# kerry-he/fsae-mpc

Measured on AMD Instinct MI355X. Metric: QP solves/sec (batched LTV-MPC, N=40 nx=5 nu=2 fp64), higher is better.
Workload: dtype f64

## Files before the change

### fsae-mpc_amd/_lib.py

```python
import ctypes as C
import os

_HERE = os.path.dirname(os.path.abspath(__file__))
LIB_PATH = os.environ.get("FSAEMPC_LIB") or os.path.join(_HERE, "lib", "libfsaempc.so")

EXPORTS = [
    "fsaempc_qp_default_opts", "fsaempc_qp_workspace_bytes", "fsaempc_qp_solve_batch_device", "fsaempc_qp_solve_batch",
    "fsaempc_ltv_nx", "fsaempc_ltv_nV", "fsaempc_ltv_nC", "fsaempc_ltv_build_qp_batch_device",
    "fsaempc_ltv_workspace_bytes", "fsaempc_ltv_step_batch_device", "fsaempc_ltv_step_batch_device_aux", "fsaempc_last_error", "fsaempc_selftest_mfma", "fsaempc_selftest_lane_reduce", "fsaempc_selftest_diag_factor",
    "fsaempc_debug_set_dump", "fsaempc_qp_solve_batch_device_aux", "fsaempc_qp_set_timing", "fsaempc_qp_get_timing", "fsaempc_ltv_get_timing",
    "fsaempc_seq_init", "fsaempc_seq_hotstart", "fsaempc_seq_hotstart_matrices", "fsaempc_seq_equality", "fsaempc_seq_cleanup",
    "fsaempc_obtain_reference_batch_device", "fsaempc_reference_live_batch_device",
    "fsaempc_cl_pre_batch_device", "fsaempc_cl_plant_batch_device", "fsaempc_cl_accept_batch_device",
    "fsaempc_track_from_csv", "fsaempc_track_from_points", "fsaempc_track_free", "fsaempc_track_save", "fsaempc_track_load", "fsaempc_track_last_error",
    "fsaempc_nlp_build_qp_batch_device", "fsaempc_sqp_default_opts", "fsaempc_sqp_workspace_bytes", "fsaempc_sqp_batch_device",
    "fsaempc_sqp_get_timing", "fsaempc_qp_vjp_workspace_bytes", "fsaempc_qp_vjp_batch_device",
    "fsaempc_ltv_affine_maps_batch_device", "fsaempc_ltv_step_batch_device_lambda", "fsaempc_ltv_step_vjp_workspace_bytes",
    "fsaempc_ltv_step_vjp_batch_device",
    "fsaempc_ltv_default_params", "fsaempc_ltv_build_qp_batch_device_p", "fsaempc_ltv_step_batch_device_p",
    "fsaempc_nlp_build_qp_batch_device_p", "fsaempc_sqp_batch_device_p", "fsaempc_cl_plant_batch_device_p",
    "fsaempc_ltv_blocked_nV", "fsaempc_ltv_build_qp_batch_device_b", "fsaempc_ltv_workspace_bytes_b", "fsaempc_ltv_step_batch_device_b",
    "fsaempc_qp_workspace_bytes_s", "fsaempc_qp_solve_batch_device_s", "fsaempc_qp_layout",
    "fsaempc_plan_profile_batch_device", "fsaempc_plan_reference_batch_device", "fsaempc_cl_pre_plan_batch_device",
    "fsaempc_raceline_build_qp_device", "fsaempc_plan_line_profile_batch_device", "fsaempc_plan_raceline_workspace_bytes",
    "fsaempc_plan_raceline_batch_device",
]

NPAR = 32
PARAM_INDEX = {name: i for i, name in enumerate(
    ["M", "IZ", "LF", "LR", "GRAV", "PB", "PC", "PD", "PE", "Q_S", "Q_N", "Q_MU", "Q_TERMINAL", "R_ACC", "R_STEER",
     "R_SOFT0", "R_SOFT1", "R_SOFT2", "R_SOFT3", "U_ACC_MAX", "U_STEER_MAX", "DELTA_MAX", "N_MAX", "V_MIN", "ALAT_MAX", "SLIP_MAX",
     "ELL_LONG", "ELL_LAT", "PID_KP_V", "PID_MAX_F", "PID_KP_D", "PID_MAX_DRATE"])}


class QpOpts(C.Structure):
    _fields_ = [("tol", C.c_double), ("tol_loose", C.c_double), ("tol_x", C.c_double), ("inf_bound", C.c_double),
                ("max_iter", C.c_int), ("polish", C.c_int)]


class QpAux(C.Structure):
    _fields_ = [("kkt", C.c_void_p), ("polished", C.c_void_p), ("x_init", C.c_void_p), ("difficulty", C.c_void_p)]


class QpDesc(C.Structure):
    _fields_ = [("nV", C.c_int), ("nC", C.c_int), ("batch", C.c_int), ("shared_HA", C.c_int)]


class QpVjpIO(C.Structure):
    _fields_ = [("xbar", C.c_void_p), ("fbar", C.c_void_p), ("gbar", C.c_void_p), ("lbbar", C.c_void_p), ("ubbar", C.c_void_p),
                ("lbAbar", C.c_void_p), ("ubAbar", C.c_void_p), ("Hbar", C.c_void_p), ("Abar", C.c_void_p)]


class LtvVjpIO(C.Structure):
    _fields_ = [("ubar", C.c_void_p), ("xbar", C.c_void_p), ("sbar", C.c_void_p), ("fbar", C.c_void_p), ("x0bar", C.c_void_p),
                ("xrefbar", C.c_void_p)]


class Spline(C.Structure):
    _fields_ = [("M", C.c_int), ("dl", C.c_double), ("xP", C.c_void_p), ("yP", C.c_void_p)]


class LtvDesc(C.Structure):
    _fields_ = [("model", C.c_int), ("N", C.c_int), ("batch", C.c_int), ("dt", C.c_double), ("integrator", C.c_int)]


class LtvParams(C.Structure):
    _fields_ = [("values", C.c_void_p), ("per_instance", C.c_int)]


class LtvBlocking(C.Structure):
    _fields_ = [("n_blocks", C.c_int), ("len", C.POINTER(C.c_int))]


PLAN_MAX_NS = 4096
LINE_MAX_NS = 2048
LINE_MIN_NC = 8
MAX_NV = 196


class PlanTable(C.Structure):
    _fields_ = [("table", C.c_void_p), ("t", C.c_void_p), ("N_s", C.c_int), ("ds", C.c_double), ("per_instance", C.c_int)]


def check_blocking(blocking, N):
    try:
        lens = [int(v) for v in blocking]
    except TypeError:
        raise ValueError("blocking must be a sequence of block lengths")
    if any(int(v) != v for v in blocking):
        raise ValueError("blocking: the block lengths must be integers")
    if len(lens) < 1:
        raise ValueError("blocking: at least one block")
    if min(lens) < 1:
        raise ValueError("blocking: every block length must be >= 1")
    if sum(lens) != N:
        raise ValueError("blocking: the block lengths sum to %d, the horizon has N = %d steps" % (sum(lens), N))
    return lens


class Blocking:

    def __init__(self, blocking, N):
        self.lens = check_blocking(blocking, N)
        self.n_blocks = len(self.lens)
        self.trivial = self.n_blocks == N
        self._arr = (C.c_int * self.n_blocks)(*self.lens)
        self.c = LtvBlocking(self.n_blocks, C.cast(self._arr, C.POINTER(C.c_int)))
        self.block_of_step = [j for j, l in enumerate(self.lens) for _ in range(l)]
        self.start = [sum(self.lens[:j]) for j in range(self.n_blocks)]

    def ref(self):
        return C.byref(self.c)


class SqpOpts(C.Structure):
    _fields_ = [("max_sweeps", C.c_int), ("trials", C.c_int), ("tol_step", C.c_double), ("tol_feas", C.c_double), ("armijo", C.c_double),
                ("rho0", C.c_double), ("warm_start", C.c_int)]


class SqpAux(C.Structure):
    _fields_ = [("lambda_", C.c_void_p), ("qp_iter", C.c_void_p), ("step_norm", C.c_void_p), ("hard_viol", C.c_void_p), ("merit", C.c_void_p)]


class TrackTable(C.Structure):
    _fields_ = [("M", C.c_int), ("dl", C.c_double), ("L", C.c_double), ("xP", C.POINTER(C.c_double)), ("yP", C.POINTER(C.c_double))]


class FsaempcError(RuntimeError):
    pass


_LIB = None


def lib():
    global _LIB
    if _LIB is None:
        if not os.path.exists(LIB_PATH):
            raise FsaempcError("libfsaempc.so not built (%s): run `make` or __graft_entry__.build(); "
                               "there is no CPU fallback" % LIB_PATH)
        try:
            import torch
        except ImportError:
            pass
        L = C.CDLL(LIB_PATH)
        L.fsaempc_last_error.restype = C.c_char_p
        L.fsaempc_qp_workspace_bytes.restype = C.c_longlong
        L.fsaempc_ltv_workspace_bytes.restype = C.c_longlong
        L.fsaempc_sqp_workspace_bytes.restype = C.c_longlong
        L.fsaempc_qp_vjp_workspace_bytes.restype = C.c_longlong
        L.fsaempc_ltv_step_vjp_workspace_bytes.restype = C.c_longlong
        vp, ll = C.c_void_p, C.c_longlong
        L.fsaempc_qp_solve_batch_device.argtypes = [C.POINTER(QpDesc)] + [vp] * 7 + [C.POINTER(QpOpts)] + [vp] * 5 + [vp, ll, vp]
        L.fsaempc_qp_solve_batch_device_aux.argtypes = [C.POINTER(QpDesc)] + [vp] * 7 + [C.POINTER(QpOpts)] + [vp] * 5 + [C.POINTER(QpAux), vp, ll, vp]
        L.fsaempc_qp_vjp_workspace_bytes.argtypes = [C.POINTER(QpDesc)]
        L.fsaempc_qp_vjp_batch_device.argtypes = [C.POINTER(QpDesc), C.c_int] + [vp] * 7 + [vp] * 4 + [C.POINTER(QpOpts), C.POINTER(QpVjpIO), vp, vp, ll, vp]
        L.fsaempc_ltv_affine_maps_batch_device.argtypes = [C.POINTER(LtvDesc), C.POINTER(Spline)] + [vp] * 5
        L.fsaempc_ltv_step_batch_device_lambda.argtypes = [C.POINTER(LtvDesc), C.POINTER(Spline)] + [vp] * 4 + [C.POINTER(QpOpts)] + [vp] * 7 + \
            [C.POINTER(QpAux), vp, ll, vp]
        L.fsaempc_ltv_step_vjp_workspace_bytes.argtypes = [C.POINTER(LtvDesc), C.c_int]
        L.fsaempc_ltv_step_vjp_batch_device.argtypes = [C.POINTER(LtvDesc), C.POINTER(Spline), C.c_int] + [vp] * 4 + [vp] * 5 + \
            [C.POINTER(QpOpts), C.POINTER(LtvVjpIO), vp, vp, ll, vp]
        L.fsaempc_qp_solve_batch.argtypes = [C.POINTER(QpDesc)] + [vp] * 7 + [C.POINTER(QpOpts)] + [vp] * 5
        L.fsaempc_ltv_build_qp_batch_device.argtypes = [C.POINTER(LtvDesc), C.POINTER(Spline)] + [vp] * 4 + [vp] * 7 + [vp] * 3 + [vp]
        L.fsaempc_ltv_step_batch_device.argtypes = [C.POINTER(LtvDesc), C.POINTER(Spline)] + [vp] * 4 + [C.POINTER(QpOpts)] + [vp] * 6 + [vp, ll, vp]
        L.fsaempc_ltv_step_batch_device_aux.argtypes = [C.POINTER(LtvDesc), C.POINTER(Spline)] + [vp] * 4 + [C.POINTER(QpOpts)] + [vp] * 6 + [C.POINTER(QpAux), vp, ll, vp]
        L.fsaempc_nlp_build_qp_batch_device.argtypes = [C.POINTER(LtvDesc), C.POINTER(Spline)] + [vp] * 3 + [vp] * 7 + [vp] * 3 + [vp]
        L.fsaempc_sqp_default_opts.argtypes = [C.POINTER(SqpOpts)]
        L.fsaempc_sqp_workspace_bytes.argtypes = [C.POINTER(LtvDesc)]
        L.fsaempc_sqp_batch_device.argtypes = [C.POINTER(LtvDesc), C.POINTER(Spline)] + [vp] * 3 + [C.POINTER(QpOpts), C.POINTER(SqpOpts)] + \
            [vp] * 6 + [C.POINTER(SqpAux), vp, ll, vp]
        L.fsaempc_sqp_get_timing.argtypes = [C.POINTER(C.c_double)] * 4
        L.fsaempc_obtain_reference_batch_device.argtypes = [vp, C.c_double, C.c_int, vp, vp, C.c_double, C.c_int, C.c_int, vp, vp]
        L.fsaempc_reference_live_batch_device.argtypes = [C.c_int, C.c_int, C.c_double, C.c_double, C.c_int, vp, vp, vp]
        L.fsaempc_cl_pre_batch_device.argtypes = [C.c_int, C.c_int, C.c_double, C.c_double, C.c_double, C.POINTER(Spline), vp, vp, C.c_int, vp, vp, vp, vp]
        L.fsaempc_cl_plant_batch_device.argtypes = [C.c_int, C.c_int, C.c_double, C.c_int, vp, vp, vp, vp, vp, vp, vp]
        L.fsaempc_cl_accept_batch_device.argtypes = [C.c_int, C.c_int, C.c_int, vp, vp, vp, vp, vp, vp]
        L.fsaempc_ltv_default_params.argtypes = [C.c_int, C.POINTER(C.c_double)]
        L.fsaempc_ltv_build_qp_batch_device_p.argtypes = [C.POINTER(LtvDesc), C.POINTER(Spline), C.POINTER(LtvParams)] + [vp] * 4 + [vp] * 7 + [vp] * 3 + [vp]
        L.fsaempc_ltv_step_batch_device_p.argtypes = [C.POINTER(LtvDesc), C.POINTER(Spline), C.POINTER(LtvParams)] + [vp] * 4 + [C.POINTER(QpOpts)] + \
            [vp] * 7 + [C.POINTER(QpAux), vp, ll, vp]
        L.fsaempc_nlp_build_qp_batch_device_p.argtypes = [C.POINTER(LtvDesc), C.POINTER(Spline), C.POINTER(LtvParams)] + [vp] * 3 + [vp] * 7 + [vp] * 3 + [vp]
        L.fsaempc_sqp_batch_device_p.argtypes = [C.POINTER(LtvDesc), C.POINTER(Spline), C.POINTER(LtvParams)] + [vp] * 3 + \
            [C.POINTER(QpOpts), C.POINTER(SqpOpts)] + [vp] * 6 + [C.POINTER(SqpAux), vp, ll, vp]
        L.fsaempc_cl_plant_batch_device_p.argtypes = [C.c_int, C.c_int, C.c_double, C.c_int, C.POINTER(LtvParams), vp, vp, vp, vp, vp, vp, vp]
        L.fsaempc_ltv_blocked_nV.argtypes = [C.c_int, C.POINTER(LtvBlocking)]
        L.fsaempc_ltv_build_qp_batch_device_b.argtypes = [C.POINTER(LtvDesc), C.POINTER(Spline), C.POINTER(LtvParams), C.POINTER(LtvBlocking)] + \
            [vp] * 4 + [vp] * 7 + [vp] * 3 + [vp]
        L.fsaempc_ltv_workspace_bytes_b.restype = C.c_longlong
        L.fsaempc_ltv_workspace_bytes_b.argtypes = [C.POINTER(LtvDesc), C.POINTER(LtvBlocking)]
        L.fsaempc_ltv_step_batch_device_b.argtypes = [C.POINTER(LtvDesc), C.POINTER(Spline), C.POINTER(LtvParams), C.POINTER(LtvBlocking)] + \
            [vp] * 4 + [C.POINTER(QpOpts)] + [vp] * 7 + [C.POINTER(QpAux), vp, ll, vp]
        L.fsaempc_qp_workspace_bytes_s.restype = C.c_longlong
        L.fsaempc_qp_workspace_bytes_s.argtypes = [C.POINTER(QpDesc), C.c_int]
        L.fsaempc_qp_solve_batch_device_s.argtypes = [C.POINTER(QpDesc), C.c_int] + [vp] * 7 + [C.POINTER(QpOpts)] + [vp] * 5 + \
            [C.POINTER(QpAux), vp, ll, vp]
        L.fsaempc_qp_layout.argtypes = [C.POINTER(QpDesc), C.c_int, C.POINTER(C.c_int)]
        L.fsaempc_plan_profile_batch_device.argtypes = [C.c_int, C.POINTER(Spline), C.c_double, C.POINTER(LtvParams), C.c_int, C.c_int,
                                                        C.c_double, C.c_double, vp, vp, vp]
        L.fsaempc_plan_reference_batch_device.argtypes = [C.c_int, C.POINTER(PlanTable), vp, C.c_double, C.c_int, C.c_int, vp, vp]
        L.fsaempc_cl_pre_plan_batch_device.argtypes = [C.c_int, C.c_int, C.c_double, C.c_double, C.POINTER(Spline), C.POINTER(PlanTable),
                                                       vp, vp, C.c_int, vp, vp, vp, vp]
        L.fsaempc_raceline_build_qp_device.argtypes = [C.POINTER(Spline), C.c_double, C.c_int, C.c_int, vp, vp, vp]
        L.fsaempc_plan_line_profile_batch_device.argtypes = [C.c_int, C.POINTER(Spline), C.c_double, C.POINTER(LtvParams), C.c_int, C.c_int, C.c_int,
                                                             vp, C.c_int, C.c_double, C.c_double, vp, vp, vp]
        L.fsaempc_plan_raceline_workspace_bytes.restype = C.c_longlong
        L.fsaempc_plan_raceline_workspace_bytes.argtypes = [C.c_int, C.c_int]
        L.fsaempc_plan_raceline_batch_device.argtypes = [C.c_int, C.POINTER(Spline), C.c_double, C.POINTER(LtvParams), C.c_int, C.c_int, C.c_int,
                                                         C.c_double, C.c_double, C.c_double, C.POINTER(QpOpts), vp, vp, vp, vp, vp, ll, vp]
        L.fsaempc_debug_set_dump.argtypes = [vp, C.c_int]
        L.fsaempc_track_last_error.restype = C.c_char_p
        L.fsaempc_track_from_csv.argtypes = [C.c_char_p, C.c_int, C.POINTER(TrackTable)]
        L.fsaempc_track_from_points.argtypes = [vp, vp, C.c_int, C.c_int, C.POINTER(TrackTable)]
        L.fsaempc_track_free.argtypes = [C.POINTER(TrackTable)]
        L.fsaempc_track_save.argtypes = [C.POINTER(TrackTable), C.c_char_p]
        L.fsaempc_track_load.argtypes = [C.c_char_p, C.POINTER(TrackTable)]
        _LIB = L
    return _LIB


def check(rc, what):
    if rc != 0:
        raise FsaempcError("%s failed (%d): %s" % (what, rc, lib().fsaempc_last_error().decode()))


def default_params(model):
    import numpy as np
    out = np.zeros(NPAR, dtype=np.float64)
    check(lib().fsaempc_ltv_default_params(int(model), out.ctypes.data_as(C.POINTER(C.c_double))), "fsaempc_ltv_default_params")
    return out


class ParamBlock:

    def __init__(self, params, batch, device):
        import numpy as np
        import torch
        t = params if isinstance(params, torch.Tensor) else torch.from_numpy(np.ascontiguousarray(np.asarray(params, dtype=np.float64)))
        if tuple(t.shape) not in ((NPAR,), (batch, NPAR)):
            raise ValueError("params must be (%d,) or (batch = %d, %d), got %s" % (NPAR, batch, NPAR, tuple(t.shape)))
        self.tensor = t.to(device=device, dtype=torch.float64).contiguous()
        self.per_instance = 1 if t.dim() == 2 else 0
        self.c = LtvParams(C.c_void_p(self.tensor.data_ptr()), self.per_instance)

    def ref(self):
        return C.byref(self.c)


def sqp_default_opts(**kw):
    o = SqpOpts()
    lib().fsaempc_sqp_default_opts(C.byref(o))
    for k, v in kw.items():
        if not hasattr(o, k):
            raise TypeError("unknown SQP option %r" % k)
        setattr(o, k, v)
    return o


def default_opts(**kw):
    o = QpOpts()
    lib().fsaempc_qp_default_opts(C.byref(o))
    for k, v in kw.items():
        setattr(o, k, v)
    return o
```

### fsae-mpc_amd/csrc/capi.hip

```cpp
#include <hip/hip_runtime.h>
#include <math.h>
#include <stdio.h>
#include <string.h>
#include <stdlib.h>
#include <dlfcn.h>
#include <atomic>
#include <mutex>
#include <vector>
#include "fsaempc.h"
#include "qp_solver.h"
#include "ltv_build.h"
#include "reference.h"
#include "plant.h"
#include "planner.h"
#include "raceline.h"
#include "sqp.h"
#include "qp_sens.h"

namespace {
thread_local char g_err[512] = "";
std::atomic<double*> g_dump{nullptr}; std::atomic<int> g_dump_stage{0};
std::atomic<bool> g_timing{false}; hipEvent_t g_ev[3] = {nullptr, nullptr, nullptr};
hipEvent_t g_evf[2] = {nullptr, nullptr};
hipEvent_t g_evs[5] = {nullptr, nullptr, nullptr, nullptr, nullptr};
// ... 767 lines not shown
  if (desc->batch == 0) return 0;
  SqpCarve c; sqp_carve(desc, &c);
  if ((long long)c.total > workspace_bytes) return fail(FSAEMPC_ERR_WORKSPACE, "workspace too small");
  char* w = (char*)workspace;
  auto D = [&](size_t off) { return (double*)(w + off); };
  auto Iw = [&](size_t off) { return (int*)(w + off); };
  hipStream_t st = (hipStream_t)stream;
  const int nx = fsaempc_ltv_nx(desc->model), N = desc->N, nV = fsaempc_ltv_nV(desc->model, N), nC = fsaempc_ltv_nC(desc->model, N);
  SqpParams P; memset(&P, 0, sizeof(P));
  P.nx = nx; P.N = N; P.integ = ltv_integ(desc); P.B = desc->batch; P.dt = desc->dt;
  P.spM = sp->M; P.spdl = sp->dl; P.xP = sp->xP; P.yP = sp->yP;
  P.x0 = x0; P.x_ref = x_ref; P.u = u_opt; P.x = x_opt; P.s = slack; P.fval = fval; P.status = status; P.sweeps = sweeps;
  P.rho = D(c.rho); P.J = D(c.J); P.viol = D(c.viol); P.vmax = D(c.vmax);
  if (aux) { P.lambda_out = aux->lambda; P.qp_iter = aux->qp_iter; P.step_norm = aux->step_norm; P.hard_viol = aux->hard_viol; P.merit = aux->merit; }
  P.max_sweeps = o.max_sweeps; P.trials = o.trials; P.tol_step = o.tol_step; P.tol_feas = o.tol_feas; P.armijo = o.armijo; P.rho0 = o.rho0;
  Range whole("fsaempc.sqp");
  const bool timing = g_timing.load();
  for (double& v : g_sqp_ms) v = 0;
  hipError_t e = sqp_init_launch(P, u_init, st, par_values(par), par_stride(par));
  if (e != hipSuccess) return hipfail(e, "sqp_init_launch");
  for (int sweep = 0; sweep < o.max_sweeps; ++sweep) {
    if (timing) { e = hipEventRecord(g_evs[0], st); if (e != hipSuccess) return hipfail(e, "hipEventRecord"); }
    int cnt = 0;
    { Range r("fsaempc.sqp.compact");
      e = sqp_compact_launch(status, desc->batch, Iw(c.idx), Iw(c.cnt), st);
      if (e == hipSuccess) e = hipMemcpyAsync(&cnt, Iw(c.cnt), sizeof(int), hipMemcpyDeviceToHost, st);
      if (e == hipSuccess) e = hipStreamSynchronize(st); }
    if (e != hipSuccess) return hipfail(e, "sqp compaction");
    if (cnt == 0) break;
    double* xinit = o.warm_start ? D(c.xinit) : nullptr;
    e = sqp_gather_launch(P, Iw(c.idx), cnt, D(c.gx0), D(c.gxr), D(c.gu), xinit, nV, st);
    if (e != hipSuccess) return hipfail(e, "sqp_gather_launch");
    if (timing) { e = hipEventRecord(g_evs[1], st); if (e != hipSuccess) return hipfail(e, "hipEventRecord"); }
    fsaempc_ltv_desc sub = *desc; sub.batch = cnt;
    { Range r("fsaempc.sqp.build");
      rc = build_qp(&sub, sp, D(c.gx0), D(c.gxr), nullptr, D(c.gu), D(c.H), D(c.g), D(c.A), D(c.lb), D(c.ub), D(c.lbA), D(c.ubA),
                    D(c.pred), D(c.Bt), D(c.qc), stream, true, par, Iw(c.idx)); }
    if (rc) return rc;
    if (timing) { e = hipEventRecord(g_evs[2], st); if (e != hipSuccess) return hipfail(e, "hipEventRecord"); }
    fsaempc_qp_desc q{nV, nC, cnt, 0};
    fsaempc_qp_aux qa{nullptr, nullptr, xinit, nullptr};
    rc = fsaempc_qp_solve_batch_device_aux(&q, D(c.H), D(c.g), D(c.A), D(c.lb), D(c.ub), D(c.lbA), D(c.ubA), qp_opts, D(c.z), D(c.qf),
                                           Iw(c.qflag), Iw(c.qit), D(c.lam), &qa, w + c.qpws, (long long)(c.total - c.qpws), stream);
    if (rc) return rc;
    if (timing) { e = hipEventRecord(g_evs[3], st); if (e != hipSuccess) return hipfail(e, "hipEventRecord"); }
    { Range r("fsaempc.sqp.linesearch");
      e = sqp_linesearch_launch(P, Iw(c.idx), cnt, sweep, D(c.z), D(c.qf), D(c.qc), Iw(c.qflag), Iw(c.qit), D(c.lam), st,
                                par_values(par), par_stride(par)); }
    if (e != hipSuccess) return hipfail(e, "sqp_linesearch_launch");
    if (timing) {
      e = hipEventRecord(g_evs[4], st); if (e == hipSuccess) e = hipEventSynchronize(g_evs[4]);
      if (e != hipSuccess) return hipfail(e, "hipEventRecord");
      for (int k = 0; k < 4; ++k) { float ms = 0; if (hipEventElapsedTime(&ms, g_evs[k], g_evs[k + 1]) == hipSuccess) g_sqp_ms[k] += ms; }
    }
  }
  return 0;
}

int fsaempc_sqp_get_timing(double* build_ms, double* solve_ms, double* linesearch_ms, double* compact_ms) {
  if (!build_ms || !solve_ms || !linesearch_ms || !compact_ms) return fail(FSAEMPC_ERR_ARG, "null argument");
  *compact_ms = g_sqp_ms[0]; *build_ms = g_sqp_ms[1]; *solve_ms = g_sqp_ms[2]; *linesearch_ms = g_sqp_ms[3];
  return 0;
}

int fsaempc_obtain_reference_batch_device(const double* plan, double ds, int N_s, const double* t, const double* s0, double dt,
                                          int N_t, int batch, double* x_ref, void* stream) {
  if (!plan || !t || !s0 || !x_ref) return fail(FSAEMPC_ERR_ARG, "null argument");
  if (N_s <= 0 || N_t <= 0 || batch < 0 || !(ds > 0) || !(dt > 0)) return fail(FSAEMPC_ERR_ARG, "bad dimensions");
  RefParams P; P.plan = plan; P.t = t; P.s0 = s0; P.x_ref = x_ref; P.ds = ds; P.dt = dt; P.N_s = N_s; P.N_t = N_t; P.batch = batch;
  hipError_t e = obtain_reference_launch(P, (hipStream_t)stream);
  if (e != hipSuccess) return hipfail(e, "obtain_reference_launch");
  return 0;
}

int fsaempc_reference_live_batch_device(int nx, int N, double dt, double target_vel, int batch, const double* x0, double* x_ref, void* stream) {
  if (!x0 || !x_ref) return fail(FSAEMPC_ERR_ARG, "null argument");
  if ((nx != 5 && nx != 7) || N <= 0 || batch < 0 || !(dt > 0)) return fail(FSAEMPC_ERR_ARG, "bad dimensions");
  hipError_t e = reference_live_launch(nx, N, dt, target_vel, batch, x0, x_ref, (hipStream_t)stream);
  if (e != hipSuccess) return hipfail(e, "reference_live_launch");
  return 0;
}

int fsaempc_cl_pre_batch_device(int model, int N, double dt, double target_vel, double L, const fsaempc_spline* sp, const double* cart,
                                const double* s_guess, int batch, double* x0, double* x_ref, int* finished, void* stream) {
  if (!sp || !sp->xP || !sp->yP || !cart || !s_guess || !x0 || !x_ref || !finished) return fail(FSAEMPC_ERR_ARG, "null argument");
  if (model != FSAEMPC_MODEL_KINEMATIC && model != FSAEMPC_MODEL_DYNAMIC) return fail(FSAEMPC_ERR_ARG, "unknown model");
  if (N <= 0 || batch < 0 || !(dt > 0) || sp->M <= 0 || !(sp->dl > 0) || !(L > 0)) return fail(FSAEMPC_ERR_ARG, "bad dimensions");
  ClPreParams P; P.nx = fsaempc_ltv_nx(model); P.N = N; P.batch = batch; P.dt = dt; P.target_vel = target_vel; P.L = L;
  P.spM = sp->M; P.spdl = sp->dl; P.xP = sp->xP; P.yP = sp->yP; P.cart = cart; P.s_guess = s_guess; P.x0 = x0; P.x_ref = x_ref; P.finished = finished;
  hipError_t e = cl_pre_launch(P, (hipStream_t)stream);
  if (e != hipSuccess) return hipfail(e, "cl_pre_launch");
  return 0;
}

int fsaempc_cl_plant_batch_device(int model, int N, double dt, int batch, double* cart, double* pid, const double* x_opt,
                                  const int* finished, const int* exitflag, double* u_last, void* stream) {
  return fsaempc_cl_plant_batch_device_p(model, N, dt, batch, nullptr, cart, pid, x_opt, finished, exitflag, u_last, stream);
}

int fsaempc_cl_plant_batch_device_p(int model, int N, double dt, int batch, const fsaempc_ltv_params* par, double* cart, double* pid,
                                    const double* x_opt, const int* finished, const int* exitflag, double* u_last, void* stream) {
  if (!cart || !pid || !x_opt) return fail(FSAEMPC_ERR_ARG, "null argument");
  if (model != FSAEMPC_MODEL_KINEMATIC && model != FSAEMPC_MODEL_DYNAMIC) return fail(FSAEMPC_ERR_ARG, "unknown model");
  if (N <= 0 || batch < 0 || !(dt > 0)) return fail(FSAEMPC_ERR_ARG, "bad dimensions");
  ClPlantParams P; P.nx = fsaempc_ltv_nx(model); P.N = N; P.batch = batch; P.dt = dt; P.cart = cart; P.pid = pid; P.x_opt = x_opt;
  P.finished = finished; P.exitflag = exitflag; P.u_last = u_last;
  hipError_t e = cl_plant_launch(P, (hipStream_t)stream, par_values(par), par_stride(par));
  if (e != hipSuccess) return hipfail(e, "cl_plant_launch");
  return 0;
}

int fsaempc_cl_accept_batch_device(int model, int N, int batch, const double* x_new, const double* u_new, const int* exitflag, double* x_keep, double* u_keep, void* stream) {
  if (!x_new || !u_new || !x_keep || !u_keep) return fail(FSAEMPC_ERR_ARG, "null argument");
  if (model != FSAEMPC_MODEL_KINEMATIC && model != FSAEMPC_MODEL_DYNAMIC) return fail(FSAEMPC_ERR_ARG, "unknown model");
  if (N <= 0 || batch < 0) return fail(FSAEMPC_ERR_ARG, "bad dimensions");
  hipError_t e = cl_accept_launch(fsaempc_ltv_nx(model) * N, 2 * N, batch, x_new, u_new, exitflag, x_keep, u_keep, (hipStream_t)stream);
  if (e != hipSuccess) return hipfail(e, "cl_accept_launch");
  return 0;
}

static bool pos_finite(double v) { return v > 0 && v < INFINITY; }
static int plan_check(const fsaempc_plan* plan, PlanTable* out) {
  if (!plan || !plan->table || !plan->t) return fail(FSAEMPC_ERR_ARG, "null argument");
  if (plan->N_s < 1 || !pos_finite(plan->ds)) return fail(FSAEMPC_ERR_ARG, "bad plan dimensions");
  out->table = plan->table; out->t = plan->t; out->N_s = plan->N_s; out->ds = plan->ds; out->per_instance = plan->per_instance ? 1 : 0;
  return 0;
}

int fsaempc_plan_profile_batch_device(int model, const fsaempc_spline* sp, double L, const fsaempc_ltv_params* par, int n_plans, int N_s,
                                      double v_cap, double grip, double* table, double* t, void* stream) {
  if (!sp || !sp->xP || !sp->yP || !table || !t) return fail(FSAEMPC_ERR_ARG, "null argument");
  if (model != FSAEMPC_MODEL_KINEMATIC && model != FSAEMPC_MODEL_DYNAMIC) return fail(FSAEMPC_ERR_ARG, "unknown model");
  if (sp->M <= 0 || !(sp->dl > 0)) return fail(FSAEMPC_ERR_ARG, "bad dimensions");
  if (N_s < 2 || N_s > FSAEMPC_PLAN_MAX_NS) return fail(FSAEMPC_ERR_ARG, "N_s must be 2 .. FSAEMPC_PLAN_MAX_NS");
  if (!pos_finite(v_cap) || !pos_finite(grip) || !pos_finite(L)) return fail(FSAEMPC_ERR_ARG, "v_cap, grip and L must be finite and > 0");
  if (grip > 1) return fail(FSAEMPC_ERR_ARG, "grip must be <= 1");
  if (n_plans < 1) return fail(FSAEMPC_ERR_ARG, "n_plans must be >= 1");
  if (par_values(par) && !par->per_instance && n_plans != 1) return fail(FSAEMPC_ERR_ARG, "a shared parameter block makes one plan");
  PlanProfileParams P; P.dynamic = model == FSAEMPC_MODEL_DYNAMIC; P.n_plans = n_plans; P.N_s = N_s; P.ds = L / N_s; P.v_cap = v_cap; P.grip = grip;
  P.spM = sp->M; P.spdl = sp->dl; P.xP = sp->xP; P.yP = sp->yP; P.table = table; P.t = t;
  hipError_t e = plan_profile_launch(P, par_values(par), par_stride(par), (hipStream_t)stream);
  if (e != hipSuccess) return hipfail(e, "plan_profile_launch");
  return 0;
}

int fsaempc_plan_reference_batch_device(int model, const fsaempc_plan* plan, const double* s0, double dt, int N, int batch, double* x_ref,
                                        void* stream) {
  PlanRefParams P;
  if (int rc = plan_check(plan, &P.plan)) return rc;
  if (!s0 || !x_ref) return fail(FSAEMPC_ERR_ARG, "null argument");
  if (model != FSAEMPC_MODEL_KINEMATIC && model != FSAEMPC_MODEL_DYNAMIC) return fail(FSAEMPC_ERR_ARG, "unknown model");
  if (N <= 0 || batch < 0 || !pos_finite(dt)) return fail(FSAEMPC_ERR_ARG, "bad dimensions");
  P.nx = fsaempc_ltv_nx(model); P.N = N; P.batch = batch; P.dt = dt; P.s0 = s0; P.x_ref = x_ref;
  hipError_t e = plan_reference_launch(P, (hipStream_t)stream);
  if (e != hipSuccess) return hipfail(e, "plan_reference_launch");
  return 0;
}

int fsaempc_cl_pre_plan_batch_device(int model, int N, double dt, double L, const fsaempc_spline* sp, const fsaempc_plan* plan,
                                     const double* cart, const double* s_guess, int batch, double* x0, double* x_ref, int* finished,
                                     void* stream) {
  ClPrePlanParams P;
  if (!sp || !sp->xP || !sp->yP || !cart || !s_guess || !x0 || !x_ref || !finished) return fail(FSAEMPC_ERR_ARG, "null argument");
  if (int rc = plan_check(plan, &P.plan)) return rc;
  if (model != FSAEMPC_MODEL_KINEMATIC && model != FSAEMPC_MODEL_DYNAMIC) return fail(FSAEMPC_ERR_ARG, "unknown model");
  if (N <= 0 || batch < 0 || !pos_finite(dt) || sp->M <= 0 || !(sp->dl > 0) || !(L > 0)) return fail(FSAEMPC_ERR_ARG, "bad dimensions");
  P.nx = fsaempc_ltv_nx(model); P.N = N; P.batch = batch; P.dt = dt; P.L = L;
  P.spM = sp->M; P.spdl = sp->dl; P.xP = sp->xP; P.yP = sp->yP; P.cart = cart; P.s_guess = s_guess; P.x0 = x0; P.x_ref = x_ref; P.finished = finished;
  hipError_t e = cl_pre_plan_launch(P, (hipStream_t)stream);
  if (e != hipSuccess) return hipfail(e, "cl_pre_plan_launch");
  return 0;
}

static int line_check(const fsaempc_spline* sp, double L, int N_s, int N_c) {
  if (!sp || !sp->xP || !sp->yP) return fail(FSAEMPC_ERR_ARG, "null argument");
  if (sp->M <= 0 || !(sp->dl > 0)) return fail(FSAEMPC_ERR_ARG, "bad dimensions");
  if (!pos_finite(L)) return fail(FSAEMPC_ERR_ARG, "L must be finite and > 0");
  if (N_c < FSAEMPC_LINE_MIN_NC || N_c > FSAEMPC_MAX_NV) return fail(FSAEMPC_ERR_ARG, "N_c must be FSAEMPC_LINE_MIN_NC .. FSAEMPC_MAX_NV");
  if (N_s < 2 * N_c || N_s > FSAEMPC_LINE_MAX_NS) return fail(FSAEMPC_ERR_ARG, "N_s must be 2 N_c .. FSAEMPC_LINE_MAX_NS");
  return 0;
}
static int line_profile_check(int model, const fsaempc_ltv_params* par, int n_plans, double v_cap, double grip) {
  if (model != FSAEMPC_MODEL_KINEMATIC && model != FSAEMPC_MODEL_DYNAMIC) return fail(FSAEMPC_ERR_ARG, "unknown model");
  if (!pos_finite(v_cap) || !pos_finite(grip)) return fail(FSAEMPC_ERR_ARG, "v_cap and grip must be finite and > 0");
  if (grip > 1) return fail(FSAEMPC_ERR_ARG, "grip must be <= 1");
  if (n_plans < 1) return fail(FSAEMPC_ERR_ARG, "n_plans must be >= 1");
  if (par_values(par) && !par->per_instance && n_plans != 1) return fail(FSAEMPC_ERR_ARG, "a shared parameter block makes one plan");
  return 0;
}
static RacelineQpParams line_qp_params(const fsaempc_spline* sp, double L, int N_s, int N_c, double* H, double* g) {
  RacelineQpParams Q; Q.N_s = N_s; Q.N_c = N_c; Q.ds = L / N_s; Q.spM = sp->M; Q.spdl = sp->dl; Q.xP = sp->xP; Q.yP = sp->yP; Q.H = H; Q.g = g;
  return Q;
}
static PlanLineParams line_profile_params(int model, const fsaempc_spline* sp, double L, int n_plans, int N_s, int N_c, double v_cap, double grip,
                                          double* table, double* t) {
  PlanLineParams P; memset(&P, 0, sizeof(P));
  P.dynamic = model == FSAEMPC_MODEL_DYNAMIC; P.n_plans = n_plans; P.N_s = N_s; P.N_c = N_c; P.ds = L / N_s; P.h = L / N_c; P.v_cap = v_cap; P.grip = grip;
  P.spM = sp->M; P.spdl = sp->dl; P.xP = sp->xP; P.yP = sp->yP; P.table = table; P.t = t;
  return P;
}

int fsaempc_raceline_build_qp_device(const fsaempc_spline* sp, double L, int N_s, int N_c, double* H, double* g, void* stream) {
  if (!H || !g) return fail(FSAEMPC_ERR_ARG, "null argument");
  if (int rc = line_check(sp, L, N_s, N_c)) return rc;
  hipError_t e = raceline_qp_launch(line_qp_params(sp, L, N_s, N_c, H, g), (hipStream_t)stream);
  if (e != hipSuccess) return hipfail(e, "raceline_qp_launch");
  return 0;
}

int fsaempc_plan_line_profile_batch_device(int model, const fsaempc_spline* sp, double L, const fsaempc_ltv_params* par, int n_plans, int N_s,
                                           int N_c, const double* line, int line_per_plan, double v_cap, double grip, double* table, double* t,
                                           void* stream) {
  if (!line || !table || !t) return fail(FSAEMPC_ERR_ARG, "null argument");
  if (int rc = line_check(sp, L, N_s, N_c)) return rc;
  if (int rc = line_profile_check(model, par, n_plans, v_cap, grip)) return rc;
  PlanLineParams P = line_profile_params(model, sp, L, n_plans, N_s, N_c, v_cap, grip, table, t);
  P.line = line; P.line_stride = line_per_plan ? N_c : 0;
  hipError_t e = plan_line_profile_launch(P, par_values(par), par_stride(par), (hipStream_t)stream);
  if (e != hipSuccess) return hipfail(e, "plan_line_profile_launch");
  return 0;
}

struct LineCarve { size_t H, g, lb, ub, fval, iter, qp, total; long long qp_bytes; };
static int line_carve(int n_plans, int N_c, LineCarve* c) {
  if (n_plans < 1 || N_c < FSAEMPC_LINE_MIN_NC || N_c > FSAEMPC_MAX_NV) return FSAEMPC_ERR_ARG;
  const fsaempc_qp_desc d = {N_c, 0, n_plans, 1};
  c->qp_bytes = fsaempc_qp_workspace_bytes_s(&d, 0);
  if (c->qp_bytes < 0) return (int)c->qp_bytes;
  const size_t vec = align64((size_t)n_plans * N_c * sizeof(double));
  size_t off = 0;
  c->H = off; off += align64((size_t)N_c * N_c * sizeof(double));
  c->g = off; off += vec;
  c->lb = off; off += vec;
  c->ub = off; off += vec;
  c->fval = off; off += align64((size_t)n_plans * sizeof(double));
  c->iter = off; off += align64((size_t)n_plans * sizeof(int));
  c->qp = off; off += (size_t)c->qp_bytes;
  c->total = off;
  return 0;
}
long long fsaempc_plan_raceline_workspace_bytes(int n_plans, int N_c) {
  LineCarve c;
  if (int rc = line_carve(n_plans, N_c, &c)) return rc;
  return (long long)c.total;
}

int fsaempc_plan_raceline_batch_device(int model, const fsaempc_spline* sp, double L, const fsaempc_ltv_params* par, int n_plans, int N_s,
                                       int N_c, double margin, double v_cap, double grip, const fsaempc_qp_opts* opts, double* line, int* flag,
                                       double* table, double* t, void* workspace, long long workspace_bytes, void* stream) {
  if (!line || !flag || !table || !t || !workspace) return fail(FSAEMPC_ERR_ARG, "null argument");
  if (int rc = line_check(sp, L, N_s, N_c)) return rc;
  if (int rc = line_profile_check(model, par, n_plans, v_cap, grip)) return rc;
  if (!(margin >= 0 && margin < INFINITY)) return fail(FSAEMPC_ERR_ARG, "margin must be finite and >= 0");
  LineCarve c;
  if (int rc = line_carve(n_plans, N_c, &c)) return fail(rc, "bad dimensions");
  if ((long long)c.total > workspace_bytes) return fail(FSAEMPC_ERR_WORKSPACE, "workspace too small");
  char* ws = (char*)workspace;
  double *H = (double*)(ws + c.H), *g = (double*)(ws + c.g), *lb = (double*)(ws + c.lb), *ub = (double*)(ws + c.ub);
  hipError_t e = raceline_qp_launch(line_qp_params(sp, L, N_s, N_c, H, g), (hipStream_t)stream);
  if (e != hipSuccess) return hipfail(e, "raceline_qp_launch");
  RacelineBoundsParams B; B.n_plans = n_plans; B.N_c = N_c; B.margin = margin; B.g = g; B.lb = lb; B.ub = ub;
  e = raceline_bounds_launch(B, par_values(par), par_stride(par), (hipStream_t)stream);
  if (e != hipSuccess) return hipfail(e, "raceline_bounds_launch");
  const fsaempc_qp_desc d = {N_c, 0, n_plans, 1};
  if (int rc = fsaempc_qp_solve_batch_device_s(&d, 0, H, g, nullptr, lb, ub, nullptr, nullptr, opts, line, (double*)(ws + c.fval), flag,
                                               (int*)(ws + c.iter), nullptr, nullptr, ws + c.qp, c.qp_bytes, stream)) return rc;
  PlanLineParams P = line_profile_params(model, sp, L, n_plans, N_s, N_c, v_cap, grip, table, t);
  P.line = line; P.line_stride = N_c; P.flag = flag; P.line_out = line; P.check_width = 1; P.margin = margin;
  e = plan_line_profile_launch(P, par_values(par), par_stride(par), (hipStream_t)stream);
  if (e != hipSuccess) return hipfail(e, "plan_line_profile_launch");
  return 0;
}

int fsaempc_selftest_mfma(void) {
  int cnt = 0;
  hipError_t e = hipGetDeviceCount(&cnt);
  if (e != hipSuccess || cnt == 0) return fail(FSAEMPC_ERR_NODEVICE, "no HIP device");
  char msg[256] = "";
  int bad = qp_selftest_mfma(msg, sizeof(msg));
  if (bad != 0) snprintf(g_err, sizeof(g_err), "%s", msg);
  return bad;
}

int fsaempc_selftest_lane_reduce(void) {
  int cnt = 0;
  hipError_t e = hipGetDeviceCount(&cnt);
  if (e != hipSuccess || cnt == 0) return fail(FSAEMPC_ERR_NODEVICE, "no HIP device");
  char msg[256] = "";
  int bad = qp_selftest_lane_reduce(msg, sizeof(msg));
  if (bad != 0) snprintf(g_err, sizeof(g_err), "%s", msg);
  return bad;
}

int fsaempc_selftest_diag_factor(void) {
  int cnt = 0;
  hipError_t e = hipGetDeviceCount(&cnt);
  if (e != hipSuccess || cnt == 0) return fail(FSAEMPC_ERR_NODEVICE, "no HIP device");
  char msg[256] = "";
  int bad = qp_selftest_diag_factor(msg, sizeof(msg));
  if (bad != 0) snprintf(g_err, sizeof(g_err), "%s", msg);
  return bad;
}

int fsaempc_debug_set_dump(double* out, int stage) { g_dump.store(out); g_dump_stage.store(stage); return 0; }

int fsaempc_qp_set_timing(int enable) {
  if (enable && !g_ev[0]) {
    for (int i = 0; i < 3; ++i) { hipError_t e = hipEventCreate(&g_ev[i]); if (e != hipSuccess) return hipfail(e, "hipEventCreate"); }
    for (int i = 0; i < 2; ++i) { hipError_t e = hipEventCreate(&g_evf[i]); if (e != hipSuccess) return hipfail(e, "hipEventCreate"); }
    for (int i = 0; i < 5; ++i) { hipError_t e = hipEventCreate(&g_evs[i]); if (e != hipSuccess) return hipfail(e, "hipEventCreate"); }
  }
  g_timing.store(enable != 0);
  return 0;
}

int fsaempc_ltv_get_timing(double* build_ms, double* prep_ms, double* solve_ms, double* post_ms) {
  if (!g_evf[0]) return fail(FSAEMPC_ERR_ARG, "timing was never enabled");
  hipError_t e = hipEventSynchronize(g_evf[1]);
  if (e != hipSuccess) return hipfail(e, "hipEventSynchronize (no fused step since timing was enabled?)");
  float t[4] = {0, 0, 0, 0};
  e = hipEventElapsedTime(&t[0], g_evf[0], g_ev[0]); if (e != hipSuccess) return hipfail(e, "hipEventElapsedTime");
  e = hipEventElapsedTime(&t[1], g_ev[0], g_ev[1]); if (e != hipSuccess) return hipfail(e, "hipEventElapsedTime");
  e = hipEventElapsedTime(&t[2], g_ev[1], g_ev[2]); if (e != hipSuccess) return hipfail(e, "hipEventElapsedTime");
  e = hipEventElapsedTime(&t[3], g_ev[2], g_evf[1]); if (e != hipSuccess) return hipfail(e, "hipEventElapsedTime");
  if (build_ms) *build_ms = t[0];
  if (prep_ms) *prep_ms = t[1];
  if (solve_ms) *solve_ms = t[2];
  if (post_ms) *post_ms = t[3];
  return 0;
}

int fsaempc_qp_get_timing(double* prep_ms, double* solve_ms) {
  if (!g_ev[0]) return fail(FSAEMPC_ERR_ARG, "timing was never enabled");
  hipError_t e = hipEventSynchronize(g_ev[2]);
  if (e != hipSuccess) return hipfail(e, "hipEventSynchronize");
  float a = 0, b = 0;
  e = hipEventElapsedTime(&a, g_ev[0], g_ev[1]); if (e != hipSuccess) return hipfail(e, "hipEventElapsedTime");
  e = hipEventElapsedTime(&b, g_ev[1], g_ev[2]); if (e != hipSuccess) return hipfail(e, "hipEventElapsedTime");
  if (prep_ms) *prep_ms = a;
  if (solve_ms) *solve_ms = b;
  return 0;
}

}
```

### fsae-mpc_amd/csrc/qp_selftest.h

```cpp
#pragma once
#include <stdlib.h>
#include <stdio.h>
#include "qp_solve_kernel.h"

namespace {

__global__ void mfma_selftest_kernel(const double* Am, const double* Bm, double* Cm) {
  const int lane = threadIdx.x;
  const double a = Am[(lane & 15) * 4 + (lane >> 4)];
  const double bb = Bm[(lane >> 4) * 16 + (lane & 15)];
  v4d c = {0, 0, 0, 0};
  c = __builtin_amdgcn_mfma_f64_16x16x4f64(a, bb, c, 0, 0, 0);
#pragma unroll
  for (int p = 0; p < 4; ++p) Cm[((lane >> 4) + 4 * p) * 16 + (lane & 15)] = c[p];
}

DEVINL bool same_bits(double a, double b) { return __double_as_longlong(a) == __double_as_longlong(b) || (a != a && b != b); }
template <class OP> DEVINL double lds_grp16(double* sh, int lane, double v) {
  const int src[4] = {lane ^ 1, lane ^ 2, (lane & ~7) | (7 - (lane & 7)), (lane & ~15) | (15 - (lane & 15))};
#pragma unroll
  for (int s = 0; s < 4; ++s) {
    sh[lane] = v; __syncthreads();
    const double o = sh[src[s]]; __syncthreads();
    v = OP::f(v, o);
  }
  return v;
}
template <class OP> DEVINL double lds_q(double* sh, int lane, double v) {
#pragma unroll
  for (int bit = 16; bit <= 32; bit <<= 1) {
    sh[lane] = v; __syncthreads();
    const double a = sh[lane & ~bit], b = sh[lane | bit]; __syncthreads();
    v = OP::f(a, b);
  }
  return v;
}
DEVINL double q_named(OpSum, double v) { return q_sum(v); }
DEVINL double q_named(OpMax, double v) { return q_max(v); }
DEVINL double q_named(OpMin, double v) { return q_min(v); }
DEVINL double wave_named(OpSum, double v) { return wave_sum(v); }
DEVINL double wave_named(OpMax, double v) { return wave_max(v); }
DEVINL double wave_named(OpMin, double v) { return wave_min(v); }
DEVINL double wave_named_zf(OpSum, double v) { return wave_sum_zf(v); }
DEVINL double wave_named_zf(OpMax, double v) { return wave_max_zf(v); }
DEVINL double wave_named_zf(OpMin, double v) { return wave_min_zf(v); }
DEVINL double grp16_named(OpSum, double v) { return grp16_sum(v); }
DEVINL double grp16_named(OpMax, double v) { return grp16_max(v); }
DEVINL double grp16_named(OpMin, double v) { return grp16_min(v); }
template <int N> DEVINL void grp16_named(OpSum, double (&v)[N]) { grp16_sum(v); }
template <int N> DEVINL void grp16_named(OpMax, double (&v)[N]) { grp16_max(v); }
template <int N> DEVINL void grp16_named(OpMin, double (&v)[N]) { grp16_min(v); }
template <class OP, int N> DEVINL int lane_reduce_batch_bad(const double (&x)[8], const double (&rz)[8], const double (&rl_)[8]) {
  double a[N];
#pragma unroll
  for (int i = 0; i < N; ++i) a[i] = x[i];
  grp16_named(OP{}, a);
  int bad = 0;
#pragma unroll
  for (int i = 0; i < N; ++i) bad += (same_bits(a[i], rz[i]) ? 0 : 1) + (same_bits(a[i], rl_[i]) ? 0 : 1);
  return bad;
}
template <class OP> DEVINL int lane_reduce_op_bad(int op, double* sh, int lane, const double (&x)[8], int& first) {
  double rz[8], rl_[8];
#pragma unroll
  for (int i = 0; i < 8; ++i) {
    double z[1] = {x[i]};
    grp16_reduce<OP, true>(z);
    rz[i] = z[0];
    rl_[i] = lds_grp16<OP>(sh, lane, x[i]);
  }
  int bad = 0, b;
  auto note = [&](int test, int nb) { if (nb && first < 0) first = 100 * test + op; bad += nb; };
  { const double g = grp16_named(OP{}, x[0]); note(1, (same_bits(g, rz[0]) ? 0 : 1) + (same_bits(g, rl_[0]) ? 0 : 1)); }
  b = lane_reduce_batch_bad<OP, 2>(x, rz, rl_); note(2, b);
  b = lane_reduce_batch_bad<OP, 4>(x, rz, rl_); note(4, b);
  b = lane_reduce_batch_bad<OP, 8>(x, rz, rl_); note(8, b);
  { const double g = q_named(OP{}, x[1]); note(16, same_bits(g, lds_q<OP>(sh, lane, x[1])) ? 0 : 1); }
  {
    const double g = wave_named(OP{}, x[2]), z = wave_named_zf(OP{}, x[2]), l = lds_q<OP>(sh, lane, rl_[2]);
    note(64, (same_bits(g, z) ? 0 : 1) + (same_bits(g, l) ? 0 : 1));
  }
  return bad;
}
__global__ __launch_bounds__(64) void lane_reduce_selftest_kernel(const double* __restrict__ in, int rounds, int* __restrict__ out) {
  __shared__ double sh[64];
  const int lane = threadIdx.x;
  int bad = 0, first = -1, first_round = -1;
  for (int r = 0; r < rounds; ++r) {
    double x[8];
#pragma unroll
    for (int i = 0; i < 8; ++i) x[i] = in[((size_t)r * 8 + i) * 64 + lane];
    const int before = bad;
    bad += lane_reduce_op_bad<OpSum>(0, sh, lane, x, first);
    bad += lane_reduce_op_bad<OpMax>(1, sh, lane, x, first);
    bad += lane_reduce_op_bad<OpMin>(2, sh, lane, x, first);
    {
      double a[4] = {x[4], x[5], x[6], x[7]};
      wave_sum(a);
      int nb = 0;
#pragma unroll
      for (int i = 0; i < 4; ++i) nb += same_bits(a[i], wave_sum_zf(x[4 + i])) ? 0 : 1;
      if (nb && first < 0) first = 100 * 65;
      bad += nb;
    }
    if (bad != before && first_round < 0) first_round = r;
  }
  if (bad) {
    if (atomicAdd(&out[0], bad) == 0) { out[1] = first; out[2] = first_round; out[3] = lane; }
  }
}

template <int FORM> DEVINL int diag_factor_bad_vs_old(const Ctx& k, const v4d& U0, const v4d& R0, double floor_abs, const v4d& Uo, const v4d& Yo, const v4d& Ro, int bo) {
  v4d U = U0, R = R0, Y;
#pragma unroll
  for (int p = 0; p < 4; ++p) Y[p] = (k.q + 4 * p == k.c) ? 1.0 : 0.0;
  const int b = diag_factor<FORM>(k, U, Y, R, floor_abs);
  int bad = (b != bo) ? 1 : 0;
#pragma unroll
  for (int p = 0; p < 4; ++p)
    bad += (__double_as_longlong(U[p]) != __double_as_longlong(Uo[p])) + (__double_as_longlong(Y[p]) != __double_as_longlong(Yo[p])) +
           (__double_as_longlong(R[p]) != __double_as_longlong(Ro[p]));
  return bad;
}
__global__ __launch_bounds__(64) void diag_factor_selftest_kernel(const double* __restrict__ in, int ntiles, double floor_abs, int* __restrict__ out) {
  Ctx k = {};
  k.lane = threadIdx.x; k.c = k.lane & 15; k.q = k.lane >> 4;
  int bad = 0, first = -1, form = 0;
  for (int t = 0; t < ntiles; ++t) {
    v4d U0, R0, Uo, Ro, Yo;
#pragma unroll
    for (int p = 0; p < 4; ++p) {
      U0[p] = in[(size_t)t * 512 + (k.q + 4 * p) * 16 + k.c];
      R0[p] = in[(size_t)t * 512 + 256 + (k.q + 4 * p) * 16 + k.c];
      Yo[p] = (k.q + 4 * p == k.c) ? 1.0 : 0.0;
    }
    Uo = U0; Ro = R0;
    const int bo = diag_factor<0>(k, Uo, Yo, Ro, floor_abs);
    const int b1 = diag_factor_bad_vs_old<1>(k, U0, R0, floor_abs, Uo, Yo, Ro, bo);
    const int b2 = diag_factor_bad_vs_old<2>(k, U0, R0, floor_abs, Uo, Yo, Ro, bo);
    if ((b1 | b2) && first < 0) { first = t; form = b1 ? 1 : 2; }
    bad += b1 + b2;
  }
  if (bad) {
    if (atomicAdd(&out[0], bad) == 0) { out[1] = first; out[2] = form; out[3] = k.lane; }
  }
}

}

int qp_selftest_mfma(char* msg, int msglen) {
  double hA[64], hB[64], hC[256], ref[256];
  for (int i = 0; i < 16; ++i) for (int kk = 0; kk < 4; ++kk) hA[i * 4 + kk] = (double)(1 + i * 7 + kk * 3);
  for (int kk = 0; kk < 4; ++kk) for (int j = 0; j < 16; ++j) hB[kk * 16 + j] = (double)(2 + kk * 11 - j * 5);
  for (int i = 0; i < 16; ++i) for (int j = 0; j < 16; ++j) {
    double s = 0; for (int kk = 0; kk < 4; ++kk) s += hA[i * 4 + kk] * hB[kk * 16 + j];
    ref[i * 16 + j] = s;
  }
  double *dA = 0, *dB = 0, *dC = 0;
  if (hipMalloc(&dA, sizeof(hA)) != hipSuccess || hipMalloc(&dB, sizeof(hB)) != hipSuccess || hipMalloc(&dC, sizeof(hC)) != hipSuccess) return -1;
  (void)hipMemcpy(dA, hA, sizeof(hA), hipMemcpyHostToDevice);
  (void)hipMemcpy(dB, hB, sizeof(hB), hipMemcpyHostToDevice);
  (void)hipMemset(dC, 0, sizeof(hC));
  hipLaunchKernelGGL(mfma_selftest_kernel, dim3(1), dim3(64), 0, 0, dA, dB, dC);
  hipError_t e = hipDeviceSynchronize();
  if (e != hipSuccess) { snprintf(msg, msglen, "selftest launch: %s", hipGetErrorString(e)); (void)hipFree(dA); (void)hipFree(dB); (void)hipFree(dC); return -1; }
  (void)hipMemcpy(hC, dC, sizeof(hC), hipMemcpyDeviceToHost);
  (void)hipFree(dA); (void)hipFree(dB); (void)hipFree(dC);
  int bad = 0;
  for (int i = 0; i < 256; ++i) if (hC[i] != ref[i]) { if (!bad) snprintf(msg, msglen, "mfma layout mismatch at (%d,%d): got %g want %g", i / 16, i % 16, hC[i], ref[i]); ++bad; }
  return bad;
}

int qp_selftest_lane_reduce(char* msg, int msglen) {
  const int rounds = 256, nval = rounds * 8 * 64;
  double* h = (double*)malloc(sizeof(double) * nval);
  if (!h) return -1;
  unsigned long long st = 0x9E3779B97F4A7C15ull;
  auto rnd = [&]() { st = st * 6364136223846793005ull + 1442695040888963407ull; return (unsigned)(st >> 33); };
  for (int i = 0; i < nval; ++i) {
    const double e = -300.0 + 600.0 * (rnd() / 2147483648.0), m = 1.0 + 9.0 * (rnd() / 2147483648.0);
    h[i] = ((rnd() & 1) ? -1.0 : 1.0) * m * pow(10.0, e);
  }
  const double special[8] = {0.0, -0.0, 4.9406564584124654e-324, -2.2250738585072009e-308 / 3.0, INFINITY, -INFINITY, NAN, -NAN};
  for (int g = 0; g < rounds * 8; ++g) {
    const unsigned u = rnd();
    if ((u & 3) != 0) h[(size_t)g * 64 + ((u >> 2) & 63)] = special[(u >> 8) & 7];
    if ((u & 0x30000) == 0x30000) h[(size_t)g * 64 + ((u >> 18) & 63)] = special[(u >> 24) & 7];
  }
  double* d = 0; int* dout = 0; int hout[4] = {0, 0, 0, 0};
  if (hipMalloc(&d, sizeof(double) * nval) != hipSuccess || hipMalloc(&dout, sizeof(hout)) != hipSuccess) { free(h); if (d) (void)hipFree(d); return -1; }
  (void)hipMemcpy(d, h, sizeof(double) * nval, hipMemcpyHostToDevice);
  (void)hipMemset(dout, 0, sizeof(hout));
  free(h);
  hipLaunchKernelGGL(lane_reduce_selftest_kernel, dim3(1), dim3(64), 0, 0, d, rounds, dout);
  hipError_t e = hipDeviceSynchronize();
  if (e == hipSuccess) e = hipMemcpy(hout, dout, sizeof(hout), hipMemcpyDeviceToHost);
  (void)hipFree(d); (void)hipFree(dout);
  if (e != hipSuccess) { snprintf(msg, msglen, "lane-reduce selftest: %s", hipGetErrorString(e)); return -1; }
  if (hout[0]) snprintf(msg, msglen, "lane reductions: %d mismatches, first: test %d (1/2/4/8: grp16 single / batched, 16: q, 64: wave, 65: wave_sum batch) op %d (sum/max/min) round %d lane %d",
                        hout[0], hout[1] / 100, hout[1] % 100, hout[2], hout[3]);
  return hout[0];
}

int qp_selftest_diag_factor(char* msg, int msglen) {
  const int ntiles = 64;
  const double floor_abs = 1e-9;
  double* h = (double*)malloc(sizeof(double) * ntiles * 512);
  if (!h) return -1;
  unsigned long long st = 0xD1B54A32D192ED03ull;
  auto rnd = [&]() { st = st * 6364136223846793005ull + 1442695040888963407ull; return ((unsigned)(st >> 33)) / 2147483648.0; };
  for (int t = 0; t < ntiles; ++t) {
    double* D = h + (size_t)t * 512; double* R = D + 256;
    double Q[16][16], sv[16];
    for (int i = 0; i < 16; ++i) for (int j = 0; j < 16; ++j) Q[i][j] = i == j ? 1.0 : 0.0;
    for (int r = 0; r < 3; ++r) {
      double v[16], vv = 0;
      for (int i = 0; i < 16; ++i) { v[i] = 2.0 * rnd() - 1.0; vv += v[i] * v[i]; }
      for (int i = 0; i < 16; ++i) {
        double qv = 0;
        for (int j = 0; j < 16; ++j) qv += Q[i][j] * v[j];
        for (int j = 0; j < 16; ++j) Q[i][j] -= 2.0 * qv * v[j] / vv;
      }
    }
    const double lc = 10.0 * (t < 61 ? t / 60.0 : 0.3);
    for (int i = 0; i < 16; ++i) sv[i] = pow(10.0, -lc * i / 15.0);
    for (int i = 0; i < 16; ++i) for (int j = 0; j < 16; ++j) {
      double a = 0;
      for (int l = 0; l < 16; ++l) a += Q[i][l] * sv[l] * Q[j][l];
      D[i * 16 + j] = a;
    }
    for (int i = 0; i < 16; ++i) for (int j = 0; j < i; ++j) D[i * 16 + j] = D[j * 16 + i];
    for (int i = 0; i < 256; ++i) R[i] = 20.0 * rnd() - 10.0;
    if (t == 61) for (int j = 0; j < 16; ++j) { D[6 * 16 + j] *= 1e-6; D[j * 16 + 6] *= 1e-6; }
    if (t == 62) { D[5 * 16 + 9] = NAN; D[9 * 16 + 5] = NAN; }
    if (t == 63) D[10 * 16 + 10] = INFINITY;
  }
  double* d = 0; int* dout = 0; int hout[4] = {0, 0, 0, 0};
  if (hipMalloc(&d, sizeof(double) * ntiles * 512) != hipSuccess || hipMalloc(&dout, sizeof(hout)) != hipSuccess) { free(h); if (d) (void)hipFree(d); return -1; }
  (void)hipMemcpy(d, h, sizeof(double) * ntiles * 512, hipMemcpyHostToDevice);
  (void)hipMemset(dout, 0, sizeof(hout));
  free(h);
  hipLaunchKernelGGL(diag_factor_selftest_kernel, dim3(1), dim3(64), 0, 0, d, ntiles, floor_abs, dout);
  hipError_t e = hipDeviceSynchronize();
  if (e == hipSuccess) e = hipMemcpy(hout, dout, sizeof(hout), hipMemcpyDeviceToHost);
  (void)hipFree(d); (void)hipFree(dout);
  if (e != hipSuccess) { snprintf(msg, msglen, "diag_factor selftest: %s", hipGetErrorString(e)); return -1; }
  if (hout[0]) snprintf(msg, msglen, "diag_factor forms: %d mismatches with the former form, first: tile %d form %d lane %d", hout[0], hout[1], hout[2], hout[3]);
  return hout[0];
}
```

### fsae-mpc_amd/csrc/qp_solve_kernel.h

```cpp
#pragma once
#include "qp_solver.h"
#include "qp_lane.h"

#ifndef QP_SOLVE_PAIR
#define QP_SOLVE_PAIR 0
#endif
#ifndef QP_DIAG_FLAT
#define QP_DIAG_FLAT 1
#endif
#ifndef QP_SYRK_INTERLEAVE
#define QP_SYRK_INTERLEAVE 0
#endif

namespace {

template <int T> struct Tri {
  static constexpr int NT = T * (T + 1) / 2;
  __host__ __device__ static constexpr int idx(int I, int J) { return I * T - (I * (I - 1)) / 2 + (J - I); }
};

struct Ctx {
  int n, m, T, Kq, J, JB, JT, np, lane, c, q, nc, nb, ntr;
  const int* perm; const int* tcs; const int* aoff; const int* tend;
  const double* Aw; const double* Hw; const double* Ab; const double* Hb;
  double* rows;
  double* ring;
  double* cof;
  int rowlen;
  double* vec;
};
enum VecArr { V_X = 0, V_G, V_HX, V_R1, V_R2, V_P1, V_P2, V_P3, V_DX, V_E, V_NARR };

DEVINL double* rowp(const Ctx& k, int arr) { return k.rows + (size_t)arr * k.rowlen; }
DEVINL double* vecp(const Ctx& k, int arr) { return k.vec + arr * k.np; }

DEVINL bool row_valid(const Ctx& k, int js) {
  if (js < k.J) { const int s = 16 * js + k.c; return s < k.Kq && 4 * s + k.q < k.m; }
  return (js - k.J) * 64 + k.lane < k.n;
}

template <int T> DEVINL void hx_tiles(const Ctx& k, const double* X, double* HX) {
  double hx[T], hn[T][4], hc[T][4];
#pragma unroll
  for (int t = 0; t < T; ++t) hx[t] = 0.0;
#pragma unroll
  for (int Jt = 0; Jt < T; ++Jt)
#pragma unroll
    for (int p = 0; p < 4; ++p) hn[Jt][p] = k.Hw[((size_t)Jt * 4 + p) * 64 + k.lane];
#pragma unroll 1
  for (int I = 0; I < T; ++I) {
#pragma unroll
    for (int Jt = 0; Jt < T; ++Jt)
#pragma unroll
      for (int p = 0; p < 4; ++p) hc[Jt][p] = hn[Jt][p];
    if (I + 1 < T) {
#pragma unroll
      for (int Jt = 0; Jt < T; ++Jt)
#pragma unroll
        for (int p = 0; p < 4; ++p) hn[Jt][p] = k.Hw[((size_t)((I + 1) * T + Jt) * 4 + p) * 64 + k.lane];
    }
    double xk[4];
#pragma unroll
    for (int p = 0; p < 4; ++p) xk[p] = X[16 * I + k.q + 4 * p];
#pragma unroll
    for (int Jt = 0; Jt < T; ++Jt)
#pragma unroll
      for (int p = 0; p < 4; ++p) hx[Jt] = fma(hc[Jt][p], xk[p], hx[Jt]);
  }
#pragma unroll
  for (int t = 0; t < T; ++t) {
    double v = q_sum(hx[t]);
    if (k.q == 0) HX[16 * t + k.c] = v;
  }
}
template <int T> DEVINL void acc_init(const Ctx& k, v4d* acc) {
#pragma unroll
  for (int I = 0; I < T; ++I)
#pragma unroll
    for (int Jt = I; Jt < T; ++Jt) {
      const double* hp = k.Hw + ((size_t)(I * T + Jt) * 4) * 64 + k.lane;
      v4d h;
#pragma unroll
      for (int p = 0; p < 4; ++p) h[p] = hp[p * 64];
      acc[Tri<T>::idx(I, Jt)] = h;
    }
}

template <int T> DEVINL void hx_from_acc(const Ctx& k, const v4d* acc, const double* XV, double* HX) {
  double xr[T][4], xc[T], sc[T], sr[T][4];
#pragma unroll
  for (int I = 0; I < T; ++I) {
    xc[I] = XV[16 * I + k.c]; sc[I] = 0.0;
#pragma unroll
    for (int p = 0; p < 4; ++p) { xr[I][p] = XV[16 * I + k.q + 4 * p]; sr[I][p] = 0.0; }
  }
#pragma unroll
  for (int I = 0; I < T; ++I)
#pragma unroll
    for (int J = I; J < T; ++J) {
      const v4d& h = acc[Tri<T>::idx(I, J)];
#pragma unroll
      for (int p = 0; p < 4; ++p) {
        sc[J] = fma(h[p], xr[I][p], sc[J]);
        if (J > I) sr[I][p] = fma(h[p], xc[J], sr[I][p]);
      }
    }
  WAVE_SYNC();
#pragma unroll
  for (int J = 0; J < T; ++J) { const double v = q_sum(sc[J]); if (k.q == 0) HX[16 * J + k.c] = v; }
  WAVE_SYNC();
#pragma unroll
  for (int I = 0; I < T - 1; ++I) {
    grp16_sum(sr[I]);
#pragma unroll
    for (int p = 0; p < 4; ++p) if (k.c == 0) HX[16 * I + k.q + 4 * p] += sr[I][p];
  }
}

template <int C> struct IC { static constexpr int value = C; };

template <int T> struct StreamCfg {
  static constexpr int D = 2 * T;
  static constexpr int R = D + T;
};
template <int T> struct Stream {
  static constexpr int D = StreamCfg<T>::D, R = StreamCfg<T>::R;
  static_assert(R == QP_SOLVE_RING(T), "qp_solve_lds (qp_solver.h) sizes the ring");
  const char* gnext; int slot_i, slot_e;
  int tend[T + 1];
  DEVINL void issue(const Ctx& k) {
    __builtin_amdgcn_global_load_lds((const __attribute__((address_space(1))) void*)(gnext + k.lane * 16),
                                     (__attribute__((address_space(3))) void*)(k.ring + slot_i * 128), 16, 0, 0);
    gnext += 1024;
    slot_i = slot_i + 1 == R ? 0 : slot_i + 1;
  }
  DEVINL void open(const Ctx& k) {
    gnext = reinterpret_cast<const char*>(k.Aw); slot_i = 0; slot_e = 0;
#pragma unroll
    for (int C = 0; C <= T; ++C) tend[C] = uni(k.tend[C]);
  }
  DEVINL void start(const Ctx& k) {
    gnext = reinterpret_cast<const char*>(k.Aw); slot_i = 0; slot_e = 0;
    if (k.ntr > 0) {
#pragma unroll
      for (int j = 0; j < D; ++j) issue(k);
    }
#pragma unroll
    for (int C = 0; C <= T; ++C) tend[C] = uni(tend[C]);
  }
  template <int C> DEVINL void next_pair(const Ctx& k, v2d* b) {
#pragma unroll
    for (int t = 0; t < C; ++t) issue(k);
    asm volatile("s_waitcnt vmcnt(%0)" :: "n"(D) : "memory");
#pragma unroll
    for (int t = 0; t < C; ++t) {
      int sl = slot_e + t; if (sl >= R) sl -= R;
      b[t] = *reinterpret_cast<const v2d*>(k.ring + sl * 128 + k.lane * 2);
    }
    slot_e += C; if (slot_e >= R) slot_e -= R;
  }
  DEVINL void finish() { asm volatile("s_waitcnt vmcnt(0)" ::: "memory"); }
  DEVINL void close() { asm volatile("s_waitcnt vmcnt(0)" ::: "memory"); }
};

template <int NA> struct CoefStage {
  double reg[NA > 0 ? NA : 1];
  DEVINL void load(const Ctx& k, const double* const* arr, int js) {
    const int jc = js < k.J ? js : k.J - 1;
#pragma unroll
    for (int a = 0; a < NA; ++a) reg[a] = arr[a][jc * 64 + k.lane];
  }
  DEVINL void commit(const Ctx& k) {
#pragma unroll
    for (int a = 0; a < NA; ++a) k.cof[a * 64 + k.lane] = reg[a];
  }
  DEVINL void read_pair(const Ctx& k, int s, v2d* out) const {
#pragma unroll
    for (int a = 0; a < NA; ++a) out[a] = *reinterpret_cast<const v2d*>(k.cof + a * 64 + k.q * 16 + (s & 15));
  }
};

template <int T, int NB> DEVINL void pass_syrk(const Ctx& k, Stream<T>& st, v4d* acc, double* P1, double* P2, double* P3, double* MB) {
  constexpr int NBB = NB > 0 ? NB : 1;
  constexpr int NA = 4 + NB;
  const int JS = k.J * 64;
  const double* arr[NA];
  arr[0] = rowp(k, R_D); arr[1] = rowp(k, R_W1); arr[2] = rowp(k, R_W2); arr[3] = rowp(k, R_W3);
#pragma unroll
  for (int e = 0; e < NB; ++e) arr[4 + e] = k.Ab + (size_t)e * JS;
  double p1[T], p2[T], p3[T];
  double pb[NBB][T], sbb[NBB][NBB], pwb[3][NBB];
#pragma unroll
  for (int t = 0; t < T; ++t) { p1[t] = 0; p2[t] = 0; p3[t] = 0; }
#pragma unroll
  for (int e = 0; e < NBB; ++e) {
#pragma unroll
    for (int t = 0; t < T; ++t) pb[e][t] = 0;
#pragma unroll
    for (int f = 0; f < NBB; ++f) sbb[e][f] = 0;
    pwb[0][e] = pwb[1][e] = pwb[2][e] = 0;
  }
  CoefStage<NA> cs;
  int tr = 0;
  st.start(k);
  if (k.ntr > 0) cs.load(k, arr, 0);
  auto phase = [&](auto Cc) __attribute__((always_inline)) {
    constexpr int C = decltype(Cc)::value;
    const int tr_end = st.tend[C];
    for (; tr < tr_end; ++tr) {
      if ((tr & 3) == 0) { cs.commit(k); cs.load(k, arr, (tr >> 2) + 1); }
#pragma unroll
      for (int u = 0; u < 2; ++u) {
        v2d b[C], cf[NA];
        st.template next_pair<C>(k, b);
        cs.read_pair(k, 4 * tr + 2 * u, cf);
        asm volatile("" ::: "memory");
#if QP_SYRK_INTERLEAVE
        double a2[2][C];
#pragma unroll
        for (int h = 0; h < 2; ++h)
#pragma unroll
          for (int t = 0; t < C; ++t) a2[h][t] = cf[0][h] * b[t][h];
#endif
#pragma unroll
        for (int h = 0; h < 2; ++h) {
          double a[C], ab[NBB];
          const double dd = cf[0][h], w1 = cf[1][h], w2 = cf[2][h], w3 = cf[3][h];
#pragma unroll
          for (int e = 0; e < NB; ++e) ab[e] = cf[4 + e][h];
#pragma unroll
#if QP_SYRK_INTERLEAVE
          for (int t = 0; t < C; ++t) a[t] = a2[h][t];
#else
          for (int t = 0; t < C; ++t) a[t] = dd * b[t][h];
#endif
#pragma unroll
          for (int I = 0; I < C; ++I)
#pragma unroll
            for (int Jt = I; Jt < C; ++Jt)
              acc[Tri<T>::idx(I, Jt)] = __builtin_amdgcn_mfma_f64_16x16x4f64(a[I], b[Jt][h], acc[Tri<T>::idx(I, Jt)], 0, 0, 0);
#pragma unroll
          for (int t = 0; t < C; ++t) {
            p1[t] = fma(w1, b[t][h], p1[t]); p2[t] = fma(w2, b[t][h], p2[t]); p3[t] = fma(w3, b[t][h], p3[t]);
          }
#pragma unroll
          for (int e = 0; e < NB; ++e) {
            const double dab = dd * ab[e];
#pragma unroll
            for (int t = 0; t < C; ++t) pb[e][t] = fma(dab, b[t][h], pb[e][t]);
#pragma unroll
            for (int f = e; f < NB; ++f) sbb[e][f] = fma(dab, ab[f], sbb[e][f]);
            pwb[0][e] = fma(w1, ab[e], pwb[0][e]); pwb[1][e] = fma(w2, ab[e], pwb[1][e]); pwb[2][e] = fma(w3, ab[e], pwb[2][e]);
          }
#if QP_SYRK_INTERLEAVE
#pragma unroll
          for (int i = 0; i < C * (C + 1) / 2; ++i) {
            __builtin_amdgcn_sched_group_barrier(0x008, 1, 0);
            __builtin_amdgcn_sched_group_barrier(0x002, 2, 0);
          }
#endif
        }
      }
    }
  };
  if constexpr (T >= 1) phase(IC<1>{});
  if constexpr (T >= 2) phase(IC<2>{});
  if constexpr (T >= 3) phase(IC<3>{});
  if constexpr (T >= 4) phase(IC<4>{});
  if constexpr (T >= 5) phase(IC<5>{});
  if constexpr (T >= 6) phase(IC<6>{});
  if constexpr (T >= 7) phase(IC<7>{});
  if constexpr (T >= 8) phase(IC<8>{});
  if (k.ntr > 0) st.finish();
#pragma unroll
  for (int t = 0; t < T; ++t) {
    double v1 = q_sum(p1[t]), v2 = q_sum(p2[t]), v3 = q_sum(p3[t]);
    if (k.q == 0) { P1[16 * t + k.c] = v1; P2[16 * t + k.c] = v2; P3[16 * t + k.c] = v3; }
  }
#pragma unroll
  for (int e = 0; e < NB; ++e) {
#pragma unroll
    for (int t = 0; t < T; ++t) { const double vb = q_sum(pb[e][t]); if (k.q == 0) MB[e * k.np + 16 * t + k.c] = vb; }
    const double v1 = q_sum(pwb[0][e]), v2 = q_sum(pwb[1][e]), v3 = q_sum(pwb[2][e]);
    if (k.lane == 0) { P1[k.nc + e] = v1; P2[k.nc + e] = v2; P3[k.nc + e] = v3; }
#pragma unroll
    for (int f = 0; f < NB; ++f) {
      const double sv = q_sum(f >= e ? sbb[e][f] : sbb[f][e]);
      if (k.lane == 0) MB[e * k.np + k.nc + f] = sv;
    }
  }
}

template <int T, int NB, int NVEC, int FUSE> DEVINL void pass_Av(const Ctx& k, Stream<T>& st, const double* const* vin, double* const* rout, double* Pcor, double* Pcor2 = nullptr, const double* const* cfarr = nullptr) {
  constexpr int NBB = NB > 0 ? NB : 1;
  constexpr int NC = FUSE == 1 ? 6 : (FUSE >= 2 ? 3 : 0);
  constexpr int NA = NC + NB;
  const int JS = k.J * 64;
  const double* arr[NA > 0 ? NA : 1];
  if (FUSE == 1) { arr[0] = rowp(k, R_RPL); arr[1] = rowp(k, R_CB1); arr[2] = rowp(k, R_CC1); arr[3] = rowp(k, R_RPU); arr[4] = rowp(k, R_CB2); arr[5] = rowp(k, R_CC2); }
  if (FUSE >= 2) { arr[0] = cfarr ? cfarr[0] : rowp(k, R_CB1); arr[1] = cfarr ? cfarr[1] : rowp(k, R_RPL); arr[2] = cfarr ? cfarr[2] : rowp(k, R_CC1); }
#pragma unroll
  for (int f = 0; f < NB; ++f) arr[NC + f] = k.Ab + (size_t)f * JS;
  double v[NVEC][T], vb[NVEC][NBB], pc[T], pcb[NBB], pd[FUSE >= 2 ? T : 1], pdb[NBB];
#pragma unroll
  for (int e = 0; e < NVEC; ++e) {
#pragma unroll
    for (int t = 0; t < T; ++t) v[e][t] = vin[e][16 * t + k.c];
#pragma unroll
    for (int f = 0; f < NB; ++f) vb[e][f] = vin[e][k.nc + f];
  }
#pragma unroll
  for (int t = 0; t < T; ++t) pc[t] = 0.0;
#pragma unroll
  for (int f = 0; f < NBB; ++f) { pcb[f] = 0.0; pdb[f] = 0.0; }
#pragma unroll
  for (int t = 0; t < (FUSE >= 2 ? T : 1); ++t) pd[t] = 0.0;
  double keep[NVEC + 1];
#pragma unroll
  for (int e = 0; e < NVEC + 1; ++e) keep[e] = 0.0;
  CoefStage<NA> cs;
  int tr = 0;
  st.start(k);
  if (k.ntr > 0 && NA > 0) cs.load(k, arr, 0);
  auto phase = [&](auto Cc) __attribute__((always_inline)) {
    constexpr int C = decltype(Cc)::value;
    const int tr_end = st.tend[C];
    for (; tr < tr_end; ++tr) {
      if (NA > 0 && (tr & 3) == 0) { cs.commit(k); cs.load(k, arr, (tr >> 2) + 1); }
#pragma unroll
      for (int u = 0; u < 2; ++u) {
        v2d b[C], cf[NA > 0 ? NA : 1];
        st.template next_pair<C>(k, b);
        if (NA > 0) cs.read_pair(k, 4 * tr + 2 * u, cf);
        asm volatile("" ::: "memory");
        double ds[2 * NVEC];
#pragma unroll
        for (int h = 0; h < 2; ++h)
#pragma unroll
          for (int e = 0; e < NVEC; ++e) {
            double a = 0.0;
#pragma unroll
            for (int t = 0; t < C; ++t) a = fma(b[t][h], v[e][t], a);
            ds[h * NVEC + e] = a;
          }
        grp16_sum(ds);
#pragma unroll
        for (int h = 0; h < 2; ++h) {
          const int s = 4 * tr + 2 * u + h;
          const int cc = s & 15;
#pragma unroll
          for (int e = 0; e < NVEC; ++e) {
            double dsum = ds[h * NVEC + e];
#pragma unroll
            for (int f = 0; f < NB; ++f) dsum = fma(cf[NC + f][h], vb[e][f], dsum);
            if (k.c == cc) keep[e] = dsum;
            if (FUSE >= 2 && e == 0) {
              const double pen = cf[0][h] * (dsum - cf[1][h]);
              const double ynew = cf[2][h] - pen;
              if (k.c == cc) keep[NVEC] = ynew;
#pragma unroll
              for (int t = 0; t < C; ++t) { pc[t] = fma(ynew, b[t][h], pc[t]); pd[t] = fma(pen, b[t][h], pd[t]); }
#pragma unroll
              for (int f = 0; f < NB; ++f) { pcb[f] = fma(ynew, cf[NC + f][h], pcb[f]); pdb[f] = fma(pen, cf[NC + f][h], pdb[f]); }
            }
            if (FUSE == 1 && e == 0) {
              const double dl_ = dsum + cf[0][h], du_ = cf[3][h] - dsum;
              const double w = dl_ * fma(cf[2][h], dl_, cf[1][h]) - du_ * fma(cf[5][h], du_, cf[4][h]);
#pragma unroll
              for (int t = 0; t < C; ++t) pc[t] = fma(w, b[t][h], pc[t]);
#pragma unroll
              for (int f = 0; f < NB; ++f) pcb[f] = fma(w, cf[NC + f][h], pcb[f]);
            }
          }
          if (cc == 15 || s + 1 == 4 * k.ntr) {
            const int js = s >> 4;
#pragma unroll
            for (int e = 0; e < NVEC; ++e) { rout[e][js * 64 + k.lane] = keep[e]; keep[e] = 0.0; }
            if (FUSE >= 2) { rout[NVEC][js * 64 + k.lane] = keep[NVEC]; keep[NVEC] = 0.0; }
          }
        }
      }
    }
  };
  if constexpr (T >= 1) phase(IC<1>{});
  if constexpr (T >= 2) phase(IC<2>{});
  if constexpr (T >= 3) phase(IC<3>{});
  if constexpr (T >= 4) phase(IC<4>{});
  if constexpr (T >= 5) phase(IC<5>{});
  if constexpr (T >= 6) phase(IC<6>{});
  if constexpr (T >= 7) phase(IC<7>{});
  if constexpr (T >= 8) phase(IC<8>{});
  if (k.ntr > 0) st.finish();
  if (FUSE) {
#pragma unroll
    for (int t = 0; t < T; ++t) {
      double pv = q_sum(pc[t]);
      if (k.q == 0) Pcor[16 * t + k.c] = pv;
    }
#pragma unroll
    for (int f = 0; f < NB; ++f) { const double pv = q_sum(pcb[f]); if (k.lane == 0) Pcor[k.nc + f] = pv; }
  }
  if (FUSE >= 2) {
#pragma unroll
    for (int t = 0; t < T; ++t) {
      double pv = q_sum(pd[t]);
      if (k.q == 0) Pcor2[16 * t + k.c] = pv;
    }
#pragma unroll
    for (int f = 0; f < NB; ++f) { const double pv = q_sum(pdb[f]); if (k.lane == 0) Pcor2[k.nc + f] = pv; }
  }
}

template <int T, int NB> DEVINL void pass_Atw(const Ctx& k, const double* W, double* Pout) {
  constexpr int NBB = NB > 0 ? NB : 1;
  const int JS = k.J * 64;
  double p[T], pbv[NBB];
#pragma unroll
  for (int t = 0; t < T; ++t) p[t] = 0.0;
#pragma unroll
  for (int f = 0; f < NBB; ++f) pbv[f] = 0.0;
  for (int s = 0; s < 4 * k.ntr; ++s) {
    const int ri = (s >> 4) * 64 + k.q * 16 + (s & 15);
    const double w = W[ri];
    const int tr = s >> 2, tc = k.tcs[tr];
    const double* src = k.Aw + ((size_t)k.aoff[tr] + ((s >> 1) & 1) * tc) * 128 + k.lane * 2 + (s & 1);
#pragma unroll
    for (int t = 0; t < T; ++t)
      if (t < tc) p[t] = fma(w, src[t * 128], p[t]);
#pragma unroll
    for (int f = 0; f < NB; ++f) pbv[f] = fma(w, k.Ab[(size_t)f * JS + ri], pbv[f]);
  }
#pragma unroll
  for (int t = 0; t < T; ++t) {
    double v = q_sum(p[t]);
    if (k.q == 0) Pout[16 * t + k.c] = v;
  }
#pragma unroll
  for (int f = 0; f < NB; ++f) { const double pv = q_sum(pbv[f]); if (k.lane == 0) Pout[k.nc + f] = pv; }
}

template <int T> DEVINL void mfma4_sub(const v4d& X, const v4d& Y, v4d& Dst) {
#pragma unroll
  for (int p = 0; p < 4; ++p) Dst = __builtin_amdgcn_mfma_f64_16x16x4f64(-X[p], Y[p], Dst, 0, 0, 0);
}
DEVINL v4d mfma4_new(const v4d& X, const v4d& Y) {
  v4d Z = {0.0, 0.0, 0.0, 0.0};
#pragma unroll
  for (int p = 0; p < 4; ++p) Z = __builtin_amdgcn_mfma_f64_16x16x4f64(X[p], Y[p], Z, 0, 0, 0);
  return Z;
}

DEVINL void tile_store(const Ctx& k, double* slot, const v4d& Xt) {
#pragma unroll
  for (int p = 0; p < 4; ++p) slot[(k.q + 4 * p) * 17 + k.c] = Xt[p];
}
DEVINL v4d tile_load(const Ctx& k, const double* slot) {
  v4d Z;
#pragma unroll
  for (int p = 0; p < 4; ++p) Z[p] = slot[(k.q + 4 * p) * 17 + k.c];
  return Z;
}
DEVINL v4d tile_load_t(const Ctx& k, const double* slot) {
  v4d Z;
#pragma unroll
  for (int p = 0; p < 4; ++p) Z[p] = slot[k.c * 17 + k.q + 4 * p];
  return Z;
}

DEVINL double on_lanes(unsigned long long mask, double v, double otherwise) {
  return __builtin_amdgcn_inverse_ballot_w64(mask) ? v : otherwise;
}
template <int FORM> DEVINL int diag_factor(const Ctx& k, v4d& Ud, v4d& Yk, v4d& rk, double floor_abs) {
  constexpr bool FLAT = FORM >= 1;
  int bad = 0;
#pragma unroll
  for (int p = 0; p < 4; ++p) {
    const double d00 = rl(Ud[p], 4 * p + 0), d01 = rl(Ud[p], 4 * p + 1), d02 = rl(Ud[p], 4 * p + 2), d03 = rl(Ud[p], 4 * p + 3);
    const double d11 = rl(Ud[p], 16 + 4 * p + 1), d12 = rl(Ud[p], 16 + 4 * p + 2), d13 = rl(Ud[p], 16 + 4 * p + 3);
    const double d22 = rl(Ud[p], 32 + 4 * p + 2), d23 = rl(Ud[p], 32 + 4 * p + 3);
    const double d33 = rl(Ud[p], 48 + 4 * p + 3);
    auto piv = [&](double t) {
      if constexpr (FORM >= 2) {
        const bool low = !(t > floor_abs);
        bad |= (low & !(fabs(t) < INFINITY)) ? 1 : 0;
        t = low ? floor_abs : t;
      } else {
        if (!(t > floor_abs)) { if (!(fabs(t) < INFINITY)) bad = 1; t = floor_abs; }
      }
      return rsqrt(t);
    };
    const double i0 = piv(d00);
    const double r01 = d01 * i0, r02 = d02 * i0, r03 = d03 * i0;
    const double i1 = piv(fma(-r01, r01, d11));
    const double r12 = fma(-r01, r02, d12) * i1, r13 = fma(-r01, r03, d13) * i1;
    const double i2 = piv(fma(-r12, r12, fma(-r02, r02, d22)));
    const double r23 = fma(-r12, r13, fma(-r02, r03, d23)) * i2;
    const double i3 = piv(fma(-r23, r23, fma(-r13, r13, fma(-r03, r03, d33))));
    const double w10 = -r01 * i0 * i1;
    const double w20 = -fma(r12, w10, r02 * i0) * i2, w21 = -r12 * i1 * i2;
    const double w30 = -fma(r23, w20, fma(r13, w10, r03 * i0)) * i3, w31 = -fma(r23, w21, r13 * i1) * i3, w32 = -r23 * i2 * i3;
    const v4d z = {0.0, 0.0, 0.0, 0.0};
    if constexpr (FLAT) {
      const unsigned long long L0 = 1ull << (4 * p), L1 = 1ull << (16 + 4 * p), L2 = 1ull << (32 + 4 * p), L3 = 1ull << (48 + 4 * p);
      double wa = on_lanes(L0, i0, 0.0);
      wa = on_lanes(L0 << 1, w10, wa); wa = on_lanes(L0 << 2, w20, wa); wa = on_lanes(L0 << 3, w30, wa);
      wa = on_lanes(L1 << 1, i1, wa); wa = on_lanes(L1 << 2, w21, wa); wa = on_lanes(L1 << 3, w31, wa);
      wa = on_lanes(L2 << 2, i2, wa); wa = on_lanes(L2 << 3, w32, wa);
      wa = on_lanes(L3 << 3, i3, wa);
      const v4d nu = __builtin_amdgcn_mfma_f64_16x16x4f64(wa, Ud[p], z, 0, 0, 0);
      Ud[p] = nu[p];
      double a = 0.0;
      if (p < 3) {
        a = on_lanes(0x0001000100010001ull * (0xFFFFull & (0xFFFFull << (4 * p + 4))), -Ud[p], 0.0);
        Ud = __builtin_amdgcn_mfma_f64_16x16x4f64(a, Ud[p], Ud, 0, 0, 0);
      }
      const v4d ny = __builtin_amdgcn_mfma_f64_16x16x4f64(wa, Yk[p], z, 0, 0, 0);
      const v4d nr = __builtin_amdgcn_mfma_f64_16x16x4f64(wa, rk[p], z, 0, 0, 0);
      Yk[p] = ny[p]; rk[p] = nr[p];
      if (p < 3) {
        Yk = __builtin_amdgcn_mfma_f64_16x16x4f64(a, Yk[p], Yk, 0, 0, 0);
        rk = __builtin_amdgcn_mfma_f64_16x16x4f64(a, rk[p], rk, 0, 0, 0);
      }
      if constexpr (FORM >= 2) asm("" : "+v"(bad));
    } else {
      const int a_ = k.c - 4 * p;
      double wa = 0.0;
      if (k.q == 0) wa = a_ == 0 ? i0 : (a_ == 1 ? w10 : (a_ == 2 ? w20 : (a_ == 3 ? w30 : 0.0)));
      if (k.q == 1) wa = a_ == 1 ? i1 : (a_ == 2 ? w21 : (a_ == 3 ? w31 : 0.0));
      if (k.q == 2) wa = a_ == 2 ? i2 : (a_ == 3 ? w32 : 0.0);
      if (k.q == 3) wa = a_ == 3 ? i3 : 0.0;
      const v4d nu = __builtin_amdgcn_mfma_f64_16x16x4f64(wa, Ud[p], z, 0, 0, 0);
      const v4d ny = __builtin_amdgcn_mfma_f64_16x16x4f64(wa, Yk[p], z, 0, 0, 0);
      const v4d nr = __builtin_amdgcn_mfma_f64_16x16x4f64(wa, rk[p], z, 0, 0, 0);
      Ud[p] = nu[p]; Yk[p] = ny[p]; rk[p] = nr[p];
      if (p < 3) {
        const double a = (k.c > 4 * p + 3) ? -Ud[p] : 0.0;
        Yk = __builtin_amdgcn_mfma_f64_16x16x4f64(a, Yk[p], Yk, 0, 0, 0);
        rk = __builtin_amdgcn_mfma_f64_16x16x4f64(a, rk[p], rk, 0, 0, 0);
        Ud = __builtin_amdgcn_mfma_f64_16x16x4f64(a, Ud[p], Ud, 0, 0, 0);
      }
    }
  }
#pragma unroll
  for (int p = 0; p < 4; ++p) if (k.c < k.q + 4 * p) Ud[p] = 0.0;
  return bad;
}

template <int T, int NB> struct DiagForm { static constexpr int form = (T == 5 && NB > 0) ? QP_DIAG_FLAT : 0; };

template <int T, int NB, int K> struct FactorStep {
  static DEVINL int run(const Ctx& k, v4d* acc, double* YL, double floor_abs) {
    v4d Yk, none = {0.0, 0.0, 0.0, 0.0};
#pragma unroll
    for (int p = 0; p < 4; ++p) Yk[p] = (k.q + 4 * p == k.c) ? 1.0 : 0.0;
    int bad = diag_factor<DiagForm<T, NB>::form>(k, acc[Tri<T>::idx(K, K)], Yk, none, floor_abs);
    tile_store(k, YL + K * 272, Yk);
    WAVE_SYNC();
    const v4d Wk = tile_load_t(k, YL + K * 272);
    const v4d& UKK = acc[Tri<T>::idx(K, K)];
#pragma unroll
    for (int Jt = K + 1; Jt < T; ++Jt) {
      v4d Rr = acc[Tri<T>::idx(K, Jt)];
      v4d Ukj = mfma4_new(Wk, Rr);
      mfma4_sub<T>(UKK, Ukj, Rr);
#pragma unroll
      for (int p = 0; p < 4; ++p) Ukj = __builtin_amdgcn_mfma_f64_16x16x4f64(Wk[p], Rr[p], Ukj, 0, 0, 0);
      acc[Tri<T>::idx(K, Jt)] = Ukj;
    }
#pragma unroll
    for (int I = K + 1; I < T; ++I) {
      const v4d& UKI = acc[Tri<T>::idx(K, I)];
#pragma unroll
      for (int Jt = I; Jt < T; ++Jt) mfma4_sub<T>(UKI, acc[Tri<T>::idx(K, Jt)], acc[Tri<T>::idx(I, Jt)]);
    }
    return bad | FactorStep<T, NB, K + 1>::run(k, acc, YL, floor_abs);
  }
};
template <int T, int NB> struct FactorStep<T, NB, T> {
  static DEVINL int run(const Ctx&, v4d*, double*, double) { return 0; }
};
template <int T, int NB> DEVINL int reg_factor(const Ctx& k, v4d* acc, double* YL, double floor_abs) {
  return FactorStep<T, NB, 0>::run(k, acc, YL, floor_abs);
}

template <int T, bool REFINE, int NV> DEVINL void vec_forward(const Ctx& k, const v4d* acc, const double* YL, const double* const (&B)[NV], double (&y)[NV][T][4]) {
#pragma unroll
  for (int K = 0; K < T; ++K) {
    double s[NV], t[NV];
#pragma unroll
    for (int v = 0; v < NV; ++v) {
      s[v] = 0.0;
#pragma unroll
      for (int I = 0; I < K; ++I)
#pragma unroll
        for (int p = 0; p < 4; ++p) s[v] = fma(acc[Tri<T>::idx(I, K)][p], y[v][I][p], s[v]);
    }
    if (K > 0) q_sum(s);
#pragma unroll
    for (int v = 0; v < NV; ++v) t[v] = B[v][16 * K + k.c] - (K > 0 ? s[v] : 0.0);
    const v4d Yt = tile_load(k, YL + K * 272);
    double yk[NV * 4];
#pragma unroll
    for (int v = 0; v < NV; ++v)
#pragma unroll
      for (int p = 0; p < 4; ++p) yk[4 * v + p] = Yt[p] * t[v];
    grp16_sum(yk);
    if (REFINE) {
      const v4d& U = acc[Tri<T>::idx(K, K)];
      double r[NV], dy[NV * 4];
#pragma unroll
      for (int v = 0; v < NV; ++v) {
        r[v] = 0.0;
#pragma unroll
        for (int p = 0; p < 4; ++p) r[v] = fma(U[p], yk[4 * v + p], r[v]);
      }
      q_sum(r);
#pragma unroll
      for (int v = 0; v < NV; ++v) {
        r[v] = t[v] - r[v];
#pragma unroll
        for (int p = 0; p < 4; ++p) dy[4 * v + p] = Yt[p] * r[v];
      }
      grp16_sum(dy);
#pragma unroll
      for (int i = 0; i < NV * 4; ++i) yk[i] += dy[i];
    }
#pragma unroll
    for (int v = 0; v < NV; ++v)
#pragma unroll
      for (int p = 0; p < 4; ++p) y[v][K][p] = yk[4 * v + p];
  }
}
template <int T, bool REFINE> DEVINL void vec_forward(const Ctx& k, const v4d* acc, const double* YL, const double* B, double (&y)[T][4]) {
  const double* const b1[1] = {B};
  vec_forward<T, REFINE, 1>(k, acc, YL, b1, reinterpret_cast<double (&)[1][T][4]>(y));
}
template <int T, bool REFINE, int NV> DEVINL void vec_backward(const Ctx& k, const v4d* acc, const double* YL, const double (&y)[NV][T][4], double* const (&X)[NV]) {
  double x[NV][T];
#pragma unroll
  for (int K = T - 1; K >= 0; --K) {
    const v4d Yt = tile_load(k, YL + K * 272);
    double w[NV * 4], s[NV * 4], s2[NV];
#pragma unroll
    for (int v = 0; v < NV; ++v)
#pragma unroll
      for (int p = 0; p < 4; ++p) {
        s[4 * v + p] = 0.0;
#pragma unroll
        for (int J = K + 1; J < T; ++J) s[4 * v + p] = fma(acc[Tri<T>::idx(K, J)][p], x[v][J], s[4 * v + p]);
      }
    if (K < T - 1) grp16_sum(s);
#pragma unroll
    for (int v = 0; v < NV; ++v) {
      s2[v] = 0.0;
#pragma unroll
      for (int p = 0; p < 4; ++p) {
        w[4 * v + p] = y[v][K][p] - (K < T - 1 ? s[4 * v + p] : 0.0);
        s2[v] = fma(Yt[p], w[4 * v + p], s2[v]);
      }
    }
    q_sum(s2);
#pragma unroll
    for (int v = 0; v < NV; ++v) x[v][K] = s2[v];
    if (REFINE) {
      const v4d& U = acc[Tri<T>::idx(K, K)];
      double d[NV], ux[NV * 4];
#pragma unroll
      for (int v = 0; v < NV; ++v)
#pragma unroll
        for (int p = 0; p < 4; ++p) ux[4 * v + p] = U[p] * x[v][K];
      grp16_sum(ux);
#pragma unroll
      for (int v = 0; v < NV; ++v) {
        d[v] = 0.0;
#pragma unroll
        for (int p = 0; p < 4; ++p) d[v] = fma(Yt[p], w[4 * v + p] - ux[4 * v + p], d[v]);
      }
      q_sum(d);
#pragma unroll
      for (int v = 0; v < NV; ++v) x[v][K] += d[v];
    }
#pragma unroll
    for (int v = 0; v < NV; ++v) if (k.q == 0) X[v][16 * K + k.c] = x[v][K];
  }
}
template <int T, bool REFINE> DEVINL void vec_backward(const Ctx& k, const v4d* acc, const double* YL, const double (&y)[T][4], double* X) {
  double* const x1[1] = {X};
  vec_backward<T, REFINE, 1>(k, acc, YL, reinterpret_cast<const double (&)[1][T][4]>(y), x1);
}
template <int T> DEVINL void vec_rows_store(const Ctx& k, const double (&y)[T][4], double* V) {
  if (k.c == 0) {
#pragma unroll
    for (int K = 0; K < T; ++K)
#pragma unroll
      for (int p = 0; p < 4; ++p) V[16 * K + k.q + 4 * p] = y[K][p];
  }
}
template <int T> DEVINL void vec_rows_load(const Ctx& k, const double* V, double (&y)[T][4]) {
#pragma unroll
  for (int K = 0; K < T; ++K)
#pragma unroll
    for (int p = 0; p < 4; ++p) y[K][p] = V[16 * K + k.q + 4 * p];
}

#ifndef QP_STAMPS
#define QP_STAMPS 0
#endif
#if QP_STAMPS
#define STAMP_DECL unsigned long long st_acc[16]; for (int i_ = 0; i_ < 16; ++i_) st_acc[i_] = 0; unsigned long long st_t0 = __builtin_amdgcn_s_memtime();
#define STAMP(id) do { __builtin_amdgcn_sched_barrier(0); unsigned long long t_ = __builtin_amdgcn_s_memtime(); st_acc[id] += t_ - st_t0; st_t0 = t_; __builtin_amdgcn_sched_barrier(0); } while (0)
#define STAMP_OUT do { if (P.dump && P.dump_stage == 9 && lane == 0) for (int i_ = 0; i_ < 16; ++i_) P.dump[(size_t)b * 16 + i_] = (double)st_acc[i_]; } while (0)
#else
#define STAMP_DECL
#define STAMP(id) do { } while (0)
#define STAMP_OUT do { } while (0)
#endif

#ifndef QP_REFINE_ATTEMPTS
#define QP_REFINE_ATTEMPTS 3
#endif
static_assert(V_NARR == QP_SOLVE_NVEC, "qp_solve_lds (qp_solver.h) counts the n-vectors");
template <int T> DEVINL double* ctx_setup(Ctx& k, const QpParams& P, int b, double* lds) {
  const QpDims& d = P.d;
  k.n = d.n; k.m = d.m; k.T = T; k.Kq = d.Kq; k.J = d.J; k.JB = d.JB; k.JT = d.J + d.JB; k.np = d.np;
  k.lane = threadIdx.x; k.c = k.lane & 15; k.q = k.lane >> 4; k.nc = d.nc; k.nb = d.nb;
  double* ws = P.ws + (size_t)b * d.ws_per_qp;
  k.Aw = ws + d.off_Aw; k.Hw = ws + d.off_Hw; k.Ab = ws + d.off_Ab; k.Hb = ws + d.off_Hb;
  k.rows = ws + d.off_rows; k.rowlen = d.rowlen; k.ntr = d.ntr;
  k.perm = reinterpret_cast<const int*>(ws + d.off_meta); k.tcs = k.perm + (size_t)(d.J > 0 ? d.J : 1) * 64;
  k.aoff = k.tcs + d.ntr; k.tend = k.aoff + d.ntr + 1;
  k.vec = lds;
  return ws;
}

template <int T, int NB> __global__ __launch_bounds__(64, 1) void qp_solve_kernel(QpParams P) {
  const int b = P.order ? P.order[blockIdx.x] : blockIdx.x;
  const QpDims& d = P.d;
  extern __shared__ double lds[];
  Ctx k;
  double* ws = ctx_setup<T>(k, P, b, lds);
  const QpSolveLds L = qp_solve_lds(T, NB, d.np);
  double* MB = lds + L.vecs;
  double* YL = MB + L.border;
  k.ring = YL + L.tiles;
  k.cof = k.ring + L.ring;
  const double* gw = ws + d.off_gw;
  const double* Es = ws + d.off_E;
  const double* Fs = ws + d.off_F;
  const int lane = k.lane, n = k.n, JT = k.JT, J = k.J, nc = k.nc, nb = k.nb;
  constexpr int NT = Tri<T>::NT;
  constexpr int NBB = NB > 0 ? NB : 1;

#define X vecp(k, V_X)
#define G vecp(k, V_G)
#define HX vecp(k, V_HX)
#define R1 vecp(k, V_R1)
#define R2 vecp(k, V_R2)
#define P1 vecp(k, V_P1)
#define P2 vecp(k, V_P2)
#define P3 vecp(k, V_P3)
#define DX vecp(k, V_DX)
#define EV vecp(k, V_E)
#define aL rowp(k, R_L)
#define aU rowp(k, R_U)
#define aTL rowp(k, R_TL)
#define aTU rowp(k, R_TU)
#define aZL rowp(k, R_ZL)
#define aZU rowp(k, R_ZU)
#define aV rowp(k, R_V)
#define aD rowp(k, R_D)
#define aW1 rowp(k, R_W1)
#define aW2 rowp(k, R_W2)
#define aW3 rowp(k, R_W3)
#define aVA rowp(k, R_VA)
#define aVC rowp(k, R_VC)
#define aRPL rowp(k, R_RPL)
#define aRPU rowp(k, R_RPU)

  auto hx_border = [&](const double* XV) __attribute__((always_inline)) {
    if (NB > 0) {
      WAVE_SYNC();
      double xb[NBB], sb[NBB];
#pragma unroll
      for (int e = 0; e < NB; ++e) { xb[e] = XV[nc + e]; sb[e] = 0.0; }
      for (int h = 0; h < 2; ++h) {
        const int i = lane + 64 * h;
        if (i < n) {
          double add = 0.0;
#pragma unroll
          for (int e = 0; e < NB; ++e) { const double hbi = k.Hb[(size_t)e * k.np + i]; add = fma(hbi, xb[e], add); sb[e] = fma(hbi, XV[i], sb[e]); }
          if (i < nc) HX[i] += add;
        }
      }
      wave_sum(sb);
#pragma unroll
      for (int e = 0; e < NB; ++e) if (lane == 0) HX[nc + e] = sb[e];
    }
  };
  auto hx_full = [&](const double* XV) __attribute__((always_inline)) { hx_tiles<T>(k, XV, HX); hx_border(XV); };

  Stream<T> st;
  st.open(k);

  for (int i = lane; i < k.np; i += 64) { G[i] = gw[i]; EV[i] = Es[i]; R1[i] = 0; R2[i] = 0; DX[i] = 0; }
  int cnt_local = 0, infeas = 0;
  for (int js = 0; js < JT; ++js) {
    const int ix = js * 64 + lane;
    const bool valid = row_valid(k, js);
    double l = aL[ix], u = aU[ix];
    if (valid) {
      if (l > -INFINITY && u < INFINITY) {
        if (l > u) infeas = 1;
        if (!(u > l)) {
          const double eps = 1e-9 * fmax(1.0, fabs(l));
          l -= eps; u += eps; aL[ix] = l; aU[ix] = u;
        }
      }
      cnt_local += (l > -INFINITY) + (u < INFINITY);
    }
    if (js >= J) {
      const int i = (js - J) * 64 + lane;
      if (i < k.np) {
        double xi = 0.0;
        if (P.x_init) { const int ui = i < k.n ? qp_user_index(d, i) : -1; if (ui >= 0) { const double xs = P.x_init[(size_t)b * d.nu + ui] / EV[i]; if (fabs(xs) < INFINITY) xi = xs; } }
        if (valid) { if (l > -INFINITY && xi < l) xi = l; if (u < INFINITY && xi > u) xi = u; }
        X[i] = xi;
      }
    }
  }
  const double cnt = fmax(1.0, wave_sum((double)cnt_local));
  infeas = wave_max((double)infeas) > 0;
  WAVE_SYNC();

  STAMP_DECL
  int flag = 1, it = 0, flag_polished = 0;
  double fval_s = 0.0, merit_s = INFINITY;
  if (infeas) { flag = -2; }
  if (ws[d.off_bad] != 0.0) flag = -1;

  {
    const double* vin[1] = {X}; double* rout[1] = {aV};
    pass_Av<T, NB, 1, 0>(k, st, vin, rout, nullptr);
    for (int jb = 0; jb < k.JB; ++jb) { const int i = jb * 64 + lane; aV[(J + jb) * 64 + lane] = i < n ? X[i] : 0.0; }
  }
  const double T0 = 10.0, Z0 = 100.0;
  for (int js = 0; js < JT; ++js) {
    const int ix = js * 64 + lane;
    const bool valid = row_valid(k, js);
    const double l = aL[ix], u = aU[ix], v = aV[ix];
    const bool hl = valid && l > -INFINITY, hu = valid && u < INFINITY;
    aTL[ix] = hl ? fmax(v - l, T0) : 1.0;
    aTU[ix] = hu ? fmax(u - v, T0) : 1.0;
    aZL[ix] = hl ? Z0 : 0.0;
    aZU[ix] = hu ? Z0 : 0.0;
    aW3[ix] = (js < J) ? ((hl ? Z0 : 0.0) - (hu ? Z0 : 0.0)) : 0.0;
  }
  WAVE_SYNC();
  {
    hx_full(X);
    pass_Atw<T, NB>(k, aW3, P3);
    WAVE_SYNC();
    for (int jb = 0; jb < k.JB; ++jb) {
      const int i = jb * 64 + lane, ix = (J + jb) * 64 + lane;
      if (i < n) {
        const double r = HX[i] + G[i] - P3[i];
        if (aL[ix] > -INFINITY) aZL[ix] = fmax(r, 0.0) + Z0;
        if (aU[ix] < INFINITY) aZU[ix] = fmax(-r, 0.0) + Z0;
      }
    }
    WAVE_SYNC();
  }

  double saved_merit = INFINITY, best_res = INFINITY;
  int have_saved = 0, stall = 0;
  double* XS = ws + d.off_save;
  double* LAMS = ws + d.off_save + k.np;

  auto row1_body = [&](int ix, bool valid, double l, double u, double v, double tl, double tu, double zl, double zu,
                       double& s_gap, double& m_rp) {
    const bool hl = valid && l > -INFINITY, hu = valid && u < INFINITY;
    const double rpl = hl ? v - l - tl : 0.0, rpu = hu ? u - v - tu : 0.0;
    const double dl_ = hl ? zl / tl : 0.0, du_ = hu ? zu / tu : 0.0;
    aRPL[ix] = rpl; aRPU[ix] = rpu;
    rowp(k, R_CB1)[ix] = dl_; rowp(k, R_CC1)[ix] = hl ? dl_ / tl : 0.0;
    rowp(k, R_CB2)[ix] = du_; rowp(k, R_CC2)[ix] = hu ? du_ / tu : 0.0;
    aD[ix] = dl_ + du_;
    aW1[ix] = -dl_ * rpl + du_ * rpu;
    aW2[ix] = (hl ? 1.0 / tl : 0.0) - (hu ? 1.0 / tu : 0.0);
    aW3[ix] = (hl ? zl : 0.0) - (hu ? zu : 0.0);
    s_gap += (hl ? tl * zl : 0.0) + (hu ? tu * zu : 0.0);
    const double sc = fmax(1.0, fabs(v));
    if (hl) m_rp = fmax(m_rp, fabs(rpl) / fmax(sc, fabs(l)));
    if (hu) m_rp = fmax(m_rp, fabs(rpu) / fmax(sc, fabs(u)));
  };
  struct Slot { int ix; bool valid; double l, u, v, tl, tu, zl, zu, va, vc, w2, rpl, rpu; };
  auto load_slot = [&](int js) {
    Slot s_;
    const int jc = js < JT ? js : JT - 1;
    s_.ix = jc * 64 + lane; s_.valid = js < JT && row_valid(k, jc);
    const int ix = s_.ix;
    s_.l = aL[ix]; s_.u = aU[ix]; s_.v = aV[ix]; s_.tl = aTL[ix]; s_.tu = aTU[ix]; s_.zl = aZL[ix]; s_.zu = aZU[ix];
    s_.va = aVA[ix]; s_.vc = aVC[ix]; s_.w2 = aW2[ix]; s_.rpl = aRPL[ix]; s_.rpu = aRPU[ix];
    return s_;
  };
  double gap = 0.0, rp_rel = 0.0;

  v4d acc[NT];
  double Ubb[NBB][NBB];
  auto border_solve = [&](double* R) __attribute__((always_inline)) {
    if (NB > 0) {
      double yb[NBB], xb[NBB], dsum[NBB];
#pragma unroll
      for (int e = 0; e < NB; ++e) {
        dsum[e] = 0.0;
        for (int h = 0; h < 2; ++h) { const int i = lane + 64 * h; if (i < nc) dsum[e] = fma(MB[e * k.np + i], R[i], dsum[e]); }
      }
      wave_sum(dsum);
#pragma unroll
      for (int e = 0; e < NB; ++e) {
        double tt = R[nc + e] - dsum[e];
#pragma unroll
        for (int g2 = 0; g2 < e; ++g2) tt -= Ubb[g2][e] * yb[g2];
        yb[e] = tt / Ubb[e][e];
      }
#pragma unroll
      for (int e = NB - 1; e >= 0; --e) {
        double tt = yb[e];
#pragma unroll
        for (int f = e + 1; f < NB; ++f) tt -= Ubb[e][f] * xb[f];
        xb[e] = tt / Ubb[e][e];
      }
      WAVE_SYNC();
      for (int h = 0; h < 2; ++h) {
        const int i = lane + 64 * h;
        if (i < nc) {
          double r = R[i];
#pragma unroll
          for (int e = 0; e < NB; ++e) r = fma(-MB[e * k.np + i], xb[e], r);
          R[i] = r;
        }
      }
      if (lane == 0) {
#pragma unroll
        for (int e = 0; e < NB; ++e) R[nc + e] = xb[e];
      }
      WAVE_SYNC();
    }
  };
  auto factor_solve2 = [&](int it_now) __attribute__((always_inline)) -> int {
    double dmax_l = 0;
#pragma unroll
    for (int K = 0; K < T; ++K) {
      const int i = 16 * K + k.c;
      const int ix = (J + (i >> 6)) * 64 + (i & 63);
      const double dadd = i < n ? aD[ix] : 1.0;
      const bool mine = (k.q == (k.c & 3));
#pragma unroll
      for (int p = 0; p < 4; ++p)
        if (mine && p == (k.c >> 2)) { acc[Tri<T>::idx(K, K)][p] += dadd; dmax_l = fmax(dmax_l, acc[Tri<T>::idx(K, K)][p]); }
    }
    if (NB > 0) {
      for (int h = 0; h < 2; ++h) {
        const int i = lane + 64 * h;
        if (i < k.np) {
          const int ix = (J + (i >> 6)) * 64 + (i & 63);
#pragma unroll
          for (int e = 0; e < NB; ++e) {
            double v = i < n ? k.Hb[(size_t)e * k.np + i] + MB[e * k.np + i] : 0.0;
            if (i == nc + e) { v += e < nb ? aD[ix] : 1.0; dmax_l = fmax(dmax_l, v); }
            MB[e * k.np + i] = v;
          }
        }
      }
    }
    const double dmax = wave_max(dmax_l);
    WAVE_SYNC();
#ifdef QP_DEBUG_DUMP
    if (P.dump && b == 0 && P.dump_stage == 1 && it_now == P.dump_iter) {
#pragma unroll
      for (int I = 0; I < T; ++I)
#pragma unroll
        for (int Jt = I; Jt < T; ++Jt)
#pragma unroll
          for (int p = 0; p < 4; ++p) {
            const int r = 16 * I + k.q + 4 * p, cc = 16 * Jt + k.c;
            if (r < n && cc < n) { P.dump[r * n + cc] = acc[Tri<T>::idx(I, Jt)][p]; if (I != Jt || cc >= r) P.dump[cc * n + r] = acc[Tri<T>::idx(I, Jt)][p]; }
          }
      for (int e = 0; e < nb; ++e)
        for (int i = lane; i < n; i += 64) { P.dump[i * n + nc + e] = MB[e * k.np + i]; P.dump[(nc + e) * n + i] = MB[e * k.np + i]; }
      for (int i = lane; i < n; i += 64) { P.dump[n * n + i] = P1[i]; P.dump[n * n + n + i] = P2[i]; P.dump[n * n + 2 * n + i] = P3[i]; P.dump[n * n + 3 * n + i] = HX[i]; }
    }
#endif
    int fbad = reg_factor<T, NB>(k, acc, YL, 1e-30 * dmax);
    WAVE_SYNC();
    STAMP(5);
    if (NB > 0) {
#pragma unroll
      for (int e = 0; e < NB; ++e) {
        double ue[T][4];
        vec_forward<T, true>(k, acc, YL, MB + e * k.np, ue);
        WAVE_SYNC();
        vec_rows_store<T>(k, ue, MB + e * k.np);
      }
      WAVE_SYNC();
      double S[NBB][NBB], ss[NBB * (NBB + 1) / 2];
#pragma unroll
      for (int e = 0, j = 0; e < NB; ++e)
#pragma unroll
        for (int f = e; f < NB; ++f, ++j) {
          double dsum = 0.0;
          for (int h = 0; h < 2; ++h) { const int i = lane + 64 * h; if (i < nc) dsum = fma(MB[e * k.np + i], MB[f * k.np + i], dsum); }
          ss[j] = dsum;
        }
      wave_sum(ss);
#pragma unroll
      for (int e = 0, j = 0; e < NB; ++e)
#pragma unroll
        for (int f = e; f < NB; ++f, ++j) S[e][f] = MB[e * k.np + nc + f] - ss[j];
#pragma unroll
      for (int e = 0; e < NB; ++e) {
        double dd = S[e][e];
#pragma unroll
        for (int g2 = 0; g2 < e; ++g2) dd -= Ubb[g2][e] * Ubb[g2][e];
        if (!(dd > 1e-30 * dmax)) { if (!(fabs(dd) < INFINITY)) fbad = 1; dd = 1e-30 * dmax; }
        Ubb[e][e] = sqrt(dd);
#pragma unroll
        for (int f = e + 1; f < NB; ++f) {
          double tt = S[e][f];
#pragma unroll
          for (int g2 = 0; g2 < e; ++g2) tt -= Ubb[g2][e] * Ubb[g2][f];
          Ubb[e][f] = tt / Ubb[e][e];
        }
      }
    }
    if (fbad) return 1;
    {
      double y12[2][T][4];
      double (&y1)[T][4] = y12[0], (&y2)[T][4] = y12[1];
#if QP_SOLVE_PAIR
      { const double* const b12[2] = {R1, R2}; vec_forward<T, true, 2>(k, acc, YL, b12, y12); }
#else
      vec_forward<T, true>(k, acc, YL, R1, y1);
      vec_forward<T, true>(k, acc, YL, R2, y2);
#endif
      if (NB > 0) {
        WAVE_SYNC();
        vec_rows_store<T>(k, y1, R1); vec_rows_store<T>(k, y2, R2);
        WAVE_SYNC();
        border_solve(R1); border_solve(R2);
        vec_rows_load<T>(k, R1, y1); vec_rows_load<T>(k, R2, y2);
      }
      WAVE_SYNC();
#if QP_SOLVE_PAIR
      { double* const x12[2] = {R1, R2}; vec_backward<T, true, 2>(k, acc, YL, y12, x12); }
#else
      vec_backward<T, true>(k, acc, YL, y1, R1);
      vec_backward<T, true>(k, acc, YL, y2, R2);
#endif
    }
    WAVE_SYNC();
    return 0;
  };
  auto solve1 = [&](double* V) __attribute__((always_inline)) {
    double yv[T][4];
    vec_forward<T, false>(k, acc, YL, V, yv);
    if (NB > 0) {
      WAVE_SYNC();
      vec_rows_store<T>(k, yv, V);
      WAVE_SYNC();
      border_solve(V);
      vec_rows_load<T>(k, V, yv);
    }
    WAVE_SYNC();
    vec_backward<T, false>(k, acc, YL, yv, V);
  };

  STAMP(0);
  for (it = 0; flag == 1; ++it) {
    if (it == 0) {
      double s_gap = 0, m_rp = 0;
      for (int js = 0; js < JT; ++js) {
        const int ix = js * 64 + lane;
        row1_body(ix, row_valid(k, js), aL[ix], aU[ix], aV[ix], aTL[ix], aTU[ix], aZL[ix], aZU[ix], s_gap, m_rp);
      }
      gap = wave_sum(s_gap);
      rp_rel = wave_max(m_rp);
      WAVE_SYNC();
    }
    const double mu = gap / cnt;

    STAMP(1);
    acc_init<T>(k, acc);
    hx_from_acc<T>(k, acc, X, HX);
    hx_border(X);
    STAMP(2);
    pass_syrk<T, NB>(k, st, acc, P1, P2, P3, MB);
    WAVE_SYNC();
    STAMP(3);
    double fl = 0, m_rd = 0;
    for (int h = 0; h < 2; ++h) {
      const int i = lane + 64 * h;
      if (i < n) {
        const int ix = (J + (i >> 6)) * 64 + (i & 63);
        const double gz = P3[i] + aW3[ix];
        fl += 0.5 * X[i] * HX[i] + G[i] * X[i];
        const double sc = fmax(1.0, fmax(fabs(G[i]), fmax(fabs(HX[i]), fabs(gz))));
        m_rd = fmax(m_rd, fabs(HX[i] + G[i] - gz) / sc);
      }
    }
    const double fval = wave_sum(fl);
    const double rd_rel = wave_max(m_rd);
    const double gap_rel = gap / fmax(1.0, fabs(fval));
    const double merit = (fabs(fval) < INFINITY && fabs(gap_rel) < INFINITY) ? fmax(rd_rel, fmax(rp_rel, gap_rel)) : INFINITY;
    fval_s = fval; merit_s = merit;
    const bool res_ok = merit <= P.tol;
#ifdef QP_DEBUG_DUMP
    if (P.dump && P.dump_stage == 5 && b == P.dump_iter && lane == 0 && it < 120) {
      double* o_ = P.dump + 16 * it;
      o_[0] = merit; o_[1] = rd_rel; o_[2] = rp_rel; o_[3] = gap_rel; o_[4] = mu; o_[5] = fval; o_[6] = (double)have_saved; o_[7] = saved_merit;
    }
#endif
    if (!(merit < INFINITY)) { flag = have_saved ? 2 : -1; break; }
    if (merit <= P.tol_loose && merit < saved_merit) {
      for (int i = lane; i < k.np; i += 64) XS[i] = X[i];
      for (int js = 0; js < JT; ++js) LAMS[js * 64 + lane] = aW3[js * 64 + lane];
      have_saved = 1; saved_merit = merit;
    } else if (merit > P.tol_loose && rp_rel <= P.tol_loose && gap_rel <= P.tol_loose) {
      double dgap = 0, m_rd2 = 0, lamfix[2] = {0.0, 0.0};
      for (int h = 0; h < 2; ++h) {
        const int i = lane + 64 * h;
        if (i < n) {
          const int ix = (J + (i >> 6)) * 64 + (i & 63);
          const double lam = aW3[ix], gz = P3[i] + lam, r = HX[i] + G[i] - gz;
          const double lam2 = lam + r, l = aL[ix], u = aU[ix], v = aV[ix];
          const bool ok = lam2 >= 0 ? l > -INFINITY : u < INFINITY;
          if (ok) { lamfix[h] = lam2; dgap += fabs(r) * fmax(0.0, lam2 >= 0 ? v - l : u - v); }
          else {
            lamfix[h] = lam;
            const double sc = fmax(1.0, fmax(fabs(G[i]), fmax(fabs(HX[i]), fabs(gz))));
            m_rd2 = fmax(m_rd2, fabs(r) / sc);
          }
        }
      }
      const double merit2 = fmax(wave_max(m_rd2), fmax(rp_rel, (gap + wave_sum(dgap)) / fmax(1.0, fabs(fval))));
      if (merit2 <= P.tol_loose && merit2 < saved_merit) {
        for (int i = lane; i < k.np; i += 64) XS[i] = X[i];
        for (int js = 0; js < J; ++js) LAMS[js * 64 + lane] = aW3[js * 64 + lane];
        for (int h = 0; h < 2; ++h) { const int i = lane + 64 * h; if (i < k.np) LAMS[(J + (i >> 6)) * 64 + (i & 63)] = i < n ? lamfix[h] : 0.0; }
        have_saved = 1; saved_merit = merit2;
      }
      if (have_saved) { flag = 2; break; }
    } else if (have_saved && merit > P.tol_loose) { flag = 2; break; }
    if (merit < 0.9 * best_res) { best_res = merit; stall = 0; } else ++stall;

    for (int h = 0; h < 2; ++h) {
      const int i = lane + 64 * h;
      if (i < k.np) {
        const int ix = (J + (i >> 6)) * 64 + (i & 63);
        R1[i] = i < n ? -(HX[i] + G[i]) + P1[i] + aW1[ix] : 0.0;
        R2[i] = i < n ? P2[i] + aW2[ix] : 0.0;
      }
    }
    STAMP(4);
// ... 527 lines not shown
```

### fsae-mpc_amd/csrc/qp_solver.h

```cpp
#pragma once
#include <hip/hip_runtime.h>
#include <stddef.h>

#define QP_MAX_T 12
#ifndef QP_WG_W
#define QP_WG_W 8
#endif
#define QP_BREAKDOWN_TRY_TOL 1e-4

enum RowArr { R_L = 0, R_U, R_TL, R_TU, R_ZL, R_ZU, R_V, R_D, R_W1, R_W2, R_W3, R_VA, R_VC, R_RPL, R_RPU, R_CB1, R_CC1, R_CB2, R_CC2, R_NARR };

struct QpDims {
  int n, m;
  int T, np;
  int nb, NB, nc;
  int Kq, ntr;
  int prep_tw;
  int J, JB;
  int nu;
  int rowlen;
  size_t off_Aw, off_meta, off_Hw, off_gw, off_E, off_F, off_Ab, off_Hb, off_rows, off_save, off_bad, ws_per_qp;
  size_t lds_solve, lds_prep;
  int W;
  int NBk;
  size_t wg_ring;
  size_t lds_wg;
  size_t off_U;
};

struct QpParams {
  QpDims d;
  const double *H, *g, *A, *lb, *ub, *lbA, *ubA;
  double* ws;
  double *x, *fval, *lambda;
  int *exitflag, *iter;
  double tol, tol_loose, tol_x, inf_bound;
  int max_iter, shared_HA, polish;
  int* polished;
  double* kkt;
  double* dump; int dump_stage, dump_iter;
  const double* x_init;
  int* score;
  const int* score_in;
  int* order;
};
#define QP_ORDER_MIN_BATCH 256
inline size_t qp_order_bytes(int batch) { return batch > QP_ORDER_MIN_BATCH ? (((size_t)2 * batch * sizeof(int)) + 255) & ~(size_t)255 : 0; }

#define QP_NO_SLACK_HINT (-1)
void qp_make_dims(int n, int m, QpDims* d, int n_slack = QP_NO_SLACK_HINT);
__host__ __device__ inline int qp_user_index(const QpDims& d, int i) { const int ncu = d.nu - d.nb; return i < ncu ? i : (i >= d.nc && d.nb > 0 ? ncu + (i - d.nc) : (i < d.nu && d.nb == 0 ? i : -1)); }
__host__ __device__ inline int qp_solver_index(const QpDims& d, int u) { const int ncu = d.nu - d.nb; return (d.nb > 0 && u >= ncu) ? d.nc + (u - ncu) : u; }
bool qp_runs_wavefront_kernel(const QpDims& d);
hipError_t qp_launch(const QpParams& P, int batch, hipStream_t st, hipEvent_t ev_mid = nullptr);
int qp_selftest_mfma(char* msg, int msglen);
int qp_selftest_lane_reduce(char* msg, int msglen);
int qp_selftest_diag_factor(char* msg, int msglen);
#define QP_SOLVE_NVEC 10
#define QP_SOLVE_RING(T) (3 * (T))
struct QpSolveLds {
  size_t vecs, border, tiles, ring, cof;
  __host__ __device__ size_t total() const { return vecs + border + tiles + ring + cof; }
};
__host__ __device__ inline QpSolveLds qp_solve_lds(int T, int NB, int np) {
  return {(size_t)QP_SOLVE_NVEC * np, (size_t)(NB > 0 ? NB : 1) * np, (size_t)T * 272, (size_t)QP_SOLVE_RING(T) * 128, (size_t)(6 + NB) * 64};
}
#define QP_WG_NVEC_FIXED 14
inline size_t qp_wg_lds_base_bytes(const QpDims& d, int W, int NBk) {
  const size_t part2 = (size_t)W * d.np;
  const size_t extra = (size_t)240 * d.T > part2 ? (size_t)240 * d.T : part2;
  return ((size_t)(QP_WG_NVEC_FIXED + 2 * NBk) * d.np + (size_t)d.T * 272 + (size_t)d.T * 256 + 256 + (size_t)W * 96 +
          (size_t)2 * 8 * W + (size_t)W * 6 * 64 + (size_t)3 * (16 + 256) + 16 + extra + (size_t)(3 * d.ntr / 2 + 2)) * sizeof(double);
}
```

### fsae-mpc_amd/csrc/qp_solver.hip

```cpp
#include <hip/hip_runtime.h>
#include <math.h>
#include <stdint.h>
#include <stdlib.h>
#include <stdio.h>
#include "qp_solver.h"
#include "qp_lane.h"

#if !defined(QP_TU) || QP_TU == 0
#define QP_MAIN_TU 1
#else
#define QP_MAIN_TU 0
#endif
#include "qp_solve_kernel.h"

#if QP_MAIN_TU
namespace {

__global__ __launch_bounds__(1024) void qp_prep_kernel(QpParams P) {
  const int b = blockIdx.x, tid = threadIdx.x, w = tid >> 6, lane = tid & 63, c = lane & 15, q = lane >> 4;
  const int NTH = blockDim.x, NW = NTH >> 6;
  const QpDims& d = P.d;
  const int n = d.n, nu = d.nu, m = d.m, T = d.T, Kq = d.Kq, J = d.J, JB = d.JB, np = d.np, nc = d.nc, nb = d.nb;
  const double* H = P.H + (P.shared_HA ? 0 : (size_t)b * nu * nu);
  const double* A = P.A + (P.shared_HA ? 0 : (size_t)b * m * nu);
  const double* g = P.g + (size_t)b * nu;
  auto U = [&](int i) { return qp_user_index(d, i); };
  auto Hat = [&](int i, int j) -> double { const int ui = U(i), uj = U(j); return (ui >= 0 && uj >= 0) ? H[(size_t)uj * nu + ui] : ((i == j && i < n) ? 1.0 : 0.0); };
  auto Aat = [&](int r, int j) -> double { const int uj = U(j); return uj >= 0 ? A[(size_t)uj * m + r] : 0.0; };
  double* ws = P.ws + (size_t)b * d.ws_per_qp;
  double* Aw = ws + d.off_Aw;
  double* Hw = ws + d.off_Hw;
  double* gw = ws + d.off_gw;
  double* Es = ws + d.off_E;
  double* Fs = ws + d.off_F;
  double* Ab = ws + d.off_Ab;
  double* Hb = ws + d.off_Hb;
  int* perm_g = reinterpret_cast<int*>(ws + d.off_meta);
  int* tcs_g = perm_g + (size_t)(J > 0 ? J : 1) * 64;
  int* aoff_g = tcs_g + d.ntr;
  int* tend_g = aoff_g + d.ntr + 1;
  const int ntr = d.ntr;
  double* Lr = ws + d.off_rows + 0 * (size_t)d.rowlen;
  double* Ur = ws + d.off_rows + 1 * (size_t)d.rowlen;
  extern __shared__ double lds[];
  double* Esh = lds;
  double* red = lds + np;
  double* tile = red + 16;
  const int TW = d.prep_tw;
  int* cls_sh = reinterpret_cast<int*>(tile + TW * (4 * Kq + 1));
  int* perm_sh = cls_sh + 4 * Kq;
  int* cnt_sh = perm_sh + 16 * ntr;
  int* tcs_sh = cnt_sh + 16;
  int* aoff_sh = tcs_sh + ntr;
  int* chc_sh = aoff_sh + ntr + 1;
  double* Fr_sh = reinterpret_cast<double*>((reinterpret_cast<uintptr_t>(chc_sh + ((m + 63) >> 6) * 16) + 7) & ~(uintptr_t)7);

  for (int j = tid; j < np; j += NTH) {
    double e = 1.0;
    if (j < n) {
      double hjj = Hat(j, j);
      if (hjj > 1e-12) e = 1.0 / sqrt(hjj);
      else e = -1.0;
    } else e = 0.0;
    Esh[j] = e;
  }
  __syncthreads();
  for (int j = 0; j < n; ++j) {
    if (Esh[j] < 0) {
      double cm = 0;
      for (int r = tid; r < m; r += NTH) cm = fmax(cm, fabs(Aat(r, j)));
      cm = wave_max_zf(cm);
      if (lane == 0) red[w] = cm;
      __syncthreads();
      if (tid == 0) { double mx = 0.0; for (int i = 0; i < NW; ++i) mx = fmax(mx, red[i]); Esh[j] = mx > 1e-12 ? 1.0 / mx : 1.0; }
      __syncthreads();
    }
  }
  int bad = 0;
  for (int j = tid; j < np; j += NTH) { const int uj = j < n ? U(j) : -1; const double gj = uj >= 0 ? g[uj] : 0.0; Es[j] = Esh[j]; gw[j] = gj * Esh[j]; bad |= !(fabs(gj) < INFINITY); }

  __syncthreads();
  const int ncols = nc < n ? nc : n;
  const int nchunk = (m + 63) >> 6;
  for (int i = tid; i < nchunk * 16; i += NTH) chc_sh[i] = 0;
  if (tid < 16) cnt_sh[tid] = 0;
  __syncthreads();
  for (int r0 = 0; r0 < m; r0 += NTH) {
    const int r = r0 + tid;
    int e = 0;
    double rm = 0.0;
    if (r < m) {
      for (int col0 = 0; col0 < n; col0 += 8) {
        double av[8];
#pragma unroll
        for (int u = 0; u < 8; ++u) av[u] = col0 + u < n ? Aat(r, col0 + u) : 0.0;
#pragma unroll
        for (int u = 0; u < 8; ++u) {
          const int col = col0 + u;
          const double a = fabs(av[u]);
          if (col < n) { rm = fmax(rm, a * Esh[col]); if (a != 0.0 && col < ncols) e = col >> 4; }
        }
      }
      cls_sh[r] = e;
      Fr_sh[r] = rm > 1e-12 ? 1.0 / rm : 1.0;
    }
    for (int cl = 0; cl < T; ++cl) {
      const unsigned long long mk = __ballot(r < m && e == cl);
      if (lane == 0 && r0 + 64 * w < m) chc_sh[((r0 >> 6) + w) * 16 + cl] = __popcll(mk);
    }
  }
  __syncthreads();
  if (tid < T) {
    int tot = 0;
    for (int ch = 0; ch < nchunk; ++ch) tot += chc_sh[ch * 16 + tid];
    cnt_sh[tid] = tot;
  }
  __syncthreads();
  if (tid < T) {
    int start = 0;
    for (int cl = 0; cl < tid; ++cl) start += cnt_sh[cl];
    for (int ch = 0; ch < nchunk; ++ch) { const int cn = chc_sh[ch * 16 + tid]; chc_sh[ch * 16 + tid] = start; start += cn; }
  }
  for (int p = tid; p < 16 * ntr; p += NTH) perm_sh[p] = -1;
  __syncthreads();
  for (int r0 = 0; r0 < m; r0 += NTH) {
    const int r = r0 + tid;
    const int e = r < m ? cls_sh[r] : -1;
    for (int cl = 0; cl < T; ++cl) {
      const unsigned long long mk = __ballot(e == cl);
      if (e == cl) perm_sh[chc_sh[((r0 >> 6) + w) * 16 + cl] + __popcll(mk & ((1ull << lane) - 1ull))] = r;
    }
  }
  __syncthreads();
  for (int tr = tid; tr < ntr; tr += NTH) {
    int tc = 1;
    for (int p = 16 * tr; p < 16 * tr + 16; ++p) { const int r = perm_sh[p]; if (r >= 0) tc = max(tc, cls_sh[r] + 1); }
    tcs_sh[tr] = tc;
  }
  __syncthreads();
  if (tid == 0) {
    int run = 0;
    for (int tr = 0; tr < ntr; ++tr) { aoff_sh[tr] = run; run += 2 * tcs_sh[tr]; }
    aoff_sh[ntr] = run;
    for (int C = 0; C <= T; ++C) { int cn = 0; for (int tr = 0; tr < ntr; ++tr) cn += (tcs_sh[tr] <= C); tend_g[C] = cn; }
  }
  __syncthreads();
  for (int tr = tid; tr <= ntr; tr += NTH) { aoff_g[tr] = aoff_sh[tr]; if (tr < ntr) tcs_g[tr] = tcs_sh[tr]; }

  int nexcl = 0;
  for (int js = w; js < J; js += NW) {
    const int s = 16 * js + c, pp = 4 * s + q;
    const int r = (s < 4 * ntr) ? perm_sh[pp] : -1;
    const bool valid = r >= 0;
    const double f = valid ? Fr_sh[r] : 0.0;
    Fs[js * 64 + lane] = f;
    perm_g[js * 64 + lane] = r;
    for (int bb = 0; bb < 4; ++bb)
    { const double v = (valid && bb < nb) ? Aat(r, nc + bb) * Esh[nc + bb] * f : 0.0; bad |= !(fabs(v) < INFINITY); Ab[(size_t)bb * J * 64 + js * 64 + lane] = v; }
    double l = -INFINITY, u = INFINITY;
    if (valid) {
      double lr = P.lbA[(size_t)b * m + r], ur = P.ubA[(size_t)b * m + r];
      bad |= (lr != lr) || (ur != ur);
      nexcl += (lr > 0.0) || (ur < 0.0);
      l = lr > -P.inf_bound ? lr * f : -INFINITY;
      u = ur < P.inf_bound ? ur * f : INFINITY;
    }
    Lr[js * 64 + lane] = l;
    Ur[js * 64 + lane] = u;
  }
  for (int jb = w; jb < JB; jb += NW) {
    const int i = jb * 64 + lane;
    double l = -INFINITY, u = INFINITY;
    const int ui = i < n ? U(i) : -1;
    if (ui >= 0) {
      double lr = P.lb[(size_t)b * nu + ui], ur = P.ub[(size_t)b * nu + ui];
      bad |= (lr != lr) || (ur != ur);
      nexcl += (lr > 0.0) || (ur < 0.0);
      l = lr > -P.inf_bound ? lr / Esh[i] : -INFINITY;
      u = ur < P.inf_bound ? ur / Esh[i] : INFINITY;
    }
    Lr[(J + jb) * 64 + lane] = l;
    Ur[(J + jb) * 64 + lane] = u;
  }
  __syncthreads();

  const int R4 = 4 * Kq, mp1 = R4 + 1;
  for (int t = 0; t < T; ++t)
    for (int c0 = 0; c0 < 16; c0 += TW) {
      for (int e = tid; e < TW * R4; e += NTH) {
        const int cc = e / R4, r = e - cc * R4;
        const int col = 16 * t + c0 + cc;
        double v = 0.0;
        if (col < nc && col < n && r < m) v = Aat(r, col) * Esh[col];
        bad |= !(fabs(v) < INFINITY);
        tile[cc * mp1 + r] = v;
      }
      __syncthreads();
      for (int s = w; s < 4 * ntr; s += NW) {
        const int tr = s >> 2, tc = tcs_sh[tr];
        if (t < tc && c >= c0 && c < c0 + TW) {
          const int r = perm_sh[4 * s + q];
          const double v = r >= 0 ? tile[(c - c0) * mp1 + r] * Fr_sh[r] : 0.0;
          Aw[((size_t)aoff_sh[tr] + ((s >> 1) & 1) * tc + t) * 128 + lane * 2 + (s & 1)] = v;
        }
      }
      __syncthreads();
    }

  for (int idx = w; idx < T * T * 4; idx += NW) {
    const int p = idx & 3, IJ = idx >> 2, I = IJ / T, Jt = IJ - I * T;
    const int row = 16 * I + q + 4 * p, col = 16 * Jt + c;
    double v = 0.0;
    if (row < nc && col < nc && row < n && col < n) v = Hat(col, row) * Esh[row] * Esh[col];
    bad |= !(fabs(v) < INFINITY);
    Hw[(size_t)idx * 64 + lane] = v;
  }
  for (int e = tid; e < 4 * np; e += NTH) {
    const int bb = e / np, i = e - bb * np;
    const double v = (bb < nb && i < n) ? Hat(i, nc + bb) * Esh[nc + bb] * Esh[i] : 0.0;
    bad |= !(fabs(v) < INFINITY);
    Hb[e] = v;
  }
  bad = __syncthreads_or(bad);
  if (tid == 0) ws[d.off_bad] = bad ? 1.0 : 0.0;
  if (P.score) {
    __shared__ int score_sh;
    if (tid == 0) score_sh = 0;
    __syncthreads();
    if (nexcl) atomicAdd(&score_sh, nexcl);
    __syncthreads();
    if (tid == 0) P.score[b] = P.score_in ? P.score_in[b] : score_sh;
  }
}

__global__ __launch_bounds__(1024) void qp_order_kernel(const int* __restrict__ score, int* __restrict__ order, int batch) {
  constexpr int NBIN = 1024, NWV = 8;
  __shared__ int cnt[NWV][NBIN], scan[NBIN];
  const int tid = threadIdx.x, w = tid >> 6, lane = tid & 63;
  for (int e = tid; e < NWV * NBIN; e += 1024) (&cnt[0][0])[e] = 0;
  __syncthreads();
  const int per = ((batch + NWV - 1) / NWV + 63) & ~63;
  const int lo = w * per, hi = min(batch, lo + per);
  auto bin = [&](int i) { return NBIN - 1 - min(max(score[i], 0), NBIN - 1); };
  auto group = [&](int k, bool on, int& rank, int& size) {
    unsigned long long same = __builtin_amdgcn_ballot_w64(on);
#pragma unroll
    for (int bit = 0; bit < 10; ++bit) {
      const bool one = (k >> bit) & 1;
      const unsigned long long v = __builtin_amdgcn_ballot_w64(one);
      same &= one ? v : ~v;
    }
    rank = __popcll(same & ((1ull << lane) - 1ull)); size = __popcll(same);
  };
  if (w < NWV)
    for (int i0 = lo; i0 < hi; i0 += 512) {
      int kv[8];
#pragma unroll
      for (int r = 0; r < 8; ++r) { const int i = i0 + 64 * r + lane; kv[r] = i < hi ? bin(i) : -1; }
#pragma unroll
      for (int r = 0; r < 8; ++r) {
        const bool on = kv[r] >= 0; const int k = on ? kv[r] : 0;
        int rank, size; group(k, on, rank, size);
        if (on && rank == 0) cnt[w][k] += size;
      }
    }
  __syncthreads();
  int v = 0;
  for (int ww = 0; ww < NWV; ++ww) v += cnt[ww][tid];
  scan[tid] = v;
  __syncthreads();
  for (int o = 1; o < NBIN; o <<= 1) {
    const int a = tid >= o ? scan[tid - o] : 0;
    __syncthreads();
    scan[tid] += a;
    __syncthreads();
  }
  int run = scan[tid] - v;
  for (int ww = 0; ww < NWV; ++ww) { const int c = cnt[ww][tid]; cnt[ww][tid] = run; run += c; }
  __syncthreads();
  if (w < NWV)
    for (int i0 = lo; i0 < hi; i0 += 512) {
      int kv[8];
#pragma unroll
      for (int r = 0; r < 8; ++r) { const int i = i0 + 64 * r + lane; kv[r] = i < hi ? bin(i) : -1; }
#pragma unroll
      for (int r = 0; r < 8; ++r) {
        const bool on = kv[r] >= 0; const int k = on ? kv[r] : 0;
        int rank, size; group(k, on, rank, size);
        int base = on ? cnt[w][k] : 0;
        if (on) order[base + rank] = i0 + 64 * r + lane;
        if (on && rank == 0) cnt[w][k] = base + size;
      }
    }
}

}

#include "qp_selftest.h"
#ifdef QP_PROBE
#include "qp_probe.h"
#endif

void qp_make_dims(int n, int m, QpDims* d, int n_slack) {
  d->n = n; d->nu = n; d->m = m;
  const int rem = n % 16;
  if (n >= 16 && rem >= 1 && rem <= 4) { d->T = n / 16; d->nb = rem; } else { d->T = (n + 15) / 16; d->nb = 0; }
  if (n_slack >= 0) {
    d->T = (n - n_slack + 15) / 16; d->nb = n_slack;
    if (n_slack > 0) d->n = 16 * d->T + n_slack;
  } else if (d->nb == 0 && n >= 20) {
    const char* sb = getenv("FSAEMPC_SLACK_BORDER");
    const int ns = (m == 10 * (n - 4) && ((n - 4) % 2) == 0) ? 4 : ((m == 3 * (n - 1) && ((n - 1) % 2) == 0) ? 1 : 0);
    const int Tp = (n - ns + 15) / 16;
    const bool pays = !(sb && sb[0] == '1') || Tp < d->T || Tp >= 6;
    if (ns > 0 && pays && !(sb && sb[0] == '0') && Tp <= QP_MAX_T) {
      d->T = Tp; d->nb = ns;
      d->n = 16 * d->T + ns;
    }
  }
  n = d->n;
  d->NB = d->nb == 0 ? 0 : (d->nb == 1 ? 1 : 4);
  d->nc = 16 * d->T;
  d->np = d->nc + (d->nb ? 16 : 0);
  d->Kq = (m + 3) / 4;
  d->J = (d->Kq + 15) / 16;
  d->JB = (d->np + 63) / 64;
  d->rowlen = (d->J + d->JB) * 64;
  size_t off = 0;
  d->ntr = (d->Kq + 3) / 4;
  d->off_Aw = off; off += (size_t)(2 * d->ntr) * d->T * 128;
  d->off_meta = off; off += ((size_t)(d->J > 0 ? d->J : 1) * 64 + 2 * (size_t)d->ntr + 1 + 16 + 1) / 2 + 1;
  off = (off + 1) & ~(size_t)1;
  d->off_Hw = off; off += (size_t)d->T * d->T * 4 * 64;
  d->off_gw = off; off += d->np;
  d->off_E = off; off += d->np;
  d->off_F = off; off += (size_t)(d->J > 0 ? d->J : 1) * 64;
  d->off_Ab = off; off += (size_t)4 * (d->J > 0 ? d->J : 1) * 64;
  d->off_Hb = off; off += (size_t)4 * d->np;
  d->off_rows = off; off += (size_t)R_NARR * d->rowlen;
  d->off_save = off; off += d->np + d->rowlen;
  d->off_bad = off; off += 2;
  off = (off + 1) & ~(size_t)1;
  d->off_U = off; off += (size_t)(d->T * (d->T + 1) / 2) * 256;
  off = (off + 63) & ~(size_t)63;
  d->ws_per_qp = off;
  d->lds_solve = qp_solve_lds(d->T, d->NB, d->np).total() * sizeof(double);
  {
    d->W = QP_WG_W;
    d->NBk = d->nb == 0 ? 0 : 4;
    d->wg_ring = 1;
    d->lds_wg = qp_wg_lds_base_bytes(*d, d->W, d->NBk);
  }
  d->prep_tw = 16;
  for (;;) {
    d->lds_prep = ((size_t)d->np + 16 + (size_t)d->prep_tw * (4 * d->Kq + 1) + (size_t)m + 2) * sizeof(double) +
                  ((size_t)4 * d->Kq + 16 * (size_t)d->ntr + 16 + 2 * (size_t)d->ntr + 1 + (size_t)((m + 63) / 64) * 16 + 6) * sizeof(int);
    if (d->lds_prep <= 96 * 1024 || d->prep_tw == 2) break;
    d->prep_tw >>= 1;
  }
}

#endif

#if defined(QP_TU)
hipError_t qp_launch_solve_g1(const QpParams& P, int batch, hipStream_t st);
hipError_t qp_launch_solve_g2(const QpParams& P, int batch, hipStream_t st);
hipError_t qp_launch_solve_g3(const QpParams& P, int batch, hipStream_t st);
hipError_t qp_launch_solve_g4(const QpParams& P, int batch, hipStream_t st);
#if QP_TU == 1
hipError_t qp_launch_solve_g1(const QpParams& P, int batch, hipStream_t st) {
  switch (P.d.T) {
    case 1: return launch_solve_T<1>(P, batch, st);
    case 2: return launch_solve_T<2>(P, batch, st);
    case 3: return launch_solve_T<3>(P, batch, st);
    case 4: return launch_solve_T<4>(P, batch, st);
    default: return hipErrorInvalidValue;
  }
}
#elif QP_TU == 2
hipError_t qp_launch_solve_g2(const QpParams& P, int batch, hipStream_t st) { return launch_solve_T<5>(P, batch, st); }
#elif QP_TU == 3
hipError_t qp_launch_solve_g3(const QpParams& P, int batch, hipStream_t st) { return launch_solve_T<6>(P, batch, st); }
#elif QP_TU == 4
hipError_t qp_launch_solve_g4(const QpParams& P, int batch, hipStream_t st) { return launch_solve_T<7>(P, batch, st); }
#endif
#endif

#if QP_MAIN_TU
#define QP_V1_MAX_T 7
static bool qp_use_wavefront_kernel(const QpDims& d) {
  return d.T <= QP_V1_MAX_T;
}
bool qp_runs_wavefront_kernel(const QpDims& d) {
  static const char* force = getenv("FSAEMPC_QP_KERNEL");
  return d.T <= QP_V1_MAX_T && ((force && force[0] == 'v') || (!(force && force[0] == 'w') && qp_use_wavefront_kernel(d)));
}
hipError_t qp_wg_launch_1(const QpParams& P, int batch, hipStream_t st);
hipError_t qp_wg_launch_6(const QpParams& P, int batch, hipStream_t st);
hipError_t qp_wg_launch_7(const QpParams& P, int batch, hipStream_t st);
hipError_t qp_wg_launch_8(const QpParams& P, int batch, hipStream_t st);
hipError_t qp_wg_launch_9(const QpParams& P, int batch, hipStream_t st);
hipError_t qp_wg_launch_10(const QpParams& P, int batch, hipStream_t st);
hipError_t qp_wg_launch_11(const QpParams& P, int batch, hipStream_t st);
hipError_t qp_wg_launch_12(const QpParams& P, int batch, hipStream_t st);
static hipError_t qp_wg_launch(const QpParams& P, int batch, hipStream_t st) {
  switch (P.d.T) {
    case 1: case 2: case 3: case 4: case 5: return qp_wg_launch_1(P, batch, st);
    case 6: return qp_wg_launch_6(P, batch, st);
    case 7: return qp_wg_launch_7(P, batch, st);
    case 8: return qp_wg_launch_8(P, batch, st);
    case 9: return qp_wg_launch_9(P, batch, st);
    case 10: return qp_wg_launch_10(P, batch, st);
    case 11: return qp_wg_launch_11(P, batch, st);
    case 12: return qp_wg_launch_12(P, batch, st);
  }
  return hipErrorInvalidValue;
}
static int prep_thr() { static const char* e = getenv("FSAEMPC_PREP_THR"); return e ? atoi(e) : 256; }
hipError_t qp_launch(const QpParams& P, int batch, hipStream_t st, hipEvent_t ev_mid) {
  hipError_t e = hipFuncSetAttribute(reinterpret_cast<const void*>(&qp_prep_kernel),
                                     hipFuncAttributeMaxDynamicSharedMemorySize, (int)P.d.lds_prep);
  if (e != hipSuccess) return e;
  hipLaunchKernelGGL(qp_prep_kernel, dim3(batch), dim3(P.d.m > prep_thr() ? 1024 : 256), P.d.lds_prep, st, P);
  e = hipGetLastError();
  if (e != hipSuccess) return e;
  if (P.order) {
    hipLaunchKernelGGL(qp_order_kernel, dim3(1), dim3(1024), 0, st, P.score, P.order, batch);
    e = hipGetLastError();
    if (e != hipSuccess) return e;
  }
  if (ev_mid) { e = hipEventRecord(ev_mid, st); if (e != hipSuccess) return e; }
#ifdef QP_PROBE
  if (P.dump && P.dump_stage == 7 && P.d.T == 5) {
    (void)hipFuncSetAttribute(reinterpret_cast<const void*>(&factor_probe_kernel<5>), hipFuncAttributeMaxDynamicSharedMemorySize, (int)P.d.lds_solve);
    hipLaunchKernelGGL((factor_probe_kernel<5>), dim3(batch), dim3(64), P.d.lds_solve, st, P, 8);
    return hipGetLastError();
  }
  if (P.dump && P.dump_stage == 8 && P.d.T == 5 && P.d.NB == 1) {
    (void)hipFuncSetAttribute(reinterpret_cast<const void*>(&syrk_probe_kernel<5, 1>), hipFuncAttributeMaxDynamicSharedMemorySize, (int)P.d.lds_solve);
    hipLaunchKernelGGL((syrk_probe_kernel<5, 1>), dim3(batch), dim3(64), P.d.lds_solve, st, P, 16);
    hipLaunchKernelGGL(overlap_probe_kernel, dim3(batch), dim3(64), 0, st, P.dump + 2 * (size_t)batch, 2048);
    return hipGetLastError();
  }
#endif
  if (!qp_runs_wavefront_kernel(P.d)) return qp_wg_launch(P, batch, st);
#if !defined(QP_TU)
  switch (P.d.T) {
#if defined(QP_ONLY_T)
    case QP_ONLY_T: return launch_solve_T<QP_ONLY_T>(P, batch, st);
#else
    case 1: return launch_solve_T<1>(P, batch, st);
    case 2: return launch_solve_T<2>(P, batch, st);
    case 3: return launch_solve_T<3>(P, batch, st);
    case 4: return launch_solve_T<4>(P, batch, st);
    case 5: return launch_solve_T<5>(P, batch, st);
    case 6: return launch_solve_T<6>(P, batch, st);
    case 7: return launch_solve_T<7>(P, batch, st);
#endif
    default: return hipErrorInvalidValue;
  }
#else
  switch (P.d.T) {
    case 1: case 2: case 3: case 4: return qp_launch_solve_g1(P, batch, st);
    case 5: return qp_launch_solve_g2(P, batch, st);
    case 6: return qp_launch_solve_g3(P, batch, st);
    case 7: return qp_launch_solve_g4(P, batch, st);
    default: return hipErrorInvalidValue;
  }
#endif
}

#endif
```

### include/fsaempc.h

```cpp
#ifndef FSAEMPC_H
#define FSAEMPC_H

#ifdef __cplusplus
extern "C" {
#endif

#define FSAEMPC_ERR_ARG      (-1)
#define FSAEMPC_ERR_DIM      (-2)
#define FSAEMPC_ERR_HIP      (-3)
#define FSAEMPC_ERR_NODEVICE (-4)
#define FSAEMPC_ERR_WORKSPACE (-5)
#define FSAEMPC_ERR_SOLVER   (-6)

#define FSAEMPC_MAX_NV 196

#define FSAEMPC_MODEL_KINEMATIC 0
#define FSAEMPC_MODEL_DYNAMIC   1

typedef struct {
  double tol;
  double tol_loose;
  double tol_x;
  double inf_bound;
  int    max_iter;
// ... 51 lines not shown
                                  const fsaempc_qp_opts* opts,
                                  double* x, double* fval, int* exitflag, int* iter, double* lambda);
int fsaempc_seq_equality(int handle, int nV, int nC, const double* g, const double* lb, const double* ub,
                         const double* lbA, const double* ubA, int k, const fsaempc_qp_opts* opts,
                         double* x, double* lambda, int* workingSetB, int* workingSetC);
int fsaempc_seq_cleanup(int handle);

#define FSAEMPC_VJP_OK 0
#define FSAEMPC_VJP_WEAK 1
#define FSAEMPC_VJP_INTERIOR 2
#define FSAEMPC_VJP_SINGULAR (-1)
#define FSAEMPC_VJP_FORWARD_FAILED (-2)

typedef struct {
  const double* xbar;
  const double* fbar;
  double* gbar;
  double* lbbar;
  double* ubbar;
  double* lbAbar;
  double* ubAbar;
  double* Hbar;
  double* Abar;
} fsaempc_qp_vjp_io;

long long fsaempc_qp_vjp_workspace_bytes(const fsaempc_qp_desc* desc);

int fsaempc_qp_vjp_batch_device(const fsaempc_qp_desc* desc, int k,
                                const double* H, const double* g, const double* A,
                                const double* lb, const double* ub, const double* lbA, const double* ubA,
                                const double* x, const double* lambda, const int* exitflag, const int* polished,
                                const fsaempc_qp_opts* opts, const fsaempc_qp_vjp_io* io, int* status,
                                void* workspace, long long workspace_bytes, void* stream);


typedef struct {
  int M;
  double dl;
  const double* xP;
  const double* yP;
} fsaempc_spline;

#define FSAEMPC_INT_DEFAULT (-1)
#define FSAEMPC_INT_EULER 0
#define FSAEMPC_INT_RK2   1
#define FSAEMPC_INT_RK4   2

typedef struct {
  int model;
  int N;
  int batch;
  double dt;
  int integrator;
} fsaempc_ltv_desc;

int fsaempc_ltv_nx(int model);
int fsaempc_ltv_nV(int model, int N);
int fsaempc_ltv_nC(int model, int N);

int fsaempc_ltv_build_qp_batch_device(const fsaempc_ltv_desc* desc, const fsaempc_spline* sp,
                                      const double* x0, const double* x_ref, const double* x_lin, const double* u_lin,
                                      double* H, double* g, double* A, double* lb, double* ub, double* lbA, double* ubA,
                                      double* pred, double* Bt, double* qconst, void* stream);

long long fsaempc_ltv_workspace_bytes(const fsaempc_ltv_desc* desc);

int fsaempc_ltv_step_batch_device(const fsaempc_ltv_desc* desc, const fsaempc_spline* sp,
                                  const double* x0, const double* x_ref, const double* x_lin, const double* u_lin,
                                  const fsaempc_qp_opts* opts,
                                  double* u_opt, double* x_opt, double* slack, double* fval, int* exitflag, int* iter,
                                  void* workspace, long long workspace_bytes, void* stream);

int fsaempc_ltv_step_batch_device_aux(const fsaempc_ltv_desc* desc, const fsaempc_spline* sp,
                                      const double* x0, const double* x_ref, const double* x_lin, const double* u_lin,
                                      const fsaempc_qp_opts* opts,
                                      double* u_opt, double* x_opt, double* slack, double* fval, int* exitflag, int* iter,
                                      const fsaempc_qp_aux* aux,
                                      void* workspace, long long workspace_bytes, void* stream);

int fsaempc_ltv_affine_maps_batch_device(const fsaempc_ltv_desc* desc, const fsaempc_spline* sp, const double* x_lin, const double* u_lin,
                                         double* Abar, double* Crow, void* stream);

int fsaempc_ltv_step_batch_device_lambda(const fsaempc_ltv_desc* desc, const fsaempc_spline* sp,
                                         const double* x0, const double* x_ref, const double* x_lin, const double* u_lin,
                                         const fsaempc_qp_opts* opts, double* u_opt, double* x_opt, double* slack, double* fval,
                                         int* exitflag, int* iter, double* lambda, const fsaempc_qp_aux* aux,
                                         void* workspace, long long workspace_bytes, void* stream);

typedef struct {
  const double* ubar;
  const double* xbar;
  const double* sbar;
  const double* fbar;
  double* x0bar;
  double* xrefbar;
} fsaempc_ltv_vjp_io;

long long fsaempc_ltv_step_vjp_workspace_bytes(const fsaempc_ltv_desc* desc, int k);

int fsaempc_ltv_step_vjp_batch_device(const fsaempc_ltv_desc* desc, const fsaempc_spline* sp, int k,
                                      const double* x0, const double* x_ref, const double* x_lin, const double* u_lin,
                                      const double* u_opt, const double* slack, const double* lambda, const int* exitflag, const int* polished,
                                      const fsaempc_qp_opts* opts, const fsaempc_ltv_vjp_io* io, int* status,
                                      void* workspace, long long workspace_bytes, void* stream);

int fsaempc_nlp_build_qp_batch_device(const fsaempc_ltv_desc* desc, const fsaempc_spline* sp,
                                      const double* x0, const double* x_ref, const double* u_lin,
                                      double* H, double* g, double* A, double* lb, double* ub, double* lbA, double* ubA,
                                      double* pred, double* Bt, double* qconst, void* stream);

typedef struct {
  int max_sweeps;
  int trials;
  double tol_step;
  double tol_feas;
  double armijo;
  double rho0;
  int warm_start;
} fsaempc_sqp_opts;

void fsaempc_sqp_default_opts(fsaempc_sqp_opts* o);

typedef struct {
  double* lambda;
  int* qp_iter;
  double* step_norm;
  double* hard_viol;
  double* merit;
} fsaempc_sqp_aux;

long long fsaempc_sqp_workspace_bytes(const fsaempc_ltv_desc* desc);

int fsaempc_sqp_batch_device(const fsaempc_ltv_desc* desc, const fsaempc_spline* sp,
                             const double* x0, const double* x_ref, const double* u_init,
                             const fsaempc_qp_opts* qp_opts, const fsaempc_sqp_opts* sqp_opts,
                             double* u_opt, double* x_opt, double* slack, double* fval, int* status, int* sweeps,
                             const fsaempc_sqp_aux* aux, void* workspace, long long workspace_bytes, void* stream);

int fsaempc_sqp_get_timing(double* build_ms, double* solve_ms, double* linesearch_ms, double* compact_ms);


int fsaempc_obtain_reference_batch_device(const double* plan, double ds, int N_s, const double* t,
                                          const double* s0, double dt, int N_t, int batch,
                                          double* x_ref, void* stream);

int fsaempc_reference_live_batch_device(int nx, int N, double dt, double target_vel, int batch,
                                        const double* x0, double* x_ref, void* stream);


int fsaempc_cl_pre_batch_device(int model, int N, double dt, double target_vel, double L, const fsaempc_spline* sp,
                                const double* cart, const double* s_guess, int batch,
                                double* x0, double* x_ref, int* finished, void* stream);

int fsaempc_cl_plant_batch_device(int model, int N, double dt, int batch, double* cart, double* pid, const double* x_opt,
                                  const int* finished, const int* exitflag, double* u_last, void* stream);

int fsaempc_cl_accept_batch_device(int model, int N, int batch, const double* x_new, const double* u_new, const int* exitflag,
                                   double* x_keep, double* u_keep, void* stream);

#define FSAEMPC_NPAR 32
#define FSAEMPC_P_M            0
#define FSAEMPC_P_IZ           1
#define FSAEMPC_P_LF           2
#define FSAEMPC_P_LR           3
#define FSAEMPC_P_GRAV         4
#define FSAEMPC_P_PB           5
#define FSAEMPC_P_PC           6
#define FSAEMPC_P_PD           7
#define FSAEMPC_P_PE           8
#define FSAEMPC_P_Q_S          9
#define FSAEMPC_P_Q_N          10
#define FSAEMPC_P_Q_MU         11
#define FSAEMPC_P_Q_TERMINAL   12
#define FSAEMPC_P_R_ACC        13
#define FSAEMPC_P_R_STEER      14
#define FSAEMPC_P_R_SOFT0      15
#define FSAEMPC_P_R_SOFT1      16
#define FSAEMPC_P_R_SOFT2      17
#define FSAEMPC_P_R_SOFT3      18
#define FSAEMPC_P_U_ACC_MAX    19
#define FSAEMPC_P_U_STEER_MAX  20
#define FSAEMPC_P_DELTA_MAX    21
#define FSAEMPC_P_N_MAX        22
#define FSAEMPC_P_V_MIN        23
#define FSAEMPC_P_ALAT_MAX     24
#define FSAEMPC_P_SLIP_MAX     25
#define FSAEMPC_P_ELL_LONG     26
#define FSAEMPC_P_ELL_LAT      27
#define FSAEMPC_P_PID_KP_V     28
#define FSAEMPC_P_PID_MAX_F    29
#define FSAEMPC_P_PID_KP_D     30
#define FSAEMPC_P_PID_MAX_DRATE 31

typedef struct {
  const double* values;
  int per_instance;
} fsaempc_ltv_params;

int fsaempc_ltv_default_params(int model, double* out);

int fsaempc_ltv_build_qp_batch_device_p(const fsaempc_ltv_desc* desc, const fsaempc_spline* sp, const fsaempc_ltv_params* par,
                                        const double* x0, const double* x_ref, const double* x_lin, const double* u_lin,
                                        double* H, double* g, double* A, double* lb, double* ub, double* lbA, double* ubA,
                                        double* pred, double* Bt, double* qconst, void* stream);
int fsaempc_ltv_step_batch_device_p(const fsaempc_ltv_desc* desc, const fsaempc_spline* sp, const fsaempc_ltv_params* par,
                                    const double* x0, const double* x_ref, const double* x_lin, const double* u_lin,
                                    const fsaempc_qp_opts* opts, double* u_opt, double* x_opt, double* slack, double* fval,
                                    int* exitflag, int* iter, double* lambda, const fsaempc_qp_aux* aux,
                                    void* workspace, long long workspace_bytes, void* stream);
int fsaempc_nlp_build_qp_batch_device_p(const fsaempc_ltv_desc* desc, const fsaempc_spline* sp, const fsaempc_ltv_params* par,
                                        const double* x0, const double* x_ref, const double* u_lin,
                                        double* H, double* g, double* A, double* lb, double* ub, double* lbA, double* ubA,
                                        double* pred, double* Bt, double* qconst, void* stream);
int fsaempc_sqp_batch_device_p(const fsaempc_ltv_desc* desc, const fsaempc_spline* sp, const fsaempc_ltv_params* par,
                               const double* x0, const double* x_ref, const double* u_init,
                               const fsaempc_qp_opts* qp_opts, const fsaempc_sqp_opts* sqp_opts,
                               double* u_opt, double* x_opt, double* slack, double* fval, int* status, int* sweeps,
                               const fsaempc_sqp_aux* aux, void* workspace, long long workspace_bytes, void* stream);
int fsaempc_cl_plant_batch_device_p(int model, int N, double dt, int batch, const fsaempc_ltv_params* par, double* cart, double* pid,
                                    const double* x_opt, const int* finished, const int* exitflag, double* u_last, void* stream);

typedef struct {
  const double* table;
  const double* t;
  int N_s; double ds;
  int per_instance;
} fsaempc_plan;
#define FSAEMPC_PLAN_MAX_NS 4096

int fsaempc_plan_profile_batch_device(int model, const fsaempc_spline* sp, double L, const fsaempc_ltv_params* par,
                                      int n_plans, int N_s, double v_cap, double grip,
                                      double* table, double* t, void* stream);

int fsaempc_plan_reference_batch_device(int model, const fsaempc_plan* plan, const double* s0, double dt, int N, int batch,
                                        double* x_ref, void* stream);

int fsaempc_cl_pre_plan_batch_device(int model, int N, double dt, double L, const fsaempc_spline* sp, const fsaempc_plan* plan,
                                     const double* cart, const double* s_guess, int batch,
                                     double* x0, double* x_ref, int* finished, void* stream);

#define FSAEMPC_LINE_MAX_NS 2048
#define FSAEMPC_LINE_MIN_NC 8

int fsaempc_raceline_build_qp_device(const fsaempc_spline* sp, double L, int N_s, int N_c, double* H, double* g, void* stream);

int fsaempc_plan_line_profile_batch_device(int model, const fsaempc_spline* sp, double L, const fsaempc_ltv_params* par,
                                           int n_plans, int N_s, int N_c, const double* line, int line_per_plan,
                                           double v_cap, double grip, double* table, double* t, void* stream);

long long fsaempc_plan_raceline_workspace_bytes(int n_plans, int N_c);
int fsaempc_plan_raceline_batch_device(int model, const fsaempc_spline* sp, double L, const fsaempc_ltv_params* par,
                                       int n_plans, int N_s, int N_c, double margin, double v_cap, double grip,
                                       const fsaempc_qp_opts* opts, double* line, int* flag, double* table, double* t,
                                       void* workspace, long long workspace_bytes, void* stream);

typedef struct {
  int n_blocks;
  const int* len;
} fsaempc_ltv_blocking;

int fsaempc_ltv_blocked_nV(int model, const fsaempc_ltv_blocking* blk);
int fsaempc_ltv_build_qp_batch_device_b(const fsaempc_ltv_desc* desc, const fsaempc_spline* sp, const fsaempc_ltv_params* par,
                                        const fsaempc_ltv_blocking* blk,
                                        const double* x0, const double* x_ref, const double* x_lin, const double* u_lin,
                                        double* H, double* g, double* A, double* lb, double* ub, double* lbA, double* ubA,
                                        double* pred, double* Bt, double* qconst, void* stream);
long long fsaempc_ltv_workspace_bytes_b(const fsaempc_ltv_desc* desc, const fsaempc_ltv_blocking* blk);
int fsaempc_ltv_step_batch_device_b(const fsaempc_ltv_desc* desc, const fsaempc_spline* sp, const fsaempc_ltv_params* par,
                                    const fsaempc_ltv_blocking* blk,
                                    const double* x0, const double* x_ref, const double* x_lin, const double* u_lin,
                                    const fsaempc_qp_opts* opts, double* u_opt, double* x_opt, double* slack, double* fval,
                                    int* exitflag, int* iter, double* lambda, const fsaempc_qp_aux* aux,
                                    void* workspace, long long workspace_bytes, void* stream);

long long fsaempc_qp_workspace_bytes_s(const fsaempc_qp_desc* desc, int n_slack);
int fsaempc_qp_solve_batch_device_s(const fsaempc_qp_desc* desc, int n_slack,
                                    const double* H, const double* g, const double* A,
                                    const double* lb, const double* ub, const double* lbA, const double* ubA,
                                    const fsaempc_qp_opts* opts,
                                    double* x, double* fval, int* exitflag, int* iter, double* lambda,
                                    const fsaempc_qp_aux* aux,
                                    void* workspace, long long workspace_bytes, void* stream);
int fsaempc_qp_layout(const fsaempc_qp_desc* desc, int n_slack, int out[4]);


typedef struct {
  int M;
  double dl, L;
  double* xP;
  double* yP;
} fsaempc_track;

int fsaempc_track_from_csv(const char* path, int M, fsaempc_track* out);
int fsaempc_track_from_points(const double* x, const double* y, int n, int M, fsaempc_track* out);
void fsaempc_track_free(fsaempc_track* t);
int fsaempc_track_save(const fsaempc_track* t, const char* path);
int fsaempc_track_load(const char* path, fsaempc_track* out);
const char* fsaempc_track_last_error(void);

const char* fsaempc_last_error(void);
int fsaempc_selftest_mfma(void);
int fsaempc_selftest_lane_reduce(void);
int fsaempc_selftest_diag_factor(void);
int fsaempc_debug_set_dump(double* out, int stage);

int fsaempc_qp_set_timing(int enable);
int fsaempc_qp_get_timing(double* prep_ms, double* solve_ms);
int fsaempc_ltv_get_timing(double* build_ms, double* prep_ms, double* solve_ms, double* post_ms);

#ifdef __cplusplus
}
#endif
#endif
```

Baseline: 417,300.

## Fuse startup A^T w into initial Av pass and batch prep-kernel loads

```diff
diff --git a/fsae-mpc_amd/_lib.py b/fsae-mpc_amd/_lib.py
--- a/fsae-mpc_amd/_lib.py
+++ b/fsae-mpc_amd/_lib.py
@@ -7,7 +7,7 @@
 EXPORTS = [
     "fsaempc_qp_default_opts", "fsaempc_qp_workspace_bytes", "fsaempc_qp_solve_batch_device", "fsaempc_qp_solve_batch",
     "fsaempc_ltv_nx", "fsaempc_ltv_nV", "fsaempc_ltv_nC", "fsaempc_ltv_build_qp_batch_device",
-    "fsaempc_ltv_workspace_bytes", "fsaempc_ltv_step_batch_device", "fsaempc_ltv_step_batch_device_aux", "fsaempc_last_error", "fsaempc_selftest_mfma", "fsaempc_selftest_lane_reduce", "fsaempc_selftest_diag_factor",
+    "fsaempc_ltv_workspace_bytes", "fsaempc_ltv_step_batch_device", "fsaempc_ltv_step_batch_device_aux", "fsaempc_last_error", "fsaempc_selftest_mfma", "fsaempc_selftest_lane_reduce", "fsaempc_selftest_diag_factor", "fsaempc_selftest_initial_point",
     "fsaempc_debug_set_dump", "fsaempc_qp_solve_batch_device_aux", "fsaempc_qp_set_timing", "fsaempc_qp_get_timing", "fsaempc_ltv_get_timing",
     "fsaempc_seq_init", "fsaempc_seq_hotstart", "fsaempc_seq_hotstart_matrices", "fsaempc_seq_equality", "fsaempc_seq_cleanup",
     "fsaempc_obtain_reference_batch_device", "fsaempc_reference_live_batch_device",
diff --git a/fsae-mpc_amd/csrc/capi.hip b/fsae-mpc_amd/csrc/capi.hip
--- a/fsae-mpc_amd/csrc/capi.hip
+++ b/fsae-mpc_amd/csrc/capi.hip
@@ -1093,6 +1093,16 @@
   return bad;
 }
 
+int fsaempc_selftest_initial_point(void) {
+  int cnt = 0;
+  hipError_t e = hipGetDeviceCount(&cnt);
+  if (e != hipSuccess || cnt == 0) return fail(FSAEMPC_ERR_NODEVICE, "no HIP device");
+  char msg[256] = "";
+  int bad = qp_selftest_initial_point(msg, sizeof(msg));
+  if (bad != 0) snprintf(g_err, sizeof(g_err), "%s", msg);
+  return bad;
+}
+
 int fsaempc_debug_set_dump(double* out, int stage) { g_dump.store(out); g_dump_stage.store(stage); return 0; }
 
 int fsaempc_qp_set_timing(int enable) {
diff --git a/fsae-mpc_amd/csrc/qp_selftest.h b/fsae-mpc_amd/csrc/qp_selftest.h
--- a/fsae-mpc_amd/csrc/qp_selftest.h
+++ b/fsae-mpc_amd/csrc/qp_selftest.h
@@ -143,6 +143,57 @@
   }
   if (bad) {
     if (atomicAdd(&out[0], bad) == 0) { out[1] = first; out[2] = form; out[3] = k.lane; }
+  }
+}
+
+template <int T, int NB> __global__ __launch_bounds__(64) void initial_point_selftest_kernel(QpParams P, int* __restrict__ out) {
+  extern __shared__ double lds[];
+  Ctx k;
+  (void)ctx_setup<T>(k, P, 0, lds);
+  const QpSolveLds L = qp_solve_lds(T, NB, P.d.np);
+  k.ring = lds + L.vecs + L.border + L.tiles;
+  k.cof = k.ring + L.ring;
+  const int lane = k.lane, J = k.J, JT = k.JT;
+  double* Xv = vecp(k, V_X); double* P3o = vecp(k, V_P1); double* P3n = vecp(k, V_P3);
+  double* W3 = rowp(k, R_W3); double* Vo = rowp(k, R_VA); double* Vn = rowp(k, R_V);
+  const double* Lb = rowp(k, R_L); const double* Ub = rowp(k, R_U);
+  Stream<T> st;
+  st.open(k);
+  for (int js = 0; js < JT; ++js) {
+    const int ix = js * 64 + lane;
+    const bool valid = row_valid(k, js);
+    const double l = Lb[ix], u = Ub[ix];
+    W3[ix] = (valid && js < J) ? ((l > -INFINITY ? 100.0 : 0.0) - (u < INFINITY ? 100.0 : 0.0)) : 0.0;
+    if (js >= J) {
+      const int i = (js - J) * 64 + lane;
+      if (i < k.np) {
+        double xi = i < k.n ? 0.375 * ((i * 7) % 5 - 2) + 0.01 * i : 0.0;
+        if (valid) { if (l > -INFINITY && xi < l) xi = l; if (u < INFINITY && xi > u) xi = u; }
+        Xv[i] = xi;
+      }
+    }
+  }
+  WAVE_SYNC();
+  const double* vin[1] = {Xv};
+  { double* rout[1] = {Vo}; pass_Av<T, NB, 1, 0>(k, st, vin, rout, nullptr); }
+  pass_Atw<T, NB>(k, W3, P3o);
+  WAVE_SYNC();
+  { double* rout[1] = {Vn}; pass_Av<T, NB, 1, -1>(k, st, vin, rout, P3n); }
+  WAVE_SYNC();
+  st.close();
+  int bad = 0, kind = -1, at = -1, nz = 0;
+  for (int js = 0; js < J; ++js) {
+    const int ix = js * 64 + lane;
+    if (!same_bits(Vo[ix], Vn[ix])) { if (!bad) { kind = 0; at = ix; } ++bad; }
+    nz += Vo[ix] != 0.0;
+  }
+  for (int i = lane; i < k.nc + NB; i += 64) {
+    if (!same_bits(P3o[i], P3n[i])) { if (!bad) { kind = 1; at = i; } ++bad; }
+    nz += P3o[i] != 0.0;
+  }
+  if (nz) atomicAdd(&out[4], nz);
+  if (bad) {
+    if (atomicAdd(&out[0], bad) == 0) { out[1] = kind; out[2] = at; out[3] = lane; }
   }
 }
 
@@ -248,3 +299,94 @@
   if (hout[0]) snprintf(msg, msglen, "diag_factor forms: %d mismatches with the former form, first: tile %d form %d lane %d", hout[0], hout[1], hout[2], hout[3]);
   return hout[0];
 }
+
+template <int T, int NB> static hipError_t initial_point_launch(const QpParams& P, int* dout) {
+  hipError_t e = hipFuncSetAttribute(reinterpret_cast<const void*>(&initial_point_selftest_kernel<T, NB>), hipFuncAttributeMaxDynamicSharedMemorySize, (int)P.d.lds_solve);
+  if (e != hipSuccess) return e;
+  hipLaunchKernelGGL((initial_point_selftest_kernel<T, NB>), dim3(1), dim3(64), P.d.lds_solve, 0, P, dout);
+  return hipGetLastError();
+}
+static int initial_point_shape(int nV, int nC, char* msg, int msglen) {
+  QpDims d;
+  qp_make_dims(nV, nC, &d);
+  const int nb = d.nb, ncu = nV - nb;
+  const double inf = 1e20;
+  const size_t nH = (size_t)nV * nV, nA = (size_t)nC * nV, nin = nH + nA + 3 * (size_t)nV + 2 * (size_t)nC;
+  double* h = (double*)calloc(nin, sizeof(double));
+  if (!h) return -1;
+  double *H = h, *A = H + nH, *g = A + nA, *lb = g + nV, *ub = lb + nV, *lbA = ub + nV, *ubA = lbA + nC;
+  unsigned long long st = 0xA0761D6478BD642Full + (unsigned)nV * 1000003u + (unsigned)nC;
+  auto rnd = [&]() { st = st * 6364136223846793005ull + 1442695040888963407ull; return ((unsigned)(st >> 33)) / 2147483648.0; };
+  for (int j = 0; j < nV; ++j) {
+    for (int i = 0; i < j; ++i) if ((i + j) % 3 == 0) { const double v = 0.1 * (rnd() - 0.5); H[(size_t)j * nV + i] = v; H[(size_t)i * nV + j] = v; }
+    H[(size_t)j * nV + j] = (nb > 0 && j == nV - 1) ? 0.0 : 1.0 + 3.0 * rnd();
+    g[j] = 2.0 * rnd() - 1.0;
+  }
+  for (int r = 0; r < nC; ++r) {
+    const int reach = ncu > 0 ? 1 + (int)(((long long)(r + 1) * ncu) / nC) : 0;
+    for (int j = 0; j < ncu && j < reach; ++j) if ((r + j) % 4 != 1) A[(size_t)j * nC + r] = 4.0 * rnd() - 2.0;
+    for (int j = ncu; j < nV; ++j) A[(size_t)j * nC + r] = -1.0 + 0.5 * rnd();
+    const double mid = rnd() - 0.5;
+    switch (r % 5) {
+      case 0: lbA[r] = mid - 1.0; ubA[r] = mid + 1.0; break;
+      case 1: lbA[r] = mid; ubA[r] = 1e30; break;
+      case 2: lbA[r] = -1e30; ubA[r] = mid; break;
+      case 3: lbA[r] = mid; ubA[r] = mid; break;
+      default: lbA[r] = -1e30; ubA[r] = 1e30; break;
+    }
+  }
+  for (int j = 0; j < nV; ++j) {
+    switch (j % 4) {
+      case 0: lb[j] = -1.0; ub[j] = 1.0; break;
+      case 1: lb[j] = 0.25; ub[j] = 1e30; break;
+      case 2: lb[j] = -1e30; ub[j] = -0.125; break;
+      default: lb[j] = -1e30; ub[j] = 1e30; break;
+    }
+  }
+  double *din = 0, *ws = 0; int* dout = 0; int hout[5] = {0, 0, 0, 0, 0};
+  hipError_t e = hipMalloc(&din, sizeof(double) * nin);
+  if (e == hipSuccess) e = hipMalloc(&ws, sizeof(double) * d.ws_per_qp);
+  if (e == hipSuccess) e = hipMalloc(&dout, sizeof(hout));
+  if (e == hipSuccess) e = hipMemcpy(din, h, sizeof(double) * nin, hipMemcpyHostToDevice);
+  if (e == hipSuccess) e = hipMemset(ws, 0, sizeof(double) * d.ws_per_qp);
+  if (e == hipSuccess) e = hipMemset(dout, 0, sizeof(hout));
+  free(h);
+  if (e == hipSuccess) {
+    QpParams P = {};
+    P.d = d;
+    P.H = din; P.A = din + nH; P.g = P.A + nA; P.lb = P.g + nV; P.ub = P.lb + nV; P.lbA = P.ub + nV; P.ubA = P.lbA + nC;
+    P.ws = ws; P.inf_bound = inf;
+    e = hipFuncSetAttribute(reinterpret_cast<const void*>(&qp_prep_kernel), hipFuncAttributeMaxDynamicSharedMemorySize, (int)d.lds_prep);
+    if (e == hipSuccess) { hipLaunchKernelGGL(qp_prep_kernel, dim3(1), dim3(256), d.lds_prep, 0, P); e = hipGetLastError(); }
+    if (e == hipSuccess) {
+      if (d.T == 1 && d.NB == 4) e = initial_point_launch<1, 4>(P, dout);
+      else if (d.T == 2 && d.NB == 4) e = initial_point_launch<2, 4>(P, dout);
+      else if (d.T == 2 && d.NB == 0) e = initial_point_launch<2, 0>(P, dout);
+      else if (d.T == 2 && d.NB == 1) e = initial_point_launch<2, 1>(P, dout);
+      else if (d.T == 5 && d.NB == 1) e = initial_point_launch<5, 1>(P, dout);
+      else { snprintf(msg, msglen, "initial-point selftest: shape (%d, %d) has T = %d, NB = %d, which the self test does not instantiate (FSAEMPC_SLACK_BORDER set?)", nV, nC, d.T, d.NB); e = hipErrorInvalidValue; }
+    }
+    if (e == hipSuccess) e = hipDeviceSynchronize();
+    if (e == hipSuccess) e = hipMemcpy(hout, dout, sizeof(hout), hipMemcpyDeviceToHost);
+  }
+  if (din) (void)hipFree(din);
+  if (ws) (void)hipFree(ws);
+  if (dout) (void)hipFree(dout);
+  if (e != hipSuccess) { if (!msg[0]) snprintf(msg, msglen, "initial-point selftest (%d, %d): %s", nV, nC, hipGetErrorString(e)); return -1; }
+  if (hout[0]) { snprintf(msg, msglen, "initial point (%d, %d): %d mismatches between the start-up pass and pass_Av + pass_Atw, first: %s index %d lane %d", nV, nC, hout[0], hout[1] ? "P3" : "aV", hout[2], hout[3]); return hout[0]; }
+  if (!hout[4]) { snprintf(msg, msglen, "initial point (%d, %d): both ways gave all zeros, nothing was compared", nV, nC); return 1; }
+  return 0;
+}
+
+int qp_selftest_initial_point(char* msg, int msglen) {
+  const int shapes[5][2] = {{20, 5}, {35, 70}, {32, 64}, {25, 72}, {81, 240}};
+  int bad = 0;
+  msg[0] = 0;
+  for (int i = 0; i < 5; ++i) {
+    const int rc = initial_point_shape(shapes[i][0], shapes[i][1], msg, msglen);
+    if (rc < 0) return rc;
+    bad += rc;
+    if (rc) break;
+  }
+  return bad;
+}
diff --git a/fsae-mpc_amd/csrc/qp_solve_kernel.h b/fsae-mpc_amd/csrc/qp_solve_kernel.h
--- a/fsae-mpc_amd/csrc/qp_solve_kernel.h
+++ b/fsae-mpc_amd/csrc/qp_solve_kernel.h
@@ -10,6 +10,9 @@
 #endif
 #ifndef QP_SYRK_INTERLEAVE
 #define QP_SYRK_INTERLEAVE 0
+#endif
+#ifndef QP_STARTUP_ATW
+#define QP_STARTUP_ATW 0
 #endif
 
 namespace {
@@ -293,11 +296,12 @@
 
 template <int T, int NB, int NVEC, int FUSE> DEVINL void pass_Av(const Ctx& k, Stream<T>& st, const double* const* vin, double* const* rout, double* Pcor, double* Pcor2 = nullptr, const double* const* cfarr = nullptr) {
   constexpr int NBB = NB > 0 ? NB : 1;
-  constexpr int NC = FUSE == 1 ? 6 : (FUSE >= 2 ? 3 : 0);
+  constexpr int NC = FUSE == 1 ? 6 : (FUSE >= 2 ? 3 : (FUSE == -1 ? 1 : 0));
   constexpr int NA = NC + NB;
   const int JS = k.J * 64;
   const double* arr[NA > 0 ? NA : 1];
   if (FUSE == 1) { arr[0] = rowp(k, R_RPL); arr[1] = rowp(k, R_CB1); arr[2] = rowp(k, R_CC1); arr[3] = rowp(k, R_RPU); arr[4] = rowp(k, R_CB2); arr[5] = rowp(k, R_CC2); }
+  if (FUSE == -1) arr[0] = rowp(k, R_W3);
   if (FUSE >= 2) { arr[0] = cfarr ? cfarr[0] : rowp(k, R_CB1); arr[1] = cfarr ? cfarr[1] : rowp(k, R_RPL); arr[2] = cfarr ? cfarr[2] : rowp(k, R_CC1); }
 #pragma unroll
   for (int f = 0; f < NB; ++f) arr[NC + f] = k.Ab + (size_t)f * JS;
@@ -366,6 +370,13 @@
             if (FUSE == 1 && e == 0) {
               const double dl_ = dsum + cf[0][h], du_ = cf[3][h] - dsum;
               const double w = dl_ * fma(cf[2][h], dl_, cf[1][h]) - du_ * fma(cf[5][h], du_, cf[4][h]);
+#pragma unroll
+              for (int t = 0; t < C; ++t) pc[t] = fma(w, b[t][h], pc[t]);
+#pragma unroll
+              for (int f = 0; f < NB; ++f) pcb[f] = fma(w, cf[NC + f][h], pcb[f]);
+            }
+            if (FUSE == -1 && e == 0) {
+              const double w = cf[0][h];
 #pragma unroll
               for (int t = 0; t < C; ++t) pc[t] = fma(w, b[t][h], pc[t]);
 #pragma unroll
@@ -706,13 +717,20 @@
 #ifndef QP_STAMPS
 #define QP_STAMPS 0
 #endif
+#if QP_STAMPS >= 2
+#define STAMP(id) STAMP_AT(((id) >= 1) ? 1 : 0)
+#define STAMP_SETUP(id) STAMP_AT(id)
+#else
+#define STAMP(id) STAMP_AT(id)
+#define STAMP_SETUP(id) do { } while (0)
+#endif
 #if QP_STAMPS
 #define STAMP_DECL unsigned long long st_acc[16]; for (int i_ = 0; i_ < 16; ++i_) st_acc[i_] = 0; unsigned long long st_t0 = __builtin_amdgcn_s_memtime();
-#define STAMP(id) do { __builtin_amdgcn_sched_barrier(0); unsigned long long t_ = __builtin_amdgcn_s_memtime(); st_acc[id] += t_ - st_t0; st_t0 = t_; __builtin_amdgcn_sched_barrier(0); } while (0)
+#define STAMP_AT(id) do { __builtin_amdgcn_sched_barrier(0); unsigned long long t_ = __builtin_amdgcn_s_memtime(); st_acc[id] += t_ - st_t0; st_t0 = t_; __builtin_amdgcn_sched_barrier(0); } while (0)
 #define STAMP_OUT do { if (P.dump && P.dump_stage == 9 && lane == 0) for (int i_ = 0; i_ < 16; ++i_) P.dump[(size_t)b * 16 + i_] = (double)st_acc[i_]; } while (0)
 #else
 #define STAMP_DECL
-#define STAMP(id) do { } while (0)
+#define STAMP_AT(id) do { } while (0)
 #define STAMP_OUT do { } while (0)
 #endif
 
@@ -802,6 +820,7 @@
   Stream<T> st;
   st.open(k);
 
+  const double T0 = 10.0, Z0 = 100.0;
   for (int i = lane; i < k.np; i += 64) { G[i] = gw[i]; EV[i] = Es[i]; R1[i] = 0; R2[i] = 0; DX[i] = 0; }
   int cnt_local = 0, infeas = 0;
   for (int js = 0; js < JT; ++js) {
@@ -818,6 +837,7 @@
       }
       cnt_local += (l > -INFINITY) + (u < INFINITY);
     }
+    aW3[ix] = (valid && js < J) ? ((l > -INFINITY ? Z0 : 0.0) - (u < INFINITY ? Z0 : 0.0)) : 0.0;
     if (js >= J) {
       const int i = (js - J) * 64 + lane;
       if (i < k.np) {
@@ -840,10 +860,14 @@
 
   {
     const double* vin[1] = {X}; double* rout[1] = {aV};
+#if QP_STARTUP_ATW
     pass_Av<T, NB, 1, 0>(k, st, vin, rout, nullptr);
+#else
+    pass_Av<T, NB, 1, -1>(k, st, vin, rout, P3);
+#endif
     for (int jb = 0; jb < k.JB; ++jb) { const int i = jb * 64 + lane; aV[(J + jb) * 64 + lane] = i < n ? X[i] : 0.0; }
   }
-  const double T0 = 10.0, Z0 = 100.0;
+  STAMP_SETUP(2);
   for (int js = 0; js < JT; ++js) {
     const int ix = js * 64 + lane;
     const bool valid = row_valid(k, js);
@@ -853,12 +877,15 @@
     aTU[ix] = hu ? fmax(u - v, T0) : 1.0;
     aZL[ix] = hl ? Z0 : 0.0;
     aZU[ix] = hu ? Z0 : 0.0;
-    aW3[ix] = (js < J) ? ((hl ? Z0 : 0.0) - (hu ? Z0 : 0.0)) : 0.0;
   }
   WAVE_SYNC();
+  STAMP_SETUP(3);
   {
     hx_full(X);
+    STAMP_SETUP(4);
+#if QP_STARTUP_ATW
     pass_Atw<T, NB>(k, aW3, P3);
+#endif
     WAVE_SYNC();
     for (int jb = 0; jb < k.JB; ++jb) {
       const int i = jb * 64 + lane, ix = (J + jb) * 64 + lane;
diff --git a/fsae-mpc_amd/csrc/qp_solver.h b/fsae-mpc_amd/csrc/qp_solver.h
--- a/fsae-mpc_amd/csrc/qp_solver.h
+++ b/fsae-mpc_amd/csrc/qp_solver.h
@@ -56,6 +56,7 @@
 int qp_selftest_mfma(char* msg, int msglen);
 int qp_selftest_lane_reduce(char* msg, int msglen);
 int qp_selftest_diag_factor(char* msg, int msglen);
+int qp_selftest_initial_point(char* msg, int msglen);
 #define QP_SOLVE_NVEC 10
 #define QP_SOLVE_RING(T) (3 * (T))
 struct QpSolveLds {
diff --git a/fsae-mpc_amd/csrc/qp_solver.hip b/fsae-mpc_amd/csrc/qp_solver.hip
--- a/fsae-mpc_amd/csrc/qp_solver.hip
+++ b/fsae-mpc_amd/csrc/qp_solver.hip
@@ -16,6 +16,11 @@
 #if QP_MAIN_TU
 namespace {
 
+#ifdef QP_PREP_STAMPS
+#define PSTAMP(id) do { __builtin_amdgcn_sched_barrier(0); const unsigned long long t_ = __builtin_amdgcn_s_memtime(); pst[id] += t_ - pst_t0; pst_t0 = t_; __builtin_amdgcn_sched_barrier(0); } while (0)
+#else
+#define PSTAMP(id) do { } while (0)
+#endif
 __global__ __launch_bounds__(1024) void qp_prep_kernel(QpParams P) {
   const int b = blockIdx.x, tid = threadIdx.x, w = tid >> 6, lane = tid & 63, c = lane & 15, q = lane >> 4;
   const int NTH = blockDim.x, NW = NTH >> 6;
@@ -54,6 +59,9 @@
   int* aoff_sh = tcs_sh + ntr;
   int* chc_sh = aoff_sh + ntr + 1;
   double* Fr_sh = reinterpret_cast<double*>((reinterpret_cast<uintptr_t>(chc_sh + ((m + 63) >> 6) * 16) + 7) & ~(uintptr_t)7);
+#ifdef QP_PREP_STAMPS
+  unsigned long long pst[8] = {0, 0, 0, 0, 0, 0, 0, 0}, pst_t0 = __builtin_amdgcn_s_memtime();
+#endif
 
   for (int j = tid; j < np; j += NTH) {
     double e = 1.0;
@@ -79,6 +87,7 @@
   int bad = 0;
   for (int j = tid; j < np; j += NTH) { const int uj = j < n ? U(j) : -1; const double gj = uj >= 0 ? g[uj] : 0.0; Es[j] = Esh[j]; gw[j] = gj * Esh[j]; bad |= !(fabs(gj) < INFINITY); }
 
+  PSTAMP(0);
   __syncthreads();
   const int ncols = nc < n ? nc : n;
   const int nchunk = (m + 63) >> 6;
@@ -110,6 +119,7 @@
     }
   }
   __syncthreads();
+  PSTAMP(1);
   if (tid < T) {
     int tot = 0;
     for (int ch = 0; ch < nchunk; ++ch) tot += chc_sh[ch * 16 + tid];
@@ -132,6 +142,7 @@
     }
   }
   __syncthreads();
+  PSTAMP(2);
   for (int tr = tid; tr < ntr; tr += NTH) {
     int tc = 1;
     for (int p = 16 * tr; p < 16 * tr + 16; ++p) { const int r = perm_sh[p]; if (r >= 0) tc = max(tc, cls_sh[r] + 1); }
@@ -146,6 +157,7 @@
   }
   __syncthreads();
   for (int tr = tid; tr <= ntr; tr += NTH) { aoff_g[tr] = aoff_sh[tr]; if (tr < ntr) tcs_g[tr] = tcs_sh[tr]; }
+  PSTAMP(3);
 
   int nexcl = 0;
   for (int js = w; js < J; js += NW) {
@@ -155,11 +167,15 @@
     const double f = valid ? Fr_sh[r] : 0.0;
     Fs[js * 64 + lane] = f;
     perm_g[js * 64 + lane] = r;
+    double ab[4], lr = 0.0, ur = 0.0;
+#pragma unroll
+    for (int bb = 0; bb < 4; ++bb) ab[bb] = (valid && bb < nb) ? Aat(r, nc + bb) : 0.0;
+    if (valid) { lr = P.lbA[(size_t)b * m + r]; ur = P.ubA[(size_t)b * m + r]; }
+#pragma unroll
     for (int bb = 0; bb < 4; ++bb)
-    { const double v = (valid && bb < nb) ? Aat(r, nc + bb) * Esh[nc + bb] * f : 0.0; bad |= !(fabs(v) < INFINITY); Ab[(size_t)bb * J * 64 + js * 64 + lane] = v; }
+    { const double v = (valid && bb < nb) ? ab[bb] * Esh[nc + bb] * f : 0.0; bad |= !(fabs(v) < INFINITY); Ab[(size_t)bb * J * 64 + js * 64 + lane] = v; }
     double l = -INFINITY, u = INFINITY;
     if (valid) {
-      double lr = P.lbA[(size_t)b * m + r], ur = P.ubA[(size_t)b * m + r];
       bad |= (lr != lr) || (ur != ur);
       nexcl += (lr > 0.0) || (ur < 0.0);
       l = lr > -P.inf_bound ? lr * f : -INFINITY;
@@ -183,44 +199,87 @@
     Ur[(J + jb) * 64 + lane] = u;
   }
   __syncthreads();
+  PSTAMP(4);
 
   const int R4 = 4 * Kq, mp1 = R4 + 1;
+  const int RCH = (R4 + 63) >> 6, NIT = TW * RCH;
   for (int t = 0; t < T; ++t)
     for (int c0 = 0; c0 < 16; c0 += TW) {
-      for (int e = tid; e < TW * R4; e += NTH) {
-        const int cc = e / R4, r = e - cc * R4;
-        const int col = 16 * t + c0 + cc;
-        double v = 0.0;
-        if (col < nc && col < n && r < m) v = Aat(r, col) * Esh[col];
-        bad |= !(fabs(v) < INFINITY);
-        tile[cc * mp1 + r] = v;
-      }
-      __syncthreads();
-      for (int s = w; s < 4 * ntr; s += NW) {
-        const int tr = s >> 2, tc = tcs_sh[tr];
-        if (t < tc && c >= c0 && c < c0 + TW) {
-          const int r = perm_sh[4 * s + q];
-          const double v = r >= 0 ? tile[(c - c0) * mp1 + r] * Fr_sh[r] : 0.0;
-          Aw[((size_t)aoff_sh[tr] + ((s >> 1) & 1) * tc + t) * 128 + lane * 2 + (s & 1)] = v;
+      for (int i0 = w; i0 < NIT; i0 += 8 * NW) {
+        double av[8];
+#pragma unroll
+        for (int u = 0; u < 8; ++u) {
+          const int i = i0 + u * NW, cc = i / RCH, r = (i - cc * RCH) * 64 + lane, col = 16 * t + c0 + cc;
+          av[u] = (i < NIT && col < nc && col < n && r < m) ? Aat(r, col) : 0.0;
+        }
+#pragma unroll
+        for (int u = 0; u < 8; ++u) {
+          const int i = i0 + u * NW, cc = i / RCH, r = (i - cc * RCH) * 64 + lane, col = 16 * t + c0 + cc;
+          if (i < NIT && r < R4) {
+            double v = 0.0;
+            if (col < nc && col < n && r < m) v = av[u] * Esh[col];
+            bad |= !(fabs(v) < INFINITY);
+            tile[cc * mp1 + r] = v;
+          }
         }
       }
       __syncthreads();
-    }
-
-  for (int idx = w; idx < T * T * 4; idx += NW) {
-    const int p = idx & 3, IJ = idx >> 2, I = IJ / T, Jt = IJ - I * T;
-    const int row = 16 * I + q + 4 * p, col = 16 * Jt + c;
-    double v = 0.0;
-    if (row < nc && col < nc && row < n && col < n) v = Hat(col, row) * Esh[row] * Esh[col];
-    bad |= !(fabs(v) < INFINITY);
-    Hw[(size_t)idx * 64 + lane] = v;
-  }
-  for (int e = tid; e < 4 * np; e += NTH) {
-    const int bb = e / np, i = e - bb * np;
-    const double v = (bb < nb && i < n) ? Hat(i, nc + bb) * Esh[nc + bb] * Esh[i] : 0.0;
-    bad |= !(fabs(v) < INFINITY);
-    Hb[e] = v;
-  }
+      for (int sp0 = w; sp0 < 2 * ntr; sp0 += 4 * NW) {
+        int r0[4], r1[4]; bool on[4];
+#pragma unroll
+        for (int u = 0; u < 4; ++u) {
+          const int sp = sp0 + u * NW;
+          on[u] = sp < 2 * ntr && t < tcs_sh[sp < 2 * ntr ? sp >> 1 : 0] && c >= c0 && c < c0 + TW;
+          r0[u] = on[u] ? perm_sh[8 * sp + q] : -1; r1[u] = on[u] ? perm_sh[8 * sp + 4 + q] : -1;
+        }
+        v2d v[4];
+#pragma unroll
+        for (int u = 0; u < 4; ++u) {
+          v[u][0] = r0[u] >= 0 ? tile[(c - c0) * mp1 + r0[u]] * Fr_sh[r0[u]] : 0.0;
+          v[u][1] = r1[u] >= 0 ? tile[(c - c0) * mp1 + r1[u]] * Fr_sh[r1[u]] : 0.0;
+        }
+#pragma unroll
+        for (int u = 0; u < 4; ++u) {
+          const int sp = sp0 + u * NW;
+          if (on[u]) { const int tr = sp >> 1, tc = tcs_sh[tr]; *reinterpret_cast<v2d*>(Aw + ((size_t)aoff_sh[tr] + (sp & 1) * tc + t) * 128 + lane * 2) = v[u]; }
+        }
+      }
+      __syncthreads();
+    }
+  PSTAMP(5);
+
+  for (int i0 = w; i0 < T * T * 4; i0 += 8 * NW) {
+    double hv[8];
+#pragma unroll
+    for (int u = 0; u < 8; ++u) {
+      const int idx = i0 + u * NW, p = idx & 3, IJ = idx >> 2, I = IJ / T, Jt = IJ - I * T;
+      const int row = 16 * I + q + 4 * p, col = 16 * Jt + c;
+      hv[u] = (idx < T * T * 4 && row < nc && col < nc && row < n && col < n) ? Hat(col, row) : 0.0;
+    }
+#pragma unroll
+    for (int u = 0; u < 8; ++u) {
+      const int idx = i0 + u * NW, p = idx & 3, IJ = idx >> 2, I = IJ / T, Jt = IJ - I * T;
+      const int row = 16 * I + q + 4 * p, col = 16 * Jt + c;
+      if (idx < T * T * 4) {
+        double v = 0.0;
+        if (row < nc && col < nc && row < n && col < n) v = hv[u] * Esh[row] * Esh[col];
+        bad |= !(fabs(v) < INFINITY);
+        Hw[(size_t)idx * 64 + lane] = v;
+      }
+    }
+  }
+  for (int i = tid; i < np; i += NTH) {
+    double hv[4];
+#pragma unroll
+    for (int bb = 0; bb < 4; ++bb) hv[bb] = (bb < nb && i < n) ? Hat(i, nc + bb) : 0.0;
+#pragma unroll
+    for (int bb = 0; bb < 4; ++bb) {
+      const double v = (bb < nb && i < n) ? hv[bb] * Esh[nc + bb] * Esh[i] : 0.0;
+      bad |= !(fabs(v) < INFINITY);
+      Hb[bb * np + i] = v;
+    }
+  }
+  PSTAMP(6);
   bad = __syncthreads_or(bad);
   if (tid == 0) ws[d.off_bad] = bad ? 1.0 : 0.0;
   if (P.score) {
@@ -231,6 +290,10 @@
     __syncthreads();
     if (tid == 0) P.score[b] = P.score_in ? P.score_in[b] : score_sh;
   }
+#ifdef QP_PREP_STAMPS
+  PSTAMP(7);
+  if (P.dump && P.dump_stage == 10 && tid == 0) for (int i = 0; i < 8; ++i) P.dump[(size_t)b * 8 + i] = (double)pst[i];
+#endif
 }
 
 __global__ __launch_bounds__(1024) void qp_order_kernel(const int* __restrict__ score, int* __restrict__ order, int batch) {
@@ -416,7 +479,7 @@
   }
   return hipErrorInvalidValue;
 }
-static int prep_thr() { static const char* e = getenv("FSAEMPC_PREP_THR"); return e ? atoi(e) : 256; }
+static int prep_thr() { static const char* e = getenv("FSAEMPC_PREP_THR"); return e ? atoi(e) : 512; }
 hipError_t qp_launch(const QpParams& P, int batch, hipStream_t st, hipEvent_t ev_mid) {
   hipError_t e = hipFuncSetAttribute(reinterpret_cast<const void*>(&qp_prep_kernel),
                                      hipFuncAttributeMaxDynamicSharedMemorySize, (int)P.d.lds_prep);
diff --git a/include/fsaempc.h b/include/fsaempc.h
--- a/include/fsaempc.h
+++ b/include/fsaempc.h
@@ -377,6 +377,7 @@
 int fsaempc_selftest_mfma(void);
 int fsaempc_selftest_lane_reduce(void);
 int fsaempc_selftest_diag_factor(void);
+int fsaempc_selftest_initial_point(void);
 int fsaempc_debug_set_dump(double* out, int stage);
 
 int fsaempc_qp_set_timing(int enable);
```

Result: faster. 433,700, median of 6 (+3.9%).
